# navallo/collision_avoidance

Hardware: AMD Instinct MI355X
Metric: agent-steps/sec (whole node), 4096 arenas x 64 agents per GPU (higher is better)
Workload: dtype f32

## Files before the change

### collision_avoidance_amd/_lib.py

```python
import ctypes as C
import os

from . import build as _build

OBS_DIM = 64
MAX_NEIGHBORS, MAX_OBST_NEIGHBORS, MAX_AGENTS = 16, 64, 1024
MAX_AGENTS_LARGE = 16384
CREATE_TILED = 1
DONE_XLESS, DONE_GOAL, DONE_REGOAL = 0, 1, 2
F_OBS, F_STATS, F_AUTORESET, F_NODONE, F_FREEZE = 1, 2, 4, 8, 16
SCN_CROWD, SCN_CIRCLE, SCN_DOORWAY, SCN_CONGESTED, SCN_INCOMING, SCN_BLOCKS, SCN_DEADLOCK, SCN_CROWD_SEPARATED = range(8)

(FLD_POS_X, FLD_POS_Y, FLD_VEL_X, FLD_VEL_Y, FLD_PREF_X, FLD_PREF_Y, FLD_GOAL_X, FLD_GOAL_Y,
 FLD_GOAL2_X, FLD_GOAL2_Y, FLD_REWARD, FLD_AGENT_DONE, FLD_ARRIVE_STEP, FLD_NB_COUNT, FLD_NB_IDX,
 FLD_OBST_COUNT, FLD_OBST_IDX, FLD_OBS, FLD_STEP_COUNT, FLD_ARENA_DONE, FLD_EPISODE,
 FLD_REGOAL_COUNT, FLD_ALAN_WEIGHTS, FLD_ALAN_TIMES, FLD_ALAN_ACTION, FLD_ARENA_STATS) = range(26)

EXPORTS = ("ca_create", "ca_destroy", "ca_last_error", "ca_set_stream", "ca_set_obstacles", "ca_init_scenario", "ca_set",
           "ca_get", "ca_field_ptr", "ca_bind_obs", "ca_reset", "ca_step", "ca_step_host", "ca_orca_step", "ca_observe", "ca_rollout",
           "ca_get_stats", "ca_reset_stats", "ca_sync", "ca_debug_math", "ca_profile", "ca_profile_read", "ca_launch_info",
           "ca_alan_configure", "ca_alan_step", "ca_alan_rollout", "ca_reset_masked", "ca_get_obstacles",
           "ca_set_obstacles_per_arena", "ca_get_obstacles_arena", "ca_solver_info", "ca_source_sha", "ca_host_alloc", "ca_host_free",
           "ca_step_packed", "ca_allow_obstacle_overflow", "ca_alan_configure_per_arena", "ca_alan_actions_arena",
           "ca_set_agent_params", "ca_get_agent_params", "ca_agent_params_info",
           "ca_set_agent_counts", "ca_get_agent_counts", "ca_agent_counts_info", "ca_create_ex", "ca_tiled_info")


class Config(C.Structure):
    _fields_ = [
        ("n_arenas", C.c_int32), ("n_agents", C.c_int32), ("arena_offset", C.c_int64),
        ("seed", C.c_uint64), ("reward_scale", C.c_double), ("time_step", C.c_float),
        ("neighbor_dist", C.c_float), ("max_neighbors", C.c_int32), ("time_horizon", C.c_float),
        ("time_horizon_obst", C.c_float), ("radius", C.c_float), ("max_speed", C.c_float),
        ("max_obst_neighbors", C.c_int32), ("max_step", C.c_int32), ("done_mode", C.c_int32),
        ("done_x_thresh", C.c_float), ("spawn_x0", C.c_float), ("spawn_x1", C.c_float),
        ("spawn_y0", C.c_float), ("spawn_y1", C.c_float), ("goal_x0", C.c_float),
        ("goal_x1", C.c_float), ("goal_y0", C.c_float), ("goal_y1", C.c_float),
    ]


class Stats(C.Structure):
    _fields_ = [("agent_steps", C.c_uint64), ("episodes", C.c_uint64), ("collisions", C.c_uint64),
                ("obst_collisions", C.c_uint64), ("goals_reached", C.c_uint64),
                ("obst_overflow", C.c_uint64), ("sum_reward", C.c_double)]

    def as_dict(self):
        return {k: getattr(self, k) for k, _ in self._fields_}


_lib = None


def lib_path():
    return _build.LIB_PATH


def load():
    global _lib
    if _lib is not None:
        return _lib
    path = lib_path()
    if not os.path.exists(path):
        raise RuntimeError("libcaenv.so is not built (%s); run `python -m collision_avoidance_amd.build` "
                           "-- the HIP extension is the only implementation of this path" % path)
    L = C.CDLL(path)
    vp, i32, u32, sz = C.c_void_p, C.c_int32, C.c_uint32, C.c_size_t
    L.ca_create.argtypes = [C.POINTER(Config), C.c_int, vp, C.POINTER(vp)]
    L.ca_create_ex.argtypes = [C.POINTER(Config), u32, C.c_int, vp, C.POINTER(vp)]
    L.ca_tiled_info.argtypes = [vp] + [C.POINTER(i32)] * 4
    L.ca_destroy.argtypes = [vp]
    L.ca_last_error.argtypes = [vp]
    L.ca_last_error.restype = C.c_char_p
    L.ca_set_stream.argtypes = [vp, vp]
    L.ca_set_obstacles.argtypes = [vp, vp, vp, i32]
    L.ca_init_scenario.argtypes = [vp, i32]
    L.ca_get_obstacles.argtypes = [vp, vp, vp, vp, i32, C.POINTER(i32)]
    L.ca_set_obstacles_per_arena.argtypes = [vp, vp, vp, vp]
    L.ca_get_obstacles_arena.argtypes = [vp, i32, vp, vp, vp, i32, C.POINTER(i32)]
    L.ca_set.argtypes = [vp, i32, vp, sz, i32]
    L.ca_get.argtypes = [vp, i32, vp, sz, i32]
    L.ca_field_ptr.argtypes = [vp, i32, C.POINTER(vp), C.POINTER(sz)]
    L.ca_bind_obs.argtypes = [vp, vp, sz]
    L.ca_reset.argtypes = [vp, vp, vp, i32, u32]
    L.ca_reset_masked.argtypes = [vp, vp, i32, u32]
    L.ca_step.argtypes = [vp, vp, u32]
    L.ca_step_host.argtypes = [vp, vp, u32]
    L.ca_step_packed.argtypes = [vp, vp, u32, vp, sz]
    L.ca_host_alloc.argtypes = [vp, sz, C.POINTER(vp)]
    L.ca_host_free.argtypes = [vp, vp]
    L.ca_orca_step.argtypes = [vp, u32]
    L.ca_observe.argtypes = [vp]
    L.ca_rollout.argtypes = [vp, i32, u32]
    L.ca_alan_configure.argtypes = [vp, vp, i32, C.c_double, C.c_double, C.c_double]
    L.ca_alan_configure_per_arena.argtypes = [vp, vp, vp, C.c_double, C.c_double, C.c_double]
    L.ca_alan_actions_arena.argtypes = [vp, i32, vp, i32, C.POINTER(i32)]
    L.ca_alan_step.argtypes = [vp, vp, i32, u32]
    L.ca_alan_rollout.argtypes = [vp, i32, u32]
    L.ca_get_stats.argtypes = [vp, C.POINTER(Stats)]
    L.ca_reset_stats.argtypes = [vp]
    L.ca_sync.argtypes = [vp]
    L.ca_allow_obstacle_overflow.argtypes = [vp, i32]
    L.ca_debug_math.argtypes = [vp, i32, vp, vp, i32]
    L.ca_profile.argtypes = [vp, i32]
    L.ca_profile_read.argtypes = [vp, C.POINTER(i32), C.POINTER(C.c_float)]
    L.ca_launch_info.argtypes = [vp] + [C.POINTER(i32)] * 4
    L.ca_solver_info.argtypes = [vp, C.POINTER(i32), C.POINTER(i32)]
    L.ca_set_agent_params.argtypes = [vp, vp, vp, vp, vp, sz, i32]
    L.ca_get_agent_params.argtypes = [vp, vp, vp, vp, vp, sz, i32]
    L.ca_agent_params_info.argtypes = [vp, C.POINTER(i32)]
    L.ca_set_agent_counts.argtypes = [vp, vp, sz, i32]
    L.ca_get_agent_counts.argtypes = [vp, vp, sz, i32]
    L.ca_agent_counts_info.argtypes = [vp, C.POINTER(i32)]
    L.ca_source_sha.argtypes = []
    L.ca_source_sha.restype = C.c_char_p
    for name in EXPORTS:
        if name not in ("ca_last_error", "ca_source_sha"):
            getattr(L, name).restype = C.c_int
    _lib = L
    return L


def check(L, handle, rc, what):
    if rc != 0:
        msg = L.ca_last_error(handle)
        raise RuntimeError("%s failed (%d): %s" % (what, rc, msg.decode() if msg else "?"))
```

### collision_avoidance_amd/csrc/ca_common.h

```cpp
#pragma once
#include "ca_math.h"
#include <type_traits>
#include <utility>

struct AlanArenaSets;
struct WideObstLists;
struct AgentParams;
struct ArenaCounts;

namespace ca {

template <class T, class... P> constexpr bool has_tag = (std::is_same_v<T, P> || ...);

constexpr int SMAX = 16;
constexpr int SWIDE = 64;
constexpr float EPS = 0.00001f;

struct ObstDev {
    float px, py, ux, uy;
    float qx, qy, qux, quy;
    float pux, puy;
    int next, prev;
    int convex, qconvex, pad0, pad1;
};
static_assert(sizeof(ObstDev) == 64, "edge record is one 64-byte line");

struct Line {
    V2 point, dir;
};

struct StepCold {
    float *pos_x, *pos_y, *vel_x, *vel_y, *pref_x, *pref_y;
    double *goal_x, *goal_y;
    const double *goal2_x, *goal2_y;
    float* reward;
    float *orient_x, *orient_y;
    int *agent_done, *arrive_step, *regoal_count;
    int *step_count, *arena_done, *episode;
    unsigned long long* arena_stats;
    unsigned long long* arena_steps;
    unsigned long long* ovf_word;
    double reward_scale;
    uint64_t seed;
    int64_t arena_offset;
    int max_step, done_mode;
    float done_x_thresh;
    float spawn_x0, spawn_x1, spawn_y0, spawn_y1, goal_x0, goal_x1, goal_y0, goal_y1;
    const float *ap_radius, *ap_max_speed, *ap_time_horizon, *ap_time_horizon_obst;
    const int* agent_counts;
};

struct AlanCold {
    double *w, *t;
    int* action;
    float* reward;
    double act_c[32], act_s[32];
    double temp, window, dt, reward_scale;
    const double2* tab;
    const int* tab_n;
    int nA;
};

template <int ALAN, class AL>
__device__ __forceinline__ int alan_count(const AL& al, int a) {
    if constexpr (ALAN == 2) return al.tab_n[a];
    else return al.nA;
}
template <int ALAN, class AL>
__device__ __forceinline__ void alan_cs(const AL& al, int a, int id, double* cs, double* sn) {
    if constexpr (ALAN == 2) {
        const double2 v = al.tab[(size_t)a * 32 + id];
        *cs = v.x; *sn = v.y;
    } else {
        *cs = al.act_c[id]; *sn = al.act_s[id];
    }
}

struct StepArgs {
    const float *pos_x, *pos_y, *vel_x, *vel_y, *pref_x, *pref_y;
    const double *goal_x, *goal_y;
    unsigned short* counts;
    void* nb_idx;
    unsigned short* obst_idx;
    const int* arena_done;
    unsigned long long* arena_stats;
    const StepCold* cold;
    const ObstDev* obst;
    const int* tab_off;
#ifdef CA_STAMPS
    const int* order;
#endif
    const AlanCold* alan;
    const double* alan_u;
    const float* actions;
    const float* reset_px;
    const float* reset_py;
    const int* reset_mask;
    unsigned long long* dbg;
    int n_obst, A, N, P, logP, K, S;
    int a0, a1;
    int LS, apb, linv, dense;
    int nb_hint;
    int T;
    uint32_t flags;
    float time_step, neighbor_dist, time_horizon, time_horizon_obst, radius, max_speed;
};

__device__ __forceinline__ void note_overflow(const StepCold* cold, int a, int i, int oin) {
    const unsigned long long g = (unsigned long long)(cold->arena_offset + (int64_t)a) & 0xFFFFFFFFFFull;
    const unsigned long long v = (1ull << 63) | (g << 20) | ((unsigned long long)(i & 0x7FF) << 8) | (unsigned long long)(oin > 255 ? 255 : oin);
    __hip_atomic_store(cold->ovf_word, v, __ATOMIC_RELAXED, __HIP_MEMORY_SCOPE_SYSTEM);
}

enum { ST_EPISODES = 0, ST_COLL = 1, ST_OBST_COLL = 2, ST_GOALS = 3, ST_OVERFLOW = 4, ST_SUMREW = 5, ST_FROZEN = 6, ST_LASTEP = 7, ST_STRIDE = 8 };

#ifdef CA_STAMPS
__device__ __forceinline__ int work_block(const StepArgs& p) { return p.order ? p.order[blockIdx.x] : (int)blockIdx.x; }
#else
__device__ __forceinline__ int work_block(const StepArgs&) { return (int)blockIdx.x; }
#endif

__device__ __forceinline__ void lane_slot(const StepArgs& p, int tid, int& la, int& i) {
    la = (int)(__umul24((unsigned)tid, (unsigned)p.linv) >> 16);
    i = tid - (int)__umul24((unsigned)la, (unsigned)p.LS);
}

__device__ __forceinline__ bool arena_frozen(const StepArgs& p, int a) {
    return (p.flags & 16u) != 0 && a < p.a1 && p.arena_done[a] != 0;
}

__device__ __forceinline__ void wave_lds_sync() {
    __builtin_amdgcn_fence(__ATOMIC_RELEASE, "wavefront");
    __builtin_amdgcn_s_waitcnt(0xC07F);
    __builtin_amdgcn_wave_barrier();
    __builtin_amdgcn_fence(__ATOMIC_ACQUIRE, "wavefront");
}

#define CA_ROW_DPP(old, v, ctrl, rows) __builtin_amdgcn_update_dpp((int)(old), (int)(v), ctrl, rows, 0xF, false)
__device__ __forceinline__ unsigned wave_min_u32(unsigned v) {
    v = min(v, (unsigned)CA_ROW_DPP(~0u, v, 0x111, 0xF));
    v = min(v, (unsigned)CA_ROW_DPP(~0u, v, 0x112, 0xF));
    v = min(v, (unsigned)CA_ROW_DPP(~0u, v, 0x114, 0xF));
    v = min(v, (unsigned)CA_ROW_DPP(~0u, v, 0x118, 0xF));
    v = min(v, (unsigned)CA_ROW_DPP(~0u, v, 0x142, 0xA));
    v = min(v, (unsigned)CA_ROW_DPP(~0u, v, 0x143, 0xC));
    return v;
}
__device__ __forceinline__ unsigned wave_max_u32(unsigned v) {
    v = max(v, (unsigned)CA_ROW_DPP(0u, v, 0x111, 0xF));
    v = max(v, (unsigned)CA_ROW_DPP(0u, v, 0x112, 0xF));
    v = max(v, (unsigned)CA_ROW_DPP(0u, v, 0x114, 0xF));
    v = max(v, (unsigned)CA_ROW_DPP(0u, v, 0x118, 0xF));
    v = max(v, (unsigned)CA_ROW_DPP(0u, v, 0x142, 0xA));
    v = max(v, (unsigned)CA_ROW_DPP(0u, v, 0x143, 0xC));
    return v;
}
__device__ __forceinline__ int wave_prefix_sum(int v) {
    v += CA_ROW_DPP(0, v, 0x111, 0xF);
    v += CA_ROW_DPP(0, v, 0x112, 0xF);
    v += CA_ROW_DPP(0, v, 0x114, 0xF);
    v += CA_ROW_DPP(0, v, 0x118, 0xF);
    v += CA_ROW_DPP(0, v, 0x142, 0xA);
    v += CA_ROW_DPP(0, v, 0x143, 0xC);
    return v;
}

#ifdef CA_VAR_NB16
#define CA_NBW16(BS) true
#else
#define CA_NBW16(BS) ((BS) > 256)
#endif
#define CA_GLOBAL __attribute__((address_space(1)))
template <bool W16>
__device__ __forceinline__ int ld_idx_t(const void* b, size_t k) {
    if constexpr (W16) return (int)((const CA_GLOBAL unsigned short*)b)[k];
    else return (int)((const CA_GLOBAL unsigned char*)b)[k];
}
template <bool W16>
__device__ __forceinline__ void st_idx_t(void* b, size_t k, int v) {
    if constexpr (W16) ((CA_GLOBAL unsigned short*)b)[k] = (unsigned short)v;
    else ((CA_GLOBAL unsigned char*)b)[k] = (unsigned char)v;
}

__device__ __forceinline__ ObstDev load_obst(const ObstDev* __restrict__ t, int i) {
    const int4* q = reinterpret_cast<const int4*>(t + i);
    const int4 a = q[0], b = q[1], c = q[2], d = q[3];
    ObstDev o;
    o.px = __int_as_float(a.x); o.py = __int_as_float(a.y); o.ux = __int_as_float(a.z); o.uy = __int_as_float(a.w);
    o.qx = __int_as_float(b.x); o.qy = __int_as_float(b.y); o.qux = __int_as_float(b.z); o.quy = __int_as_float(b.w);
    o.pux = __int_as_float(c.x); o.puy = __int_as_float(c.y); o.next = c.z; o.prev = c.w;
    o.convex = d.x; o.qconvex = d.y; o.pad0 = 0; o.pad1 = 0;
    return o;
}

#ifndef CA_PRIO_B1
#define CA_PRIO_B1 2
#define CA_PRIO_B2 4
#define CA_PRIO_B3 6
#endif
#if CA_PRIO_B1 > 0
#define CA_PRIO_START() __builtin_amdgcn_s_setprio(3)
#define CA_PRIO_POINT(x)                                                    \
// ... 48 lines not shown
```

### collision_avoidance_amd/csrc/ca_env.hip

```cpp
#include "../../include/ca_env.h"

#include <hip/hip_runtime.h>
#include <hip/hip_ext.h>

#include <algorithm>
#include <cmath>
#include <cstdarg>
#include <cstdlib>
#include <cstdio>
#include <cstring>
#include <string>
#include <vector>

#include "ca_kernels.h"

using namespace ca;

struct ca_env {
    ca_config cfg;
    int device = 0;
    hipStream_t stream = nullptr;
    bool own_stream = false;
    float *pos_x = nullptr, *pos_y = nullptr, *vel_x = nullptr, *vel_y = nullptr, *pref_x = nullptr,
          *pref_y = nullptr, *reward = nullptr, *orient_x = nullptr, *orient_y = nullptr;
    bool orient_valid = false;
    double *goal_x = nullptr, *goal_y = nullptr, *goal2_x = nullptr, *goal2_y = nullptr;
    int *agent_done = nullptr, *arrive_step = nullptr, *regoal_count = nullptr;
    unsigned short* counts = nullptr;
    void* nb_idx = nullptr;
    unsigned short* obst_idx = nullptr;
    int nidx16 = 0;
    int* cvt_buf = nullptr;
    size_t cvt_cap = 0;
    int *step_count = nullptr, *arena_done = nullptr, *episode = nullptr;
    unsigned long long* arena_stats = nullptr;
    unsigned long long* arena_steps = nullptr;
    float* obs = nullptr;
    bool obs_external = false;
    float* slab = nullptr;
    unsigned long long* dbg = nullptr;
    unsigned long long* dbg_obs = nullptr;
    float *tmp_x = nullptr, *tmp_y = nullptr;
    double *alan_w = nullptr, *alan_t = nullptr, *alan_dirs = nullptr, *alan_u = nullptr;
    int* alan_action = nullptr;
    AlanCold* d_alan = nullptr;
    bool alan_fused = false;
    bool alan_lane = false;
    int* mask_buf = nullptr;
    std::vector<std::pair<void*, size_t>> host_allocs;
    int n_actions = 0;
    double act_c[CA_ALAN_MAX_ACTIONS], act_s[CA_ALAN_MAX_ACTIONS];
    bool alan_per = false;
    double2* d_act_tab = nullptr;
    int* d_act_n = nullptr;
    std::vector<double> h_act_tab;
    std::vector<int> h_act_n;
    double alan_temp = 0.2, alan_window = 2.0, alan_dt = 1.0 / 60.0;
    ObstDev* d_obst = nullptr;
    std::vector<ObstDev> h_obst;
    std::vector<int> h_tab_off;
    int* d_tab_off = nullptr;
    StepCold* d_cold = nullptr;
    unsigned long long* ovf_host = nullptr;
    bool allow_overflow = false;
    int* d_order = nullptr;
    int P = 1, logP = 0, BS = 64, grid = 1, K = 0, S = 1;
    bool obs_dense_on = false;
    bool lists_trusted = true;
    int LS = 1, apb = 1, linv = 65536, dense = 0;
    struct { int reg_lines = -1, pair = -1, alan_fused = -1; } sw;
    int ST = 0, KT = 16;
    int SMX = 4;
    int max_edges = 0;
    int n_cus = 256;
    bool pair = false;
    size_t lds_p = 0;
    bool quad = false;
    bool quad_roll = false;
    int BSq = 64, grid_q = 1, SQ = 4;
    size_t lds_q = 0;
    size_t lds = 0;
    bool ap = false, quad_cfg = false, quad_roll_cfg = false;
    float* d_ap[4] = {nullptr, nullptr, nullptr, nullptr};
    float* d_ap_oct = nullptr;
    std::vector<float> h_ap[4];
    bool ac = false, ap_user = false;
    int* d_counts = nullptr;
    std::vector<int> h_counts;
    bool tiled = false;
    int TILE = 128, tiles = 1;
    float *nv_x = nullptr, *nv_y = nullptr;
    unsigned* tscr = nullptr;
    uint64_t agent_steps_base = 0;
    uint64_t steps_done = 0;
    float rays[32], oct[32];
    bool profiling = false;
    int prof_period = 0;
    struct Span { hipEvent_t t0, t1; int kind; int steps; };
    std::vector<Span> spans;
    std::vector<hipEvent_t> free_events;
    std::string err;
};

static thread_local std::string g_create_err;

static int fail(ca_env* e, int code, const char* fmt, ...) {
    char buf[512];
    va_list ap;
    va_start(ap, fmt);
    vsnprintf(buf, sizeof buf, fmt, ap);
    va_end(ap);
    if (e) e->err = buf;
    else g_create_err = buf;
    return code;
}
#define HIPCHK(e, call)                                                                         \
    do {                                                                                        \
        hipError_t _r = (call);                                                                 \
        if (_r != hipSuccess) return fail(e, CA_EHIP, "%s failed: %s", #call, hipGetErrorString(_r)); \
    } while (0)

static int overflow_status(ca_env* e, const char* where) {
    if (e->allow_overflow || !e->ovf_host) return CA_OK;
    const unsigned long long v = *(volatile unsigned long long*)e->ovf_host;
    if (!(v >> 63)) return CA_OK;
    return fail(e, CA_ERANGE, "%s: an obstacle-neighbour list overflowed: arena %lld, agent %d had %d%s obstacle edges in range but "
                "max_obst_neighbors=%d, so the farthest were dropped (RVO2 keeps every edge in range: collision_avoidence_env.py:249, "
                "301-318).  Raise max_obst_neighbors (at most %d), coarsen the world's polylines, or accept the truncation with "
                "ca_allow_obstacle_overflow(env, 1); ca_reset_stats clears this status", where,
                (long long)(e->tiled ? (v >> 24) & 0xFFFFFFFFFull : (v >> 20) & 0xFFFFFFFFFFull),
                (int)(e->tiled ? (v >> 8) & 0xFFFF : (v >> 8) & 0x7FF), (int)(v & 0xFF), (v & 0xFF) == 255 ? "+" : "",
                e->S, CA_MAX_OBST_NEIGHBORS);
}

enum { KIND_NBR = 0, KIND_STEP = 1, KIND_OBS = 2, KIND_RESET = 3 };
enum { CA_ROLLOUT_MAX_T = 256 };
static hipEvent_t prof_event(ca_env* e) {
    if (!e->free_events.empty()) { hipEvent_t ev = e->free_events.back(); e->free_events.pop_back(); return ev; }
    hipEvent_t ev = nullptr;
    if (hipEventCreate(&ev) != hipSuccess) return nullptr;
    return ev;
}
struct ProfScope {
    ca_env* e; hipEvent_t t0 = nullptr, t1 = nullptr; int kind; int steps;
    ProfScope(ca_env* env, int k, int n_steps = 1) : e(env), kind(k), steps(n_steps) {
        if (!e->profiling) return;
        t0 = prof_event(e);
        t1 = t0 ? prof_event(e) : nullptr;
        if (t0 && !t1) { e->free_events.push_back(t0); t0 = nullptr; }
    }
    ~ProfScope() {
        if (t0) e->spans.push_back({t0, t1, kind, steps});
    }
};
template <class... Args>
static void launch_k(const ProfScope& ps, void (*kernel)(Args...), dim3 grid, dim3 block, size_t lds, hipStream_t stream,
                     Args... args) {
    if (ps.t0) hipExtLaunchKernelGGL(kernel, grid, block, (uint32_t)lds, stream, ps.t0, ps.t1, 0, args...);
    else hipLaunchKernelGGL(kernel, grid, block, lds, stream, args...);
}

static size_t AN(const ca_env* e) { return (size_t)e->cfg.n_arenas * e->cfg.n_agents; }

struct FieldInfo {
    void* ptr;
    size_t bytes;
    bool writable;
};
static FieldInfo field_info(ca_env* e, int f) {
    const size_t an = AN(e), A = e->cfg.n_arenas;
    switch (f) {
        case CA_FLD_POS_X: return {e->pos_x, an * 4, true};
        case CA_FLD_POS_Y: return {e->pos_y, an * 4, true};
        case CA_FLD_VEL_X: return {e->vel_x, an * 4, true};
        case CA_FLD_VEL_Y: return {e->vel_y, an * 4, true};
        case CA_FLD_PREF_X: return {e->pref_x, an * 4, true};
        case CA_FLD_PREF_Y: return {e->pref_y, an * 4, true};
        case CA_FLD_GOAL_X: return {e->goal_x, an * 8, true};
        case CA_FLD_GOAL_Y: return {e->goal_y, an * 8, true};
        case CA_FLD_GOAL2_X: return {e->goal2_x, an * 8, true};
        case CA_FLD_GOAL2_Y: return {e->goal2_y, an * 8, true};
        case CA_FLD_REWARD: return {e->reward, an * 4, true};
        case CA_FLD_AGENT_DONE: return {e->agent_done, an * 4, true};
        case CA_FLD_ARRIVE_STEP: return {e->arrive_step, an * 4, true};
        case CA_FLD_NB_COUNT: return {e->counts, an * 4, true};
        case CA_FLD_NB_IDX: return {e->nb_idx, an * 4 * (size_t)(e->K > 0 ? e->K : 1), true};
        case CA_FLD_OBST_COUNT: return {e->counts, an * 4, true};
        case CA_FLD_OBST_IDX: return {e->obst_idx, an * 4 * (size_t)e->S, true};
        case CA_FLD_OBS: return {e->obs, an * CA_OBS_DIM * 4, false};
        case CA_FLD_STEP_COUNT: return {e->step_count, A * 4, true};
        case CA_FLD_ARENA_DONE: return {e->arena_done, A * 4, true};
        case CA_FLD_EPISODE: return {e->episode, A * 4, true};
        case CA_FLD_REGOAL_COUNT: return {e->regoal_count, an * 4, true};
        case CA_FLD_ALAN_WEIGHTS: return {e->alan_w, an * 8 * (size_t)e->n_actions, true};
        case CA_FLD_ALAN_TIMES: return {e->alan_t, an * 8 * (size_t)e->n_actions, true};
        case CA_FLD_ALAN_ACTION: return {e->alan_action, an * 4, true};
        case CA_FLD_ARENA_STATS: return {e->arena_stats, A * ST_STRIDE * 8, false};
        default: return {nullptr, 0, false};
    }
}

static void host_tables(ca_env* e) {
    const double nd = (double)e->cfg.neighbor_dist, r = (double)e->cfg.radius;
    for (int i = 0; i < 16; ++i) {
        const double th = i * (2.0 * M_PI / 16);
        e->rays[2 * i] = (float)(nd * std::cos(th));
        e->rays[2 * i + 1] = (float)(-nd * std::sin(th));
    }
    double first[2] = {r * std::cos(0.0), -r * std::sin(0.0)}, cur[2] = {first[0], first[1]};
    int k = 0;
    for (int i = 1; i < 8; ++i, ++k) {
        const double th = i * (2.0 * M_PI / 8);
        const double nx = r * std::cos(th), ny = -r * std::sin(th);
        e->oct[4 * k] = (float)cur[0]; e->oct[4 * k + 1] = (float)cur[1];
        e->oct[4 * k + 2] = (float)nx; e->oct[4 * k + 3] = (float)ny;
        cur[0] = nx; cur[1] = ny;
    }
    e->oct[4 * k] = (float)cur[0]; e->oct[4 * k + 1] = (float)cur[1];
    e->oct[4 * k + 2] = (float)first[0]; e->oct[4 * k + 3] = (float)first[1];
}

static void fill_cold(const ca_env* e, StepCold& c) {
    const ca_config& g = e->cfg;
    c.pos_x = e->pos_x; c.pos_y = e->pos_y; c.vel_x = e->vel_x; c.vel_y = e->vel_y;
    c.pref_x = e->pref_x; c.pref_y = e->pref_y; c.goal_x = e->goal_x; c.goal_y = e->goal_y;
    c.goal2_x = e->goal2_x; c.goal2_y = e->goal2_y; c.reward = e->reward;
    c.orient_x = e->orient_x; c.orient_y = e->orient_y;
    c.agent_done = e->agent_done; c.arrive_step = e->arrive_step; c.regoal_count = e->regoal_count;
    c.step_count = e->step_count; c.arena_done = e->arena_done; c.episode = e->episode;
    c.arena_stats = e->arena_stats; c.arena_steps = e->arena_steps; c.ovf_word = e->ovf_host;
    c.reward_scale = g.reward_scale; c.seed = g.seed; c.arena_offset = g.arena_offset;
    c.max_step = g.max_step; c.done_mode = g.done_mode; c.done_x_thresh = g.done_x_thresh;
    c.spawn_x0 = g.spawn_x0; c.spawn_x1 = g.spawn_x1; c.spawn_y0 = g.spawn_y0; c.spawn_y1 = g.spawn_y1;
    c.goal_x0 = g.goal_x0; c.goal_x1 = g.goal_x1; c.goal_y0 = g.goal_y0; c.goal_y1 = g.goal_y1;
    c.ap_radius = e->ap ? e->d_ap[0] : nullptr; c.ap_max_speed = e->ap ? e->d_ap[1] : nullptr;
    c.ap_time_horizon = e->ap ? e->d_ap[2] : nullptr; c.ap_time_horizon_obst = e->ap ? e->d_ap[3] : nullptr;
    c.agent_counts = e->ac ? e->d_counts : nullptr;
}

static void fill_args(ca_env* e, StepArgs& a, const float* actions, uint32_t flags) {
    const ca_config& c = e->cfg;
    a.pos_x = e->pos_x; a.pos_y = e->pos_y; a.vel_x = e->vel_x; a.vel_y = e->vel_y;
    a.pref_x = e->pref_x; a.pref_y = e->pref_y; a.goal_x = e->goal_x; a.goal_y = e->goal_y;
    a.counts = e->counts; a.nb_idx = e->nb_idx; a.obst_idx = e->obst_idx;
    a.arena_done = e->arena_done; a.arena_stats = e->arena_stats; a.cold = e->d_cold;
    a.obst = e->d_obst; a.tab_off = e->d_tab_off; a.actions = actions; a.alan = nullptr; a.alan_u = nullptr;
#ifdef CA_STAMPS
    a.order = e->d_order;
#endif
    a.reset_px = nullptr; a.reset_py = nullptr; a.reset_mask = nullptr; a.dbg = e->dbg;
    a.n_obst = e->h_tab_off.empty() ? (int)e->h_obst.size() : 0; a.A = c.n_arenas; a.N = c.n_agents; a.P = e->P; a.logP = e->logP;
    a.K = e->K; a.S = e->S; a.flags = flags; a.a0 = 0; a.a1 = c.n_arenas; a.T = 1;
    a.LS = e->LS; a.apb = e->apb; a.linv = e->linv; a.dense = e->dense; a.nb_hint = e->lists_trusted ? 1 : 0;
    a.time_step = c.time_step; a.neighbor_dist = c.neighbor_dist; a.time_horizon = c.time_horizon;
    a.time_horizon_obst = c.time_horizon_obst; a.radius = c.radius; a.max_speed = c.max_speed;
}

struct SolveLaunch { const void* fn; dim3 grid, block; size_t lds; };
template <class F> static const void* fn_ptr(F* f) { return reinterpret_cast<const void*>(f); }
template <int KMAX, int ST, int SMX, bool ALAN, class... PER>
static const void* step_fn_for(int BS) {
    if constexpr (ALAN) {
        return BS == 64 ? fn_ptr(&step_kernel<KMAX, 64, ST, SMX, true, PER...>) : fn_ptr(&step_kernel<KMAX, 128, ST, SMX, true, PER...>);
    } else {
        switch (BS) {
            case 64: return fn_ptr(&step_kernel<KMAX, 64, ST, SMX>);
            case 128: return fn_ptr(&step_kernel<KMAX, 128, ST, SMX>);
            case 256: return fn_ptr(&step_kernel<KMAX, 256, ST, SMX>);
            case 512: return fn_ptr(&step_kernel<KMAX, 512, ST, SMX>);
            default: return fn_ptr(&step_kernel<KMAX, 1024, ST, SMX>);
        }
    }
}
template <int KMAX>
static const void* pair_fn_for(int BS) {
    return BS == 256 ? fn_ptr(&pair_kernel<KMAX, 256>) : fn_ptr(&pair_kernel<KMAX, 512>);
}
template <int KMAX, int SQ, bool ALAN, class... PER>
static const void* quad_fn_for(int BS) {
    switch (BS) {
        case 64: return fn_ptr(&quad_kernel<KMAX, 64, SQ, ALAN, PER...>);
        case 128: return fn_ptr(&quad_kernel<KMAX, 128, SQ, ALAN, PER...>);
        case 256: return fn_ptr(&quad_kernel<KMAX, 256, SQ, ALAN, PER...>);
        default: return fn_ptr(&quad_kernel<KMAX, 512, SQ, ALAN, PER...>);
    }
}
template <int KMAX>
static const void* wide_fn_for(int BS) {
    return BS == 64 ? fn_ptr(&step_kernel<KMAX, 64, 0, SWIDE>) : fn_ptr(&step_kernel<KMAX, 128, 0, SWIDE>);
}
template <int KMAX>
static const void* ap_fn_for(int BS) {
    switch (BS) {
        case 64: return fn_ptr(&step_kernel<KMAX, 64, 0, SMAX, false, AgentParams>);
        case 128: return fn_ptr(&step_kernel<KMAX, 128, 0, SMAX, false, AgentParams>);
        case 256: return fn_ptr(&step_kernel<KMAX, 256, 0, SMAX, false, AgentParams>);
        case 512: return fn_ptr(&step_kernel<KMAX, 512, 0, SMAX, false, AgentParams>);
        default: return fn_ptr(&step_kernel<KMAX, 1024, 0, SMAX, false, AgentParams>);
    }
}
template <int KMAX>
static const void* ac_fn_for(int BS) {
    switch (BS) {
        case 64: return fn_ptr(&step_kernel<KMAX, 64, 0, SMAX, false, ArenaCounts>);
        case 128: return fn_ptr(&step_kernel<KMAX, 128, 0, SMAX, false, ArenaCounts>);
        case 256: return fn_ptr(&step_kernel<KMAX, 256, 0, SMAX, false, ArenaCounts>);
        case 512: return fn_ptr(&step_kernel<KMAX, 512, 0, SMAX, false, ArenaCounts>);
        default: return fn_ptr(&step_kernel<KMAX, 1024, 0, SMAX, false, ArenaCounts>);
    }
}
template <bool ALAN, class... PER>
static const void* lane_fn_for(const ca_env* e) {
    if (e->ac) return e->KT == 5 ? ac_fn_for<5>(e->BS) : (e->KT == 16 ? ac_fn_for<16>(e->BS) : ac_fn_for<10>(e->BS));
    if (e->ap) return e->KT == 5 ? ap_fn_for<5>(e->BS) : (e->KT == 16 ? ap_fn_for<16>(e->BS) : ap_fn_for<10>(e->BS));
    if (e->SMX > SMAX) return e->KT == 5 ? wide_fn_for<5>(e->BS) : (e->KT == 16 ? wide_fn_for<16>(e->BS) : wide_fn_for<10>(e->BS));
    if (e->ST > 0 && e->SMX > 4) return e->KT == 5 ? step_fn_for<5, 4, 16, ALAN, PER...>(e->BS) : step_fn_for<10, 4, 16, ALAN, PER...>(e->BS);
    if (e->ST > 0) return e->KT == 5 ? step_fn_for<5, 4, 4, ALAN, PER...>(e->BS) : step_fn_for<10, 4, 4, ALAN, PER...>(e->BS);
    if (e->KT == 5) return step_fn_for<5, 0, SMAX, ALAN, PER...>(e->BS);
    if constexpr (!ALAN) { if (e->KT == 16) return step_fn_for<16, 0, SMAX, false>(e->BS); }
    return step_fn_for<10, 0, SMAX, ALAN, PER...>(e->BS);
}
template <bool ALAN, class... PER>
static const void* quad_fn_for(const ca_env* e) {
    if (e->SQ > 4) return e->KT == 5 ? quad_fn_for<5, 16, ALAN, PER...>(e->BSq) : quad_fn_for<10, 16, ALAN, PER...>(e->BSq);
    return e->KT == 5 ? quad_fn_for<5, 4, ALAN, PER...>(e->BSq) : quad_fn_for<10, 4, ALAN, PER...>(e->BSq);
}
template <int KMAX>
static const void* tiled_fn_for(int TILE) {
    switch (TILE) {
        case 64: return fn_ptr(&tiled_solve_kernel<KMAX, 64>);
        case 256: return fn_ptr(&tiled_solve_kernel<KMAX, 256>);
        default: return fn_ptr(&tiled_solve_kernel<KMAX, 128>);
    }
}
static SolveLaunch solve_launch(const ca_env* e, bool alan, bool rollout) {
    if (e->tiled)
        return {e->KT == 5 ? tiled_fn_for<5>(e->TILE) : (e->KT == 16 ? tiled_fn_for<16>(e->TILE) : tiled_fn_for<10>(e->TILE)),
                dim3(e->grid), dim3(e->TILE), e->lds};
    const bool per = alan && e->alan_per;
    if (e->quad || (rollout && e->quad_roll) || (alan && !e->alan_lane)) {
        const void* f = per ? quad_fn_for<true, AlanArenaSets>(e) : (alan ? quad_fn_for<true>(e) : quad_fn_for<false>(e));
        return {f, dim3(e->grid_q), dim3(e->BSq), alan ? quad_lds_bytes(e->BSq, e->KT, e->SQ, e->n_actions) : e->lds_q};
    }
    if (e->pair)
        return {e->KT == 5 ? pair_fn_for<5>(e->BS) : pair_fn_for<10>(e->BS), dim3(e->grid), dim3(2 * e->BS), e->lds_p};
    const void* f = per ? lane_fn_for<true, AlanArenaSets>(e) : (alan ? lane_fn_for<true>(e) : lane_fn_for<false>(e));
    return {f, dim3(e->grid), dim3(e->BS), e->lds};
}
static hipError_t allow_lds(const SolveLaunch& s) {
    return s.lds > 48 * 1024 ? hipFuncSetAttribute(s.fn, hipFuncAttributeMaxDynamicSharedMemorySize, (int)s.lds) : hipSuccess;
}
static hipError_t launch_step(ca_env* e, const StepArgs& a) {
    const SolveLaunch s = solve_launch(e, a.alan != nullptr, a.T > 1);
    if (!(a.flags & CA_F_FREEZE)) e->lists_trusted = true;
    if (e->tiled) {
        TiledArgs ta;
        ta.s = a; ta.nv_x = e->nv_x; ta.nv_y = e->nv_y; ta.scr = e->tscr; ta.tiles = e->tiles;
        void* params[] = {&ta};
        const void* fns[3] = {s.fn, fn_ptr(&tiled_advance_kernel), fn_ptr(&tiled_close_kernel)};
        const size_t lds[3] = {s.lds, 0, (size_t)e->TILE * 8};
        for (int k = 0; k < 3; ++k) {
            ProfScope ps(e, KIND_STEP);
            const hipError_t r = ps.t0 ? hipExtLaunchKernel(fns[k], s.grid, s.block, params, lds[k], e->stream, ps.t0, ps.t1, 0)
                                       : hipLaunchKernel(fns[k], s.grid, s.block, params, lds[k], e->stream);
            if (r != hipSuccess) return r;
        }
        return hipSuccess;
    }
    ProfScope ps(e, KIND_STEP, a.T > 1 ? a.T : 1);
    StepArgs arg = a;
    void* params[] = {&arg};
    if (ps.t0) return hipExtLaunchKernel(s.fn, s.grid, s.block, params, s.lds, e->stream, ps.t0, ps.t1, 0);
    return hipLaunchKernel(s.fn, s.grid, s.block, params, s.lds, e->stream);
}

typedef void (*obs_fn_t)(const ObsArgs);
static obs_fn_t obs_fn(int obs_bs, bool w16, bool dense = false, bool wide = false, bool ap = false, bool ac = false) {
    if (ac) return dense ? obs_kernel<256, false, true, ArenaCounts> : (w16 ? obs_kernel<256, true, false, ArenaCounts> : obs_kernel<256, false, false, ArenaCounts>);
    if (ap) return dense ? obs_kernel<256, false, true, AgentParams> : (w16 ? obs_kernel<256, true, false, AgentParams> : obs_kernel<256, false, false, AgentParams>);
    if (wide) return dense ? obs_kernel<256, false, true, WideObstLists> : obs_kernel<256, false, false, WideObstLists>;
    if (dense) return obs_kernel<256, false, true>;
    switch (obs_bs) {
        case 1024: return w16 ? obs_kernel<1024, true> : obs_kernel<1024, false>;
        case 512: return w16 ? obs_kernel<512, true> : obs_kernel<512, false>;
        case 128: return w16 ? obs_kernel<128, true> : obs_kernel<128, false>;
        case 64: return w16 ? obs_kernel<64, true> : obs_kernel<64, false>;
        default: return w16 ? obs_kernel<256, true> : obs_kernel<256, false>;
    }
}

static bool obs_dense(const ca_env* e) { return e->obs_dense_on; }
static int obs_nstage(const ca_env* e) { return e->tiled ? 0 : (obs_dense(e) ? 16 + 2 * e->cfg.n_agents : e->cfg.n_agents); }
static bool obs_wide(const ca_env* e) { return e->S > SMAX; }
static size_t obs_lds(const ca_env* e, int obs_bs) {
    if (e->ap) return obs_lds_bytes_ap(obs_nstage(e), obs_bs, 16 * (e->K + e->S));
    return obs_lds_bytes(obs_nstage(e), obs_bs, 16 * (e->K + e->S), obs_wide(e) ? e->S : 16);
}
static obs_fn_t obs_fn_of(const ca_env* e) { return obs_fn(obs_block_threads(e->cfg.n_agents), e->nidx16 != 0, obs_dense(e), obs_wide(e), e->ap, e->ac); }
static hipError_t allow_obs_lds(const ca_env* e) {
    const size_t ol = obs_lds(e, obs_block_threads(e->cfg.n_agents));
    return ol > 48 * 1024 ? hipFuncSetAttribute(reinterpret_cast<const void*>(obs_fn_of(e)), hipFuncAttributeMaxDynamicSharedMemorySize, (int)ol) : hipSuccess;
}

static hipError_t launch_obs(ca_env* e) {
    if (!e->orient_valid) {
        StepArgs a;
        fill_args(e, a, nullptr, 0);
        const unsigned an = (unsigned)AN(e);
        hipLaunchKernelGGL(orient_kernel, dim3((an + 255) / 256), dim3(256), 0, e->stream, a);
        hipError_t r = hipGetLastError();
        if (r != hipSuccess) return r;
        e->orient_valid = true;
    }
    ObsArgs o;
    o.pos_x = e->pos_x; o.pos_y = e->pos_y; o.vel_x = e->vel_x; o.vel_y = e->vel_y;
    o.orient_x = e->orient_x; o.orient_y = e->orient_y; o.counts = e->counts; o.nb_idx = e->nb_idx;
    o.obst_idx = e->obst_idx; o.obst = e->d_obst; o.tab_off = e->d_tab_off;
    o.obs = e->obs;
    o.A = e->cfg.n_arenas; o.N = e->cfg.n_agents; o.S = e->S;
    o.K = e->K > 0 ? e->K : 1;
    const int obs_bs = obs_block_threads(o.N), apb = obs_bs / 16;
    o.bpa = (o.N + apb - 1) / apb;
    o.paircap = 16 * (e->K + e->S);
    o.a0 = 0; o.dbg = e->dbg_obs;
    o.dense = obs_dense(e) ? 1 : 0;
    o.nstage_max = obs_nstage(e);
    o.xcd = (o.A % 8 == 0 && !o.dense) ? 1 : 0;
    o.radius = e->cfg.radius;
    memcpy(o.rays, e->rays, sizeof o.rays);
    memcpy(o.oct, e->oct, sizeof o.oct);
    o.ap_oct = e->ap ? e->d_ap_oct : nullptr;
    o.agent_counts = e->ac ? e->d_counts : nullptr;
    const dim3 grid(o.dense ? (unsigned)(((size_t)o.A * o.N + apb - 1) / apb) : (unsigned)((size_t)o.A * o.bpa)), block(obs_bs);
    const size_t lds = obs_lds(e, obs_bs);
    ProfScope ps(e, KIND_OBS);
    launch_k(ps, obs_fn_of(e), grid, block, lds, e->stream, o);
    return hipGetLastError();
}

static hipError_t launch_reset(ca_env* e, const StepArgs& a) {
    const unsigned an = (unsigned)AN(e);
    {
        ProfScope ps(e, KIND_RESET);
        launch_k(ps, e->ac ? reset_counts_kernel : reset_kernel, dim3((an + 255) / 256), dim3(256), 0, e->stream, a);
    }
    hipError_t r = hipGetLastError();
    if (r != hipSuccess) return r;
    {
        ProfScope ps(e, KIND_RESET);
        launch_k(ps, reset_arena_kernel, dim3((e->cfg.n_arenas + 255) / 256), dim3(256), 0, e->stream, a);
    }
    return hipGetLastError();
}

static void split_crossing_edges(std::vector<ObstDev>& tab) {
    struct Side { int left, right; };
    auto sides = [&](int split, int edge, float* a, float* b) {
        const V2 s1 = mk(tab[split].px, tab[split].py), s2 = mk(tab[tab[split].next].px, tab[tab[split].next].py);
        *a = leftOf(s1, s2, mk(tab[edge].px, tab[edge].py));
        *b = leftOf(s1, s2, mk(tab[tab[edge].next].px, tab[tab[edge].next].py));
    };
    auto worse_or_equal = [](Side x, Side y) {
        const int xm = x.left > x.right ? x.left : x.right, xn = x.left < x.right ? x.left : x.right;
        const int ym = y.left > y.right ? y.left : y.right, yn = y.left < y.right ? y.left : y.right;
        return xm > ym || (xm == ym && xn >= yn);
    };
    std::vector<std::vector<int>> work(1);
    for (int i = 0; i < (int)tab.size(); ++i) work[0].push_back(i);
    while (!work.empty()) {
        const std::vector<int> edges = std::move(work.back());
        work.pop_back();
        const int n = (int)edges.size();
        if (n == 0) continue;
        int pick = 0;
        Side best = {n, n};
        for (int i = 0; i < n; ++i) {
            Side c = {0, 0};
            for (int j = 0; j < n; ++j) {
                if (j == i) continue;
                float a, b;
                sides(edges[i], edges[j], &a, &b);
                if (a >= -EPS && b >= -EPS) ++c.left;
                else if (a <= EPS && b <= EPS) ++c.right;
                else { ++c.left; ++c.right; }
                if (worse_or_equal(c, best)) break;
            }
            if (!worse_or_equal(c, best)) { best = c; pick = i; }
        }
        std::vector<int> lhs, rhs;
        const int sp = edges[pick];
        const V2 s1 = mk(tab[sp].px, tab[sp].py), s2 = mk(tab[tab[sp].next].px, tab[tab[sp].next].py);
        for (int j = 0; j < n; ++j) {
            if (j == pick) continue;
            const int e1 = edges[j], e2 = tab[e1].next;
            float a, b;
            sides(sp, e1, &a, &b);
            if (a >= -EPS && b >= -EPS) { lhs.push_back(e1); continue; }
            if (a <= EPS && b <= EPS) { rhs.push_back(e1); continue; }
            const V2 p1 = mk(tab[e1].px, tab[e1].py), p2 = mk(tab[e2].px, tab[e2].py);
            const float t = det(s2 - s1, p1 - s1) / det(s2 - s1, p1 - p2);
            const V2 cut = p1 + t * (p2 - p1);
            ObstDev o;
            memset(&o, 0, sizeof o);
            o.px = cut.x; o.py = cut.y; o.ux = tab[e1].ux; o.uy = tab[e1].uy;
            o.prev = e1; o.next = e2; o.convex = 1;
            const int id = (int)tab.size();
            tab.push_back(o);
            tab[e1].next = id; tab[e2].prev = id;
            if (a > 0.0f) { lhs.push_back(e1); rhs.push_back(id); }
            else { rhs.push_back(e1); lhs.push_back(id); }
        }
        work.push_back(std::move(rhs));
        work.push_back(std::move(lhs));
    }
}

template <class T>
static hipError_t dalloc(ca_env* e, T** p, size_t n, bool zero = true) {
    hipError_t r = hipMalloc((void**)p, n * sizeof(T));
    if (r != hipSuccess || !zero) return r;
    return hipMemsetAsync(*p, 0, n * sizeof(T), e->stream);
}
static hipError_t upload(ca_env* e, void* dst, const void* src, size_t bytes) {
    hipError_t r = hipMemcpyAsync(dst, src, bytes, hipMemcpyHostToDevice, e->stream);
    return r != hipSuccess ? r : hipStreamSynchronize(e->stream);
}
static hipError_t download(ca_env* e, void* dst, const void* src, size_t bytes) {
    hipError_t r = hipMemcpyAsync(dst, src, bytes, hipMemcpyDeviceToHost, e->stream);
    return r != hipSuccess ? r : hipStreamSynchronize(e->stream);
}

static size_t lds_static_bytes(const ca_env* e) {
    return (size_t)e->BS * 8 +
           (e->BS >= 1024 ? (size_t)e->BS * 2 + 16 + 1024 + 1028 : (e->BS >= 256 ? (size_t)e->BS * 2 + (size_t)e->BS * 8 + 16 + 4096 + 4100 : 0)) + 64;
}

static void pick_variant(ca_env* e) {
    const bool allow = e->sw.reg_lines != 0, force = e->sw.reg_lines == 1;
    e->KT = e->K <= 5 ? 5 : (e->K <= 10 ? 10 : 16);
    if (e->tiled) {
        e->ST = 0; e->SMX = SMAX; e->pair = false;
        e->lds = tiled_lds_bytes(e->TILE, e->K, e->S);
        return;
    }
    const size_t table_per_wg = step_lds_bytes(e->BS, e->K, e->S, 0, e->KT) + lds_static_bytes(e);
    const bool table_fits = table_per_wg <= 160 * 1024;
    const bool small_world = e->max_edges <= 16;
    const bool table_resident = table_fits && (long)e->grid <= (long)e->n_cus * (long)((160 * 1024) / table_per_wg);
    if (e->S > SMAX) { e->ST = 0; e->SMX = SWIDE; }
    else if (e->ap) { e->ST = 0; e->SMX = SMAX; }
    else if (allow && e->K <= 10 && e->S <= 4) { e->ST = 4; e->SMX = 4; }
    else if (allow && e->K <= 10 && (small_world || force || !table_resident)) { e->ST = 4; e->SMX = 16; }
    else { e->ST = 0; e->SMX = 16; }
    e->lds = e->ap ? step_lds_bytes_ap(e->BS, e->K, e->S) : step_lds_bytes(e->BS, e->K, e->S, e->ST, e->KT);
    e->pair = e->sw.pair != 0 && e->ST > 0 && e->SMX == 4 && (e->BS == 256 || e->BS == 512) && e->K > 0;
    e->lds_p = pair_lds_bytes(e->BS, e->KT);
}

static const size_t LDS_PER_CU = 160 * 1024;
static hipError_t apply_variant_attributes(ca_env* e, bool* misfit) {
    const SolveLaunch plain = solve_launch(e, false, false);
    if (e->tiled) { *misfit = false; return allow_lds(plain); }
    *misfit = !e->pair && e->lds + lds_static_bytes(e) > LDS_PER_CU;
    hipError_t r = hipSuccess;
    if (e->pair) {
        hipFuncAttributes fa;
        r = hipFuncGetAttributes(&fa, plain.fn);
        *misfit = r == hipSuccess && fa.sharedSizeBytes + plain.lds > LDS_PER_CU;
    }
    if (r != hipSuccess || *misfit) return r;
    r = allow_lds(plain);
    if (r == hipSuccess) r = allow_lds(solve_launch(e, false, true));
    return r;
}

static int alan_pick(ca_env* e) {
    e->alan_fused = e->alan_lane = false;
    if (e->n_actions <= 0 || e->tiled) return CA_OK;
    const size_t lq = quad_lds_bytes(e->BSq, e->KT, e->SQ, e->n_actions);
    const bool on = e->sw.alan_fused != 0;
    e->alan_fused = on && (e->quad || e->quad_roll) && lq <= 64 * 1024;
    e->alan_lane = on && !e->ap && !e->quad && !e->pair && e->BS <= 128 && e->K <= 10 && e->S <= SMAX &&
                   e->n_actions <= (e->ST > 0 ? 4 + e->KT : 2 * (e->K + e->S));
    if (e->alan_fused) HIPCHK(e, allow_lds(solve_launch(e, true, true)));
    if (e->alan_lane) HIPCHK(e, allow_lds(solve_launch(e, true, false)));
    return CA_OK;
}

extern "C" {

const char* ca_last_error(const ca_env* env) { return env ? env->err.c_str() : g_create_err.c_str(); }

int ca_create(const ca_config* cfg, int device, void* stream, ca_env** out) { return ca_create_ex(cfg, 0u, device, stream, out); }

int ca_create_ex(const ca_config* cfg, uint32_t create_flags, int device, void* stream, ca_env** out) {
    if (!cfg || !out) return fail(nullptr, CA_EINVAL, "ca_create: null argument");
    *out = nullptr;
    if (create_flags & ~CA_CREATE_TILED) return fail(nullptr, CA_EINVAL, "ca_create_ex: unknown create_flags 0x%x", create_flags);
    const bool tiled = (create_flags & CA_CREATE_TILED) != 0;
    const int max_agents = tiled ? CA_MAX_AGENTS_LARGE : CA_MAX_AGENTS;
    if (cfg->n_arenas <= 0 || cfg->n_agents <= 0 || cfg->n_agents > max_agents)
        return fail(nullptr, CA_ERANGE, "ca_create: n_arenas=%d n_agents=%d out of range (agents 1..%d)",
                    cfg->n_arenas, cfg->n_agents, max_agents);
    if (tiled && cfg->max_obst_neighbors > SMAX)
        return fail(nullptr, CA_ERANGE, "ca_create_ex: max_obst_neighbors=%d: wide obstacle lists (above %d) have no tiled form",
                    cfg->max_obst_neighbors, SMAX);
    if (cfg->max_neighbors < 0 || cfg->max_neighbors > CA_MAX_NEIGHBORS)
        return fail(nullptr, CA_ERANGE, "ca_create: max_neighbors=%d out of range 0..%d", cfg->max_neighbors,
                    CA_MAX_NEIGHBORS);
    if (cfg->max_obst_neighbors < 1 || cfg->max_obst_neighbors > CA_MAX_OBST_NEIGHBORS)
        return fail(nullptr, CA_ERANGE, "ca_create: max_obst_neighbors=%d out of range 1..%d",
                    cfg->max_obst_neighbors, CA_MAX_OBST_NEIGHBORS);
    if (cfg->done_mode < 0 || cfg->done_mode > 2) return fail(nullptr, CA_EINVAL, "ca_create: bad done_mode");
    {
        const struct { const char* name; float v, lo, hi; } rng[] = {
            {"time_step", cfg->time_step, CA_MIN_TIME_STEP, CA_MAX_TIME_STEP}, {"neighbor_dist", cfg->neighbor_dist, CA_MIN_LENGTH, CA_MAX_LENGTH},
            {"time_horizon", cfg->time_horizon, CA_MIN_LENGTH, CA_MAX_LENGTH}, {"time_horizon_obst", cfg->time_horizon_obst, CA_MIN_LENGTH, CA_MAX_LENGTH},
            {"radius", cfg->radius, CA_MIN_LENGTH, CA_MAX_LENGTH}, {"max_speed", cfg->max_speed, CA_MIN_LENGTH, CA_MAX_LENGTH}};
        for (const auto& q : rng)
            if (!(q.v >= q.lo && q.v <= q.hi))
                return fail(nullptr, CA_ERANGE, "ca_create: %s=%g outside the supported range [%g, %g]", q.name, (double)q.v, (double)q.lo, (double)q.hi);
        const float box[] = {cfg->spawn_x0, cfg->spawn_x1, cfg->spawn_y0, cfg->spawn_y1, cfg->goal_x0, cfg->goal_x1, cfg->goal_y0, cfg->goal_y1,
                             cfg->done_x_thresh};
        for (float v : box)
            if (!(fabsf(v) <= CA_MAX_COORD)) return fail(nullptr, CA_ERANGE, "ca_create: a spawn / goal box coordinate (%g) is beyond %g or not a number", (double)v, (double)CA_MAX_COORD);
    }
    if ((size_t)cfg->n_arenas * cfg->n_agents > (size_t)1 << 30)
        return fail(nullptr, CA_ERANGE, "ca_create: more than 2^30 agents on one handle");
    int ndev = 0;
    if (hipGetDeviceCount(&ndev) != hipSuccess || ndev <= 0)
        return fail(nullptr, CA_ENODEV, "ca_create: no HIP device (this library has no CPU path)");
    if (device < 0 || device >= ndev) return fail(nullptr, CA_ENODEV, "ca_create: device %d of %d", device, ndev);
    ca_env* e = new ca_env();
    e->cfg = *cfg;
    e->device = device;
    hipError_t r = hipSetDevice(device);
    if (r == hipSuccess) {
        if (stream) e->stream = (hipStream_t)stream;
        else { r = hipStreamCreateWithFlags(&e->stream, hipStreamNonBlocking); e->own_stream = true; }
    }
    {
        auto digit = [](const char* name) { const char* v = getenv(name); return (v && v[0] >= '0' && v[0] <= '9') ? v[0] - '0' : -1; };
        e->sw.reg_lines = digit("CA_REG_LINES"); e->sw.pair = digit("CA_PAIR"); e->sw.alan_fused = digit("CA_ALAN_FUSED");
    }
    e->tiled = tiled;
    if (tiled) {
        const char* v = getenv("CA_TILE");
        const int want = v ? atoi(v) : 0;
        e->TILE = (want == 64 || want == 256) ? want : 128;
        e->tiles = (cfg->n_agents + e->TILE - 1) / e->TILE;
    }
    int P = 1, logP = 0;
    while (P < cfg->n_agents) { P <<= 1; ++logP; }
    e->P = P; e->logP = logP;
    e->BS = P > 64 ? P : 64;
    e->LS = P; e->apb = e->BS / P; e->linv = 65536 / P; e->dense = 0;
    e->grid = (cfg->n_arenas + e->apb - 1) / e->apb;
    if (tiled) {
        if ((size_t)cfg->n_arenas * e->tiles > (size_t)0x7FFFFFFF) {
            fail(nullptr, CA_ERANGE, "ca_create_ex: n_arenas=%d x %d tiles per arena is more workgroups than a launch holds", cfg->n_arenas, e->tiles);
            if (e->own_stream && e->stream) hipStreamDestroy(e->stream);
            delete e;
            return CA_ERANGE;
        }
        e->BS = e->TILE; e->LS = e->TILE; e->apb = 1; e->linv = 65536 / e->TILE;
        e->grid = cfg->n_arenas * e->tiles;
    }
    {
        const char* v = getenv("CA_OBS_DENSE");
        e->obs_dense_on = !tiled && cfg->n_agents < 16 && !(v && v[0] == '0');
    }
    {
        const char* v = getenv("CA_DENSE");
        const int N = cfg->n_agents;
        if (!tiled && !(v && v[0] == '0') && e->BS == 64 && P < 64 && 64 / N > 64 / P) {
            const int linv = (65536 + N - 1) / N;
            bool exact = true;
            for (int t = 0; t < 64; ++t) exact = exact && ((t * linv) >> 16) == t / N;
            if (exact) {
                e->LS = N; e->apb = 64 / N; e->linv = linv; e->dense = 1;
                e->grid = (cfg->n_arenas + e->apb - 1) / e->apb;
            }
        }
    }
    e->K = cfg->max_neighbors;
    e->S = cfg->max_obst_neighbors;
    {
        int cus = 0;
        if (hipDeviceGetAttribute(&cus, hipDeviceAttributeMultiprocessorCount, device) == hipSuccess && cus > 0) e->n_cus = cus;
    }
    pick_variant(e);
    {
        const char* v = getenv("CA_QUAD");
        e->SQ = e->S <= 4 ? 4 : 16;
        const bool fits = !tiled && e->S <= SMAX && e->K <= 10 && 4 * P <= ((e->SQ == 16 && e->KT == 10) ? 256 : 512);
        const long lane_waves = tiled ? 0 : (long)((cfg->n_arenas + e->BS / P - 1) / (e->BS / P)) * (e->BS / 64);
        e->quad = fits && (v ? v[0] == '1' : lane_waves < 1024);
        e->quad_roll = fits && (v ? v[0] == '1' : lane_waves <= 1024);
        e->BSq = 4 * P > 64 ? 4 * P : 64;
        const int apbq = (e->BSq / 4) / P;
        e->grid_q = (cfg->n_arenas + apbq - 1) / apbq;
        e->lds_q = quad_lds_bytes(e->BSq, e->KT, e->SQ);
        e->quad_cfg = e->quad; e->quad_roll_cfg = e->quad_roll;
    }
    if (e->S > SMAX && (e->lds + lds_static_bytes(e) > LDS_PER_CU || e->BS > 128 || obs_block_threads(cfg->n_agents) != 256)) {
        if (e->lds + lds_static_bytes(e) > LDS_PER_CU)
            fail(nullptr, CA_ERANGE, "ca_create: the solve kernel for n_agents=%d, max_neighbors=%d, max_obst_neighbors=%d does not fit the "
                 "160 KiB of LDS of a CU (%zu B: obstacle lists above %d take the LDS line table, max_neighbors + max_obst_neighbors lines "
                 "per lane)", cfg->n_agents, e->K, e->S, e->lds + lds_static_bytes(e), SMAX);
        else
            fail(nullptr, CA_ERANGE, "ca_create: max_obst_neighbors=%d: obstacle lists above %d are built for arenas of at most 128 agents "
                 "(n_agents=%d)", e->S, SMAX, cfg->n_agents);
        if (e->own_stream && e->stream) hipStreamDestroy(e->stream);
        delete e;
        return CA_ERANGE;
    }
    if (!tiled && !e->pair && e->lds + lds_static_bytes(e) > LDS_PER_CU) {
        fail(nullptr, CA_ERANGE, "ca_create: the solve kernel would need %zu B of LDS (> 160 KiB) for n_agents=%d, "
             "max_neighbors=%d, max_obst_neighbors=%d: arenas above 256 agents need max_neighbors <= 10 "
             "(register-line variant)", e->lds + lds_static_bytes(e), cfg->n_agents, e->K, e->S);
        if (e->own_stream && e->stream) hipStreamDestroy(e->stream);
        delete e;
        return CA_ERANGE;
    }
    host_tables(e);
    const size_t an = AN(e), A = cfg->n_arenas;
    float** f32s[] = {&e->pos_x, &e->pos_y, &e->vel_x, &e->vel_y, &e->pref_x, &e->pref_y,
                      &e->tmp_x, &e->tmp_y, &e->orient_x, &e->orient_y};
    for (auto p : f32s) if (r == hipSuccess) r = dalloc(e, p, an);
    double** f64s[] = {&e->goal_x, &e->goal_y, &e->goal2_x, &e->goal2_y};
    for (auto p : f64s) if (r == hipSuccess) r = dalloc(e, p, an);
    int** i32s[] = {&e->agent_done, &e->arrive_step, &e->regoal_count};
    for (auto p : i32s) if (r == hipSuccess) r = dalloc(e, p, an);
    if (tiled) {
        if (r == hipSuccess) r = dalloc(e, &e->nv_x, an);
        if (r == hipSuccess) r = dalloc(e, &e->nv_y, an);
        if (r == hipSuccess) r = dalloc(e, &e->tscr, A * (size_t)TS_STRIDE);
    }
    e->nidx16 = (tiled || CA_NBW16(e->BS)) ? 1 : 0;
    if (r == hipSuccess) r = dalloc(e, &e->counts, an);
    if (r == hipSuccess) r = dalloc(e, reinterpret_cast<unsigned char**>(&e->nb_idx),
                                    an * (size_t)(e->K > 0 ? e->K : 1) * (e->nidx16 ? 2 : 1));
    if (r == hipSuccess) r = dalloc(e, &e->obst_idx, an * (size_t)e->S);
    if (r == hipSuccess) r = dalloc(e, &e->slab, an * CA_OBS_DIM + an + 2 * A);
    if (r == hipSuccess) {
        e->obs = e->slab; e->reward = e->slab + an * CA_OBS_DIM;
        e->arena_done = reinterpret_cast<int*>(e->reward + an); e->step_count = e->arena_done + A;
    }
    if (r == hipSuccess) r = dalloc(e, &e->episode, A);
    if (r == hipSuccess) r = dalloc(e, &e->arena_stats, A * ST_STRIDE);
    if (r == hipSuccess) r = dalloc(e, &e->arena_steps, A);
    if (r == hipSuccess) r = dalloc(e, &e->d_obst, (size_t)1);
#ifdef CA_STAMPS
    if (r == hipSuccess) r = dalloc(e, &e->dbg, (size_t)std::max(e->grid * (2 * e->BS / 64), e->grid_q * (e->BSq / 64)) * 16);
    if (r == hipSuccess) r = dalloc(e, &e->dbg_obs, (size_t)cfg->n_arenas * ((cfg->n_agents + 15) / 16 + 16) * 4 * 16);
#endif
    bool lds_misfit = false;
    if (r == hipSuccess) r = apply_variant_attributes(e, &lds_misfit);
    if (r == hipSuccess) r = allow_obs_lds(e);
    if (r == hipSuccess) {
        r = hipHostMalloc((void**)&e->ovf_host, sizeof(unsigned long long), hipHostMallocDefault);
        if (r == hipSuccess) *e->ovf_host = 0ull;
    }
    if (r == hipSuccess) r = hipMalloc((void**)&e->d_cold, sizeof(StepCold));
    if (r == hipSuccess) {
        StepCold hc;
        fill_cold(e, hc);
        r = upload(e, e->d_cold, &hc, sizeof hc);
    }
    if (r == hipSuccess) r = hipStreamSynchronize(e->stream);
    if (r == hipSuccess && lds_misfit) {
        fail(nullptr, CA_ERANGE, "ca_create: the solve kernel for n_agents=%d, max_neighbors=%d, max_obst_neighbors=%d does not fit the "
             "160 KiB of LDS of a CU", cfg->n_agents, e->K, e->S);
        ca_destroy(e);
        return CA_ERANGE;
    }
    if (r != hipSuccess) {
        fail(nullptr, CA_EHIP, "ca_create: %s", hipGetErrorString(r));
        ca_destroy(e);
        return CA_EHIP;
    }
    *out = e;
    return CA_OK;
}

int ca_destroy(ca_env* e) {
    if (!e) return CA_OK;
    hipSetDevice(e->device);
    if (e->stream) hipStreamSynchronize(e->stream);
    void* bufs[] = {e->pos_x, e->pos_y, e->vel_x, e->vel_y, e->pref_x, e->pref_y, e->goal_x, e->goal_y,
                    e->goal2_x, e->goal2_y, e->slab, e->tmp_x, e->tmp_y, e->orient_x, e->orient_y,
                    e->agent_done, e->arrive_step,
                    e->regoal_count, e->counts, e->nb_idx, e->obst_idx, e->cvt_buf, e->d_tab_off, e->d_cold, e->d_order,
                    e->episode, e->arena_stats, e->arena_steps, e->d_obst, e->dbg, e->dbg_obs,
                    e->alan_w, e->alan_t, e->alan_dirs, e->alan_u, e->alan_action, e->d_alan, e->mask_buf,
                    e->d_act_tab, e->d_act_n, e->d_ap[0], e->d_ap[1], e->d_ap[2], e->d_ap[3], e->d_ap_oct, e->d_counts,
                    e->nv_x, e->nv_y, e->tscr};
    for (void* b : bufs) if (b) hipFree(b);
    for (const auto& h : e->host_allocs) hipHostFree(h.first);
    if (e->ovf_host) hipHostFree(e->ovf_host);
    for (const ca_env::Span& sp : e->spans) { hipEventDestroy(sp.t0); hipEventDestroy(sp.t1); }
    for (hipEvent_t ev : e->free_events) hipEventDestroy(ev);
    if (e->own_stream && e->stream) hipStreamDestroy(e->stream);
    delete e;
    return CA_OK;
}

int ca_set_stream(ca_env* e, void* stream) {
    if (!e) return CA_EINVAL;
    HIPCHK(e, hipSetDevice(e->device));
    HIPCHK(e, hipStreamSynchronize(e->stream));
    if (e->own_stream && e->stream) HIPCHK(e, hipStreamDestroy(e->stream));
    e->stream = (hipStream_t)stream;
    e->own_stream = false;
    return CA_OK;
}

static int build_table(ca_env* e, const float* verts_xy, const int32_t* poly_sizes, int n_poly, std::vector<ObstDev>& tab) {
    size_t off = 0;
    for (int pi = 0; pi < n_poly; ++pi) {
        const int n = poly_sizes[pi];
        if (n < 2) return fail(e, CA_EINVAL, "ca_set_obstacles: polygon %d has %d vertices (need >= 2)", pi, n);
        const int base = (int)tab.size();
        for (int i = 0; i < n; ++i) {
            const int in = (i == n - 1) ? 0 : i + 1, ip = (i == 0) ? n - 1 : i - 1;
            const V2 pt = mk(verts_xy[2 * (off + i)], verts_xy[2 * (off + i) + 1]);
            const V2 pn = mk(verts_xy[2 * (off + in)], verts_xy[2 * (off + in) + 1]);
            const V2 pp = mk(verts_xy[2 * (off + ip)], verts_xy[2 * (off + ip) + 1]);
            if (!(fabsf(pt.x) <= CA_MAX_COORD && fabsf(pt.y) <= CA_MAX_COORD))
                return fail(e, CA_ERANGE, "ca_set_obstacles: polygon %d vertex %d = (%g, %g) is beyond %g or not a number", pi, i,
                            (double)pt.x, (double)pt.y, (double)CA_MAX_COORD);
            if (pn.x == pt.x && pn.y == pt.y)
                return fail(e, CA_EINVAL, "ca_set_obstacles: polygon %d has an edge of length zero (vertex %d twice)", pi, i);
            if (absSq(pn - pt) < CA_MIN_EDGE * CA_MIN_EDGE)
                return fail(e, CA_ERANGE, "ca_set_obstacles: polygon %d edge %d is shorter than %g", pi, i, (double)CA_MIN_EDGE);
            const V2 u = normalize(pn - pt);
            ObstDev o;
            memset(&o, 0, sizeof o);
            o.px = pt.x; o.py = pt.y; o.ux = u.x; o.uy = u.y;
            o.next = base + in; o.prev = base + ip;
            o.convex = (n == 2) ? 1 : (leftOf(pp, pt, pn) >= 0.0f ? 1 : 0);
            tab.push_back(o);
        }
        off += n;
    }
    split_crossing_edges(tab);
    for (ObstDev& o : tab) {
        const ObstDev& nx = tab[o.next];
        const ObstDev& pv = tab[o.prev];
        o.qx = nx.px; o.qy = nx.py; o.qux = nx.ux; o.quy = nx.uy; o.qconvex = nx.convex;
        o.pux = pv.ux; o.puy = pv.uy;
    }
    return CA_OK;
}

__global__ void clear_obst_counts_kernel(unsigned short* counts, size_t n) {
    const size_t q = (size_t)blockIdx.x * blockDim.x + threadIdx.x;
    if (q < n) counts[q] &= 0x00FFu;
}

static int install_tables(ca_env* e, std::vector<ObstDev>& all, std::vector<int>& offs) {
    HIPCHK(e, hipSetDevice(e->device));
    HIPCHK(e, hipStreamSynchronize(e->stream));
    ObstDev* n_obst = nullptr;
    int* n_off = nullptr;
    hipError_t r = hipMalloc((void**)&n_obst, (all.size() + 1) * sizeof(ObstDev));
    if (r == hipSuccess && !all.empty()) r = upload(e, n_obst, all.data(), all.size() * sizeof(ObstDev));
    if (r == hipSuccess && !offs.empty()) {
        r = hipMalloc((void**)&n_off, offs.size() * sizeof(int));
        if (r == hipSuccess) r = upload(e, n_off, offs.data(), offs.size() * sizeof(int));
    }
    if (r == hipSuccess) {
        const size_t an = AN(e);
        hipLaunchKernelGGL(clear_obst_counts_kernel, dim3((unsigned)((an + 255) / 256)), dim3(256), 0, e->stream, e->counts, an);
        r = hipGetLastError();
        if (r == hipSuccess) r = hipStreamSynchronize(e->stream);
    }
    if (r != hipSuccess) {
        if (n_obst) hipFree(n_obst);
        if (n_off) hipFree(n_off);
        return fail(e, CA_EHIP, "ca_set_obstacles: %s (the previous tables stay installed)", hipGetErrorString(r));
    }
    int me = 0;
    if (offs.empty()) me = (int)all.size();
    else for (size_t a = 0; a + 1 < offs.size(); ++a) me = std::max(me, offs[a + 1] - offs[a]);
    struct { int ST, SMX, KT, max_edges; bool pair; size_t lds, lds_p; } old_v = {e->ST, e->SMX, e->KT, e->max_edges, e->pair, e->lds, e->lds_p};
    e->max_edges = me;
    pick_variant(e);
    bool misfit = false;
    const hipError_t ra = apply_variant_attributes(e, &misfit);
    if (misfit || ra != hipSuccess) {
        e->ST = old_v.ST; e->SMX = old_v.SMX; e->KT = old_v.KT; e->max_edges = old_v.max_edges; e->pair = old_v.pair;
        e->lds = old_v.lds; e->lds_p = old_v.lds_p;
        bool dummy = false;
        (void)apply_variant_attributes(e, &dummy);
        hipFree(n_obst);
        if (n_off) hipFree(n_off);
        if (misfit)
            return fail(e, CA_ERANGE, "ca_set_obstacles: the solve kernel this world selects does not fit the 160 KiB of LDS of a CU "
                        "(n_agents=%d, max_neighbors=%d, max_obst_neighbors=%d); the previous tables stay installed", e->cfg.n_agents, e->K, e->S);
        return fail(e, CA_EHIP, "ca_set_obstacles: %s (the previous tables stay installed)", hipGetErrorString(ra));
    }
    if (e->d_obst) hipFree(e->d_obst);
    if (e->d_tab_off) hipFree(e->d_tab_off);
    e->d_obst = n_obst;
    e->d_tab_off = n_off;
    e->h_obst.swap(all);
    e->h_tab_off.swap(offs);
    return alan_pick(e);
}

int ca_set_obstacles(ca_env* e, const float* verts_xy, const int32_t* poly_sizes, int32_t n_poly) {
    if (!e || n_poly < 0 || (n_poly > 0 && (!verts_xy || !poly_sizes))) return fail(e, CA_EINVAL, "ca_set_obstacles: bad argument");
    std::vector<ObstDev> tab;
    const int rc = build_table(e, verts_xy, poly_sizes, n_poly, tab);
    if (rc) return rc;
    if (tab.size() > 65536) return fail(e, CA_ERANGE, "ca_set_obstacles: %zu edges (at most 65536)", tab.size());
    std::vector<int> none;
    return install_tables(e, tab, none);
}

int ca_set_obstacles_per_arena(ca_env* e, const float* verts_xy, const int32_t* poly_sizes, const int32_t* n_poly) {
    if (!e || !n_poly) return fail(e, CA_EINVAL, "ca_set_obstacles_per_arena: null argument");
    const int A = e->cfg.n_arenas;
    std::vector<ObstDev> all;
    std::vector<int> offs(1, 0);
    size_t voff = 0, poff = 0;
    for (int a = 0; a < A; ++a) {
        if (n_poly[a] < 0 || (n_poly[a] > 0 && (!verts_xy || !poly_sizes)))
            return fail(e, CA_EINVAL, "ca_set_obstacles_per_arena: bad argument for arena %d", a);
        std::vector<ObstDev> tab;
        const int rc = build_table(e, verts_xy ? verts_xy + 2 * voff : nullptr, poly_sizes ? poly_sizes + poff : nullptr,
                                   n_poly[a], tab);
        if (rc) return rc;
        for (int k = 0; k < n_poly[a]; ++k) voff += (size_t)poly_sizes[poff + k];
        poff += (size_t)n_poly[a];
        if (tab.size() > 65536) return fail(e, CA_ERANGE, "ca_set_obstacles_per_arena: arena %d has %zu edges (at most 65536)", a, tab.size());
        all.insert(all.end(), tab.begin(), tab.end());
        if (all.size() > (size_t)0x7FFFFFFF) return fail(e, CA_ERANGE, "ca_set_obstacles_per_arena: too many edges");
        offs.push_back((int)all.size());
    }
    return install_tables(e, all, offs);
}

static int get_table(ca_env* e, int arena, float* verts_xy, int32_t* next, int32_t* convex, int32_t cap, int32_t* n_out) {
    const bool per = !e->h_tab_off.empty();
    const int t0 = per ? e->h_tab_off[arena] : 0;
    const int n = per ? e->h_tab_off[arena + 1] - t0 : (int)e->h_obst.size();
    *n_out = n;
    for (int i = 0; i < n && i < cap; ++i) {
// ... 458 lines not shown
    HIPCHK(e, hipMemsetAsync(e->arrive_step, 0xff, an * 4, st));
    HIPCHK(e, hipMemsetAsync(e->regoal_count, 0, an * 4, st));
    HIPCHK(e, hipMemsetAsync(e->counts, 0, an * 2, st));
    HIPCHK(e, hipMemsetAsync(e->step_count, 0, (size_t)A * 4, st));
    HIPCHK(e, hipMemsetAsync(e->arena_done, 0, (size_t)A * 4, st));
    HIPCHK(e, hipMemsetAsync(e->episode, 0, (size_t)A * 4, st));
    HIPCHK(e, hipMemsetAsync(e->obs, 0, an * CA_OBS_DIM * 4, st));
    HIPCHK(e, hipStreamSynchronize(st));
    e->orient_valid = false;
    return CA_OK;
}

__global__ void unpack_list_kernel(const void* src, int kind, int w16, int* dst, size_t n) {
    const size_t q = (size_t)blockIdx.x * blockDim.x + threadIdx.x;
    if (q >= n) return;
    if (kind == 0) dst[q] = (int)(reinterpret_cast<const unsigned short*>(src)[q] & 0xFFu);
    else if (kind == 1) dst[q] = (int)(reinterpret_cast<const unsigned short*>(src)[q] >> 8);
    else dst[q] = w16 ? ld_idx_t<true>(src, q) : ld_idx_t<false>(src, q);
}
__global__ void pack_list_kernel(const int* src, int kind, int w16, void* dst, size_t n) {
    const size_t q = (size_t)blockIdx.x * blockDim.x + threadIdx.x;
    if (q >= n) return;
    unsigned short* c = reinterpret_cast<unsigned short*>(dst);
    if (kind == 0) c[q] = (unsigned short)((c[q] & 0xFF00u) | ((unsigned)src[q] & 0xFFu));
    else if (kind == 1) c[q] = (unsigned short)((c[q] & 0x00FFu) | (((unsigned)src[q] & 0xFFu) << 8));
    else if (w16) st_idx_t<true>(dst, q, src[q]);
    else st_idx_t<false>(dst, q, src[q]);
}
static bool packed_field(int f) {
    return f == CA_FLD_NB_COUNT || f == CA_FLD_OBST_COUNT || f == CA_FLD_NB_IDX || f == CA_FLD_OBST_IDX;
}
static int packed_kind(int f) { return f == CA_FLD_NB_COUNT ? 0 : (f == CA_FLD_OBST_COUNT ? 1 : 2); }
static int cvt_reserve(ca_env* e, size_t elems) {
    if (e->cvt_cap >= elems) return CA_OK;
    HIPCHK(e, hipStreamSynchronize(e->stream));
    if (e->cvt_buf) HIPCHK(e, hipFree(e->cvt_buf));
    e->cvt_buf = nullptr; e->cvt_cap = 0;
    HIPCHK(e, hipMalloc((void**)&e->cvt_buf, elems * sizeof(int)));
    e->cvt_cap = elems;
    return CA_OK;
}

int ca_set(ca_env* e, int32_t field, const void* src, size_t bytes, int32_t src_is_device) {
    if (!e || !src) return fail(e, CA_EINVAL, "ca_set: null argument");
    const FieldInfo fi = field_info(e, field);
    if (!fi.ptr) return fail(e, CA_EINVAL, "ca_set: unknown field %d", field);
    if (!fi.writable) return fail(e, CA_EINVAL, "ca_set: field %d is read-only", field);
    if (bytes != fi.bytes) return fail(e, CA_ESIZE, "ca_set: field %d holds %zu bytes, got %zu", field, fi.bytes, bytes);
    HIPCHK(e, hipSetDevice(e->device));
    if (packed_field(field)) {
        e->lists_trusted = false;
        const size_t n = bytes / 4;
        const int rc = cvt_reserve(e, n);
        if (rc) return rc;
        HIPCHK(e, hipMemcpyAsync(e->cvt_buf, src, bytes, src_is_device ? hipMemcpyDeviceToDevice : hipMemcpyHostToDevice, e->stream));
        hipLaunchKernelGGL(pack_list_kernel, dim3((unsigned)((n + 255) / 256)), dim3(256), 0, e->stream, e->cvt_buf,
                           packed_kind(field), field == CA_FLD_NB_IDX ? e->nidx16 : 1, fi.ptr, n);
        HIPCHK(e, hipGetLastError());
        HIPCHK(e, hipStreamSynchronize(e->stream));
        return CA_OK;
    }
    HIPCHK(e, hipMemcpyAsync(fi.ptr, src, bytes, src_is_device ? hipMemcpyDeviceToDevice : hipMemcpyHostToDevice, e->stream));
    if (!src_is_device) HIPCHK(e, hipStreamSynchronize(e->stream));
    if (field == CA_FLD_POS_X || field == CA_FLD_POS_Y || field == CA_FLD_GOAL_X || field == CA_FLD_GOAL_Y)
        e->orient_valid = false;
    return CA_OK;
}

int ca_get(ca_env* e, int32_t field, void* dst, size_t bytes, int32_t dst_is_device) {
    if (!e || !dst) return fail(e, CA_EINVAL, "ca_get: null argument");
    const FieldInfo fi = field_info(e, field);
    if (!fi.ptr) return fail(e, CA_EINVAL, "ca_get: unknown field %d", field);
    if (bytes != fi.bytes) return fail(e, CA_ESIZE, "ca_get: field %d holds %zu bytes, got %zu", field, fi.bytes, bytes);
    HIPCHK(e, hipSetDevice(e->device));
    if (packed_field(field)) {
        const size_t n = bytes / 4;
        const int rc = cvt_reserve(e, n);
        if (rc) return rc;
        hipLaunchKernelGGL(unpack_list_kernel, dim3((unsigned)((n + 255) / 256)), dim3(256), 0, e->stream, fi.ptr,
                           packed_kind(field), field == CA_FLD_NB_IDX ? e->nidx16 : 1, e->cvt_buf, n);
        HIPCHK(e, hipGetLastError());
        HIPCHK(e, hipMemcpyAsync(dst, e->cvt_buf, bytes, dst_is_device ? hipMemcpyDeviceToDevice : hipMemcpyDeviceToHost, e->stream));
        HIPCHK(e, hipStreamSynchronize(e->stream));
        return CA_OK;
    }
    HIPCHK(e, hipMemcpyAsync(dst, fi.ptr, bytes, dst_is_device ? hipMemcpyDeviceToDevice : hipMemcpyDeviceToHost, e->stream));
    if (!dst_is_device) HIPCHK(e, hipStreamSynchronize(e->stream));
    return CA_OK;
}

int ca_field_ptr(ca_env* e, int32_t field, void** dev_ptr, size_t* bytes) {
    if (!e || !dev_ptr) return fail(e, CA_EINVAL, "ca_field_ptr: null argument");
    const FieldInfo fi = field_info(e, field);
    if (!fi.ptr) return fail(e, CA_EINVAL, "ca_field_ptr: unknown field %d", field);
    if (packed_field(field))
        return fail(e, CA_EINVAL, "ca_field_ptr: field %d is stored packed (u8/u16); read it through ca_get", field);
    *dev_ptr = fi.ptr;
    if (bytes) *bytes = fi.bytes;
    return CA_OK;
}

int ca_bind_obs(ca_env* e, void* dev_ptr, size_t bytes) {
    if (!e || !dev_ptr) return fail(e, CA_EINVAL, "ca_bind_obs: null argument");
    if (bytes != AN(e) * CA_OBS_DIM * 4)
        return fail(e, CA_ESIZE, "ca_bind_obs: need %zu bytes, got %zu", AN(e) * CA_OBS_DIM * 4, bytes);
    if (((uintptr_t)dev_ptr & 15) != 0) return fail(e, CA_EINVAL, "ca_bind_obs: buffer must be 16-byte aligned");
    HIPCHK(e, hipSetDevice(e->device));
    HIPCHK(e, hipStreamSynchronize(e->stream));
    e->obs = (float*)dev_ptr;
    e->obs_external = true;
    return CA_OK;
}

int ca_reset(ca_env* e, const float* pos_x, const float* pos_y, int32_t pos_is_device, uint32_t flags) {
    if (!e) return CA_EINVAL;
    if ((pos_x == nullptr) != (pos_y == nullptr)) return fail(e, CA_EINVAL, "ca_reset: pos_x and pos_y go together");
    HIPCHK(e, hipSetDevice(e->device));
    StepArgs a;
    fill_args(e, a, nullptr, flags);
    if (pos_x) {
        if (pos_is_device) { a.reset_px = pos_x; a.reset_py = pos_y; }
        else {
            HIPCHK(e, hipMemcpyAsync(e->tmp_x, pos_x, AN(e) * 4, hipMemcpyHostToDevice, e->stream));
            HIPCHK(e, hipMemcpyAsync(e->tmp_y, pos_y, AN(e) * 4, hipMemcpyHostToDevice, e->stream));
            HIPCHK(e, hipStreamSynchronize(e->stream));
            a.reset_px = e->tmp_x; a.reset_py = e->tmp_y;
        }
    }
    HIPCHK(e, launch_reset(e, a));
    HIPCHK(e, hipGetLastError());
    e->orient_valid = true;
    if (flags & CA_F_OBS) HIPCHK(e, launch_obs(e));
    return CA_OK;
}

int ca_reset_masked(ca_env* e, const int32_t* mask, int32_t mask_is_device, uint32_t flags) {
    if (!e || !mask) return fail(e, CA_EINVAL, "ca_reset_masked: null argument");
    HIPCHK(e, hipSetDevice(e->device));
    const int A = e->cfg.n_arenas;
    if (!mask_is_device) {
        if (!e->mask_buf) HIPCHK(e, dalloc(e, &e->mask_buf, (size_t)A, false));
        HIPCHK(e, upload(e, e->mask_buf, mask, (size_t)A * 4));
        mask = e->mask_buf;
    }
    StepArgs a;
    fill_args(e, a, nullptr, flags);
    a.reset_mask = mask;
    HIPCHK(e, launch_reset(e, a));
    HIPCHK(e, hipGetLastError());
    if (flags & CA_F_OBS) HIPCHK(e, launch_obs(e));
    return CA_OK;
}

static int do_step(ca_env* e, const float* actions, uint32_t flags) {
    { const int rs = overflow_status(e, "step"); if (rs) return rs; }
    if (e->prof_period > 1) e->profiling = (e->steps_done % (uint64_t)e->prof_period) == 0;
    StepArgs a;
    fill_args(e, a, actions, flags);
    HIPCHK(e, launch_step(e, a));
    e->orient_valid = true;
    if (flags & CA_F_OBS) HIPCHK(e, launch_obs(e));
    e->steps_done += 1;
    return CA_OK;
}

int ca_step(ca_env* e, const float* actions, uint32_t flags) {
    if (!e) return CA_EINVAL;
    if (!actions) return fail(e, CA_EINVAL, "ca_step: actions is null (use ca_orca_step for the ORCA-only step)");
    if (flags & CA_F_NODONE) return fail(e, CA_EINVAL, "ca_step: CA_F_NODONE applies to ca_orca_step only");
    HIPCHK(e, hipSetDevice(e->device));
    return do_step(e, actions, flags);
}

int ca_step_host(ca_env* e, const float* actions_host, uint32_t flags) {
    if (!e) return CA_EINVAL;
    if (!actions_host) return fail(e, CA_EINVAL, "ca_step_host: actions is null");
    if (flags & CA_F_NODONE) return fail(e, CA_EINVAL, "ca_step_host: CA_F_NODONE applies to ca_orca_step only");
    HIPCHK(e, hipSetDevice(e->device));
    HIPCHK(e, hipMemcpyAsync(e->tmp_x, actions_host, AN(e) * 4, hipMemcpyHostToDevice, e->stream));
    HIPCHK(e, hipStreamSynchronize(e->stream));
    return do_step(e, e->tmp_x, flags);
}

int ca_step_packed(ca_env* e, const float* actions_host, uint32_t flags, void* out_host, size_t out_bytes) {
    if (!e || !out_host) return fail(e, CA_EINVAL, "ca_step_packed: null argument");
    const size_t an = AN(e), A = (size_t)e->cfg.n_arenas;
    const size_t obs_b = an * CA_OBS_DIM * 4, rest_b = an * 4 + 2 * A * 4;
    if (out_bytes != obs_b + rest_b) return fail(e, CA_ESIZE, "ca_step_packed: need %zu bytes, got %zu", obs_b + rest_b, out_bytes);
    if (actions_host && (flags & CA_F_NODONE)) return fail(e, CA_EINVAL, "ca_step_packed: CA_F_NODONE applies to the ORCA-only step");
    HIPCHK(e, hipSetDevice(e->device));
    const float* act = nullptr;
    if (actions_host) {
        bool mapped = false;
        for (const auto& h : e->host_allocs)
            if ((const char*)actions_host >= (const char*)h.first && (const char*)actions_host + an * 4 <= (const char*)h.first + h.second) { mapped = true; break; }
        if (mapped) act = actions_host;
        else {
            HIPCHK(e, hipMemcpyAsync(e->tmp_x, actions_host, an * 4, hipMemcpyHostToDevice, e->stream));
            act = e->tmp_x;
        }
    }
    const int rc = do_step(e, act, flags);
    if (rc) return rc;
    char* out = (char*)out_host;
    if (!e->obs_external) {
        HIPCHK(e, hipMemcpyAsync(out, e->slab, obs_b + rest_b, hipMemcpyDeviceToHost, e->stream));
    } else {
        HIPCHK(e, hipMemcpyAsync(out, e->obs, obs_b, hipMemcpyDeviceToHost, e->stream));
        HIPCHK(e, hipMemcpyAsync(out + obs_b, e->reward, rest_b, hipMemcpyDeviceToHost, e->stream));
    }
    HIPCHK(e, hipStreamSynchronize(e->stream));
    return overflow_status(e, "ca_step_packed");
}

int ca_orca_step(ca_env* e, uint32_t flags) {
    if (!e) return CA_EINVAL;
    HIPCHK(e, hipSetDevice(e->device));
    return do_step(e, nullptr, flags);
}

static void alan_unit(double x, double y, double* c, double* s) {
    const double len = std::sqrt(x * x + y * y);
    *c = len == 0.0 ? 1.0 : x / len;
    *s = len == 0.0 ? 0.0 : y / len;
}

static int alan_install(ca_env* e, int nA, double temp, double timewindow, double time_step) {
    for (double** b : {&e->alan_w, &e->alan_t, &e->alan_dirs, &e->alan_u}) { if (*b) hipFree(*b); *b = nullptr; }
    if (e->alan_action) { hipFree(e->alan_action); e->alan_action = nullptr; }
    const size_t an = AN(e);
    HIPCHK(e, dalloc(e, &e->alan_w, an * (size_t)nA));
    HIPCHK(e, dalloc(e, &e->alan_t, an * (size_t)nA));
    HIPCHK(e, dalloc(e, &e->alan_dirs, an * 4));
    HIPCHK(e, dalloc(e, &e->alan_u, an));
    HIPCHK(e, dalloc(e, &e->alan_action, an));
    if (e->alan_per) {
        const size_t A = (size_t)e->cfg.n_arenas;
        if (!e->d_act_tab) HIPCHK(e, hipMalloc((void**)&e->d_act_tab, A * CA_ALAN_MAX_ACTIONS * sizeof(double2)));
        if (!e->d_act_n) HIPCHK(e, hipMalloc((void**)&e->d_act_n, A * sizeof(int)));
        HIPCHK(e, hipMemcpyAsync(e->d_act_tab, e->h_act_tab.data(), A * CA_ALAN_MAX_ACTIONS * sizeof(double2),
                                 hipMemcpyHostToDevice, e->stream));
        HIPCHK(e, hipMemcpyAsync(e->d_act_n, e->h_act_n.data(), A * sizeof(int), hipMemcpyHostToDevice, e->stream));
    }
    HIPCHK(e, hipStreamSynchronize(e->stream));
    e->n_actions = nA;
    e->alan_temp = temp; e->alan_window = timewindow; e->alan_dt = time_step;
    {
        if (!e->d_alan) HIPCHK(e, hipMalloc((void**)&e->d_alan, sizeof(AlanCold)));
        AlanCold h;
        memset(&h, 0, sizeof h);
        h.w = e->alan_w; h.t = e->alan_t; h.action = e->alan_action; h.reward = e->reward;
        memcpy(h.act_c, e->act_c, sizeof h.act_c); memcpy(h.act_s, e->act_s, sizeof h.act_s);
        h.temp = temp; h.window = timewindow; h.dt = time_step; h.reward_scale = e->cfg.reward_scale; h.nA = nA;
        h.tab = e->alan_per ? e->d_act_tab : nullptr;
        h.tab_n = e->alan_per ? e->d_act_n : nullptr;
        HIPCHK(e, upload(e, e->d_alan, &h, sizeof h));
    }
    return alan_pick(e);
}

int ca_alan_configure(ca_env* e, const double* actions_xy, int32_t n_actions, double temp, double timewindow,
                      double time_step) {
    if (!e || !actions_xy) return fail(e, CA_EINVAL, "ca_alan_configure: null argument");
    if (e->ac) return fail(e, CA_EINVAL, "ca_alan_configure: ALAN is not supported while per-arena agent counts are set");
    if (n_actions < 1 || n_actions > CA_ALAN_MAX_ACTIONS)
        return fail(e, CA_ERANGE, "ca_alan_configure: n_actions=%d out of range 1..%d", n_actions, CA_ALAN_MAX_ACTIONS);
    if (!(temp > 0.0) || !(timewindow > 0.0) || !(time_step > 0.0))
        return fail(e, CA_EINVAL, "ca_alan_configure: temp, timewindow and time_step must be positive");
    HIPCHK(e, hipSetDevice(e->device));
    HIPCHK(e, hipStreamSynchronize(e->stream));
    e->n_actions = 0;
    for (int k = 0; k < n_actions; ++k) alan_unit(actions_xy[2 * k], actions_xy[2 * k + 1], &e->act_c[k], &e->act_s[k]);
    e->alan_per = false;
    return alan_install(e, n_actions, temp, timewindow, time_step);
}

int ca_alan_configure_per_arena(ca_env* e, const double* actions_xy, const int32_t* n_actions, double temp, double timewindow,
                                double time_step) {
    if (!e || !actions_xy || !n_actions) return fail(e, CA_EINVAL, "ca_alan_configure_per_arena: null argument");
    if (e->ac) return fail(e, CA_EINVAL, "ca_alan_configure_per_arena: ALAN is not supported while per-arena agent counts are set");
    const int A = e->cfg.n_arenas;
    int nmax = 0;
    for (int a = 0; a < A; ++a) {
        if (n_actions[a] < 1 || n_actions[a] > CA_ALAN_MAX_ACTIONS)
            return fail(e, CA_ERANGE, "ca_alan_configure_per_arena: n_actions[%d]=%d out of range 1..%d", a, n_actions[a],
                        CA_ALAN_MAX_ACTIONS);
        nmax = n_actions[a] > nmax ? n_actions[a] : nmax;
    }
    if (!(temp > 0.0) || !(timewindow > 0.0) || !(time_step > 0.0))
        return fail(e, CA_EINVAL, "ca_alan_configure_per_arena: temp, timewindow and time_step must be positive");
    HIPCHK(e, hipSetDevice(e->device));
    HIPCHK(e, hipStreamSynchronize(e->stream));
    e->n_actions = 0;
    e->h_act_tab.assign((size_t)A * CA_ALAN_MAX_ACTIONS * 2, 0.0);
    e->h_act_n.assign(n_actions, n_actions + A);
    size_t off = 0;
    for (int a = 0; a < A; ++a)
        for (int k = 0; k < n_actions[a]; ++k, ++off) {
            double* cs = &e->h_act_tab[((size_t)a * CA_ALAN_MAX_ACTIONS + k) * 2];
            alan_unit(actions_xy[2 * off], actions_xy[2 * off + 1], cs, cs + 1);
        }
    e->alan_per = true;
    return alan_install(e, nmax, temp, timewindow, time_step);
}

int ca_alan_actions_arena(ca_env* e, int32_t arena, double* cs_xy, int32_t cap, int32_t* n_out) {
    if (!e || !n_out) return fail(e, CA_EINVAL, "ca_alan_actions_arena: null argument");
    if (arena < 0 || arena >= e->cfg.n_arenas)
        return fail(e, CA_ERANGE, "ca_alan_actions_arena: arena %d of %d", arena, e->cfg.n_arenas);
    if (e->n_actions <= 0) return fail(e, CA_EINVAL, "ca_alan_actions_arena: call ca_alan_configure first");
    const int n = e->alan_per ? e->h_act_n[arena] : e->n_actions;
    *n_out = n;
    if (!cs_xy) return CA_OK;
    for (int k = 0; k < n && k < cap; ++k) {
        if (e->alan_per) {
            cs_xy[2 * k] = e->h_act_tab[((size_t)arena * CA_ALAN_MAX_ACTIONS + k) * 2];
            cs_xy[2 * k + 1] = e->h_act_tab[((size_t)arena * CA_ALAN_MAX_ACTIONS + k) * 2 + 1];
        } else {
            cs_xy[2 * k] = e->act_c[k]; cs_xy[2 * k + 1] = e->act_s[k];
        }
    }
    return CA_OK;
}

int ca_alan_step(ca_env* e, const double* u, int32_t u_is_device, uint32_t flags) {
    if (!e) return CA_EINVAL;
    if (e->ac) return fail(e, CA_EINVAL, "ca_alan_step: ALAN is not supported while per-arena agent counts are set");
    if (e->n_actions <= 0) return fail(e, CA_EINVAL, "ca_alan_step: call ca_alan_configure first");
    if (flags & (CA_F_AUTORESET | CA_F_NODONE))
        return fail(e, CA_EINVAL, "ca_alan_step: CA_F_AUTORESET / CA_F_NODONE do not apply (ALAN:106-123)");
    HIPCHK(e, hipSetDevice(e->device));
    { const int rs = overflow_status(e, "ca_alan_step"); if (rs) return rs; }
    if (u && !u_is_device) {
        HIPCHK(e, hipMemcpyAsync(e->alan_u, u, AN(e) * 8, hipMemcpyHostToDevice, e->stream));
        HIPCHK(e, hipStreamSynchronize(e->stream));
        u = e->alan_u;
    }
    if (e->prof_period > 1) e->profiling = (e->steps_done % (uint64_t)e->prof_period) == 0;
    if ((e->alan_fused && e->quad) || e->alan_lane) {
        StepArgs a;
        fill_args(e, a, nullptr, flags);
        a.alan = e->d_alan; a.alan_u = u;
        HIPCHK(e, launch_step(e, a));
        e->orient_valid = true;
        if (flags & CA_F_OBS) HIPCHK(e, launch_obs(e));
        e->steps_done += 1;
        return CA_OK;
    }
    const ca_config& c = e->cfg;
    AlanArgs p;
    p.pos_x = e->pos_x; p.pos_y = e->pos_y; p.vel_x = e->vel_x; p.vel_y = e->vel_y;
    p.goal_x = e->goal_x; p.goal_y = e->goal_y; p.pref_x = e->pref_x; p.pref_y = e->pref_y; p.reward = e->reward;
    p.w = e->alan_w; p.t = e->alan_t; p.action = e->alan_action; p.dirs = e->alan_dirs; p.u = u;
    p.step_count = e->step_count; p.arena_done = e->arena_done; p.episode = e->episode; p.arena_stats = e->arena_stats;
    memcpy(p.act_c, e->act_c, sizeof p.act_c);
    memcpy(p.act_s, e->act_s, sizeof p.act_s);
    p.tab = e->alan_per ? e->d_act_tab : nullptr; p.tab_n = e->alan_per ? e->d_act_n : nullptr;
    p.temp = e->alan_temp; p.window = e->alan_window; p.dt = e->alan_dt; p.reward_scale = c.reward_scale;
    p.seed = c.seed; p.arena_offset = c.arena_offset; p.A = c.n_arenas; p.N = c.n_agents; p.nA = e->n_actions;
    p.flags = flags;
    const dim3 grid((unsigned)((AN(e) + ALAN_BS - 1) / ALAN_BS)), block(ALAN_BS);
    {
        ProfScope ps(e, KIND_RESET);
        if (e->alan_per) launch_k(ps, alan_select_kernel<2>, grid, block, (size_t)e->n_actions * ALAN_BS * 8, e->stream, p);
        else launch_k(ps, alan_select_kernel<1>, grid, block, (size_t)e->n_actions * ALAN_BS * 8, e->stream, p);
    }
    HIPCHK(e, hipGetLastError());
    StepArgs a;
    fill_args(e, a, nullptr, flags);
    HIPCHK(e, launch_step(e, a));
    {
        ProfScope ps(e, KIND_RESET);
        if (e->alan_per) launch_k(ps, alan_update_kernel<2>, grid, block, 0, e->stream, p);
        else launch_k(ps, alan_update_kernel<1>, grid, block, 0, e->stream, p);
    }
    HIPCHK(e, hipGetLastError());
    e->orient_valid = true;
    if (flags & CA_F_OBS) HIPCHK(e, launch_obs(e));
    e->steps_done += 1;
    return CA_OK;
}

int ca_alan_rollout(ca_env* e, int32_t steps, uint32_t flags) {
    if (!e || steps < 0) return fail(e, CA_EINVAL, "ca_alan_rollout: bad argument");
    if (e->ac) return fail(e, CA_EINVAL, "ca_alan_rollout: ALAN is not supported while per-arena agent counts are set");
    { const int rs = overflow_status(e, "ca_alan_rollout"); if (rs) return rs; }
    if (e->n_actions > 0 && e->alan_fused && e->quad_roll && !(flags & (CA_F_OBS | CA_F_AUTORESET | CA_F_NODONE)) && steps > 1) {
        HIPCHK(e, hipSetDevice(e->device));
        StepArgs a;
        fill_args(e, a, nullptr, flags);
        a.alan = e->d_alan;
        for (int done = 0; done < steps; done += CA_ROLLOUT_MAX_T) {
            if (e->prof_period > 1) e->profiling = (e->steps_done / (uint64_t)CA_ROLLOUT_MAX_T) % (uint64_t)e->prof_period == 0;
            a.T = steps - done < CA_ROLLOUT_MAX_T ? steps - done : CA_ROLLOUT_MAX_T;
            if (a.T == 1 && !e->quad) {
                const int rc = ca_alan_step(e, nullptr, 0, flags);
                if (rc) return rc;
                continue;
            }
            HIPCHK(e, launch_step(e, a));
            e->steps_done += (uint64_t)a.T;
        }
        e->orient_valid = true;
        return CA_OK;
    }
    for (int s = 0; s < steps; ++s) {
        const int rc = ca_alan_step(e, nullptr, 0, flags);
        if (rc) return rc;
    }
    return CA_OK;
}

int ca_observe(ca_env* e) {
    if (!e) return CA_EINVAL;
    HIPCHK(e, hipSetDevice(e->device));
    HIPCHK(e, launch_obs(e));
    return CA_OK;
}

int ca_rollout(ca_env* e, int32_t steps, uint32_t flags) {
    if (!e || steps < 0) return fail(e, CA_EINVAL, "ca_rollout: bad argument");
    HIPCHK(e, hipSetDevice(e->device));
    { const int rs = overflow_status(e, "ca_rollout"); if (rs) return rs; }
    if (e->quad_roll && !(flags & CA_F_OBS) && steps > 1) {
        StepArgs a;
        fill_args(e, a, nullptr, flags);
        for (int done = 0; done < steps; done += CA_ROLLOUT_MAX_T) {
            if (e->prof_period > 1) e->profiling = (e->steps_done / (uint64_t)CA_ROLLOUT_MAX_T) % (uint64_t)e->prof_period == 0;
            a.T = steps - done < CA_ROLLOUT_MAX_T ? steps - done : CA_ROLLOUT_MAX_T;
            HIPCHK(e, launch_step(e, a));
            e->steps_done += (uint64_t)a.T;
        }
        e->orient_valid = true;
        return CA_OK;
    }
    for (int s = 0; s < steps; ++s) {
        const int rc = do_step(e, nullptr, flags);
        if (rc) return rc;
    }
    return CA_OK;
}

int ca_sync(ca_env* e) {
    if (!e) return CA_EINVAL;
    HIPCHK(e, hipSetDevice(e->device));
    HIPCHK(e, hipStreamSynchronize(e->stream));
    return overflow_status(e, "ca_sync");
}

int ca_allow_obstacle_overflow(ca_env* e, int32_t allow) {
    if (!e) return CA_EINVAL;
    e->allow_overflow = allow != 0;
    return CA_OK;
}

int ca_get_stats(ca_env* e, ca_stats* out) {
    if (!e || !out) return fail(e, CA_EINVAL, "ca_get_stats: null argument");
    HIPCHK(e, hipSetDevice(e->device));
    const size_t A = e->cfg.n_arenas;
    std::vector<unsigned long long> h(A * ST_STRIDE);
    HIPCHK(e, hipMemcpyAsync(h.data(), e->arena_stats, h.size() * 8, hipMemcpyDeviceToHost, e->stream));
    HIPCHK(e, hipStreamSynchronize(e->stream));
    ca_stats s;
    memset(&s, 0, sizeof s);
    for (size_t a = 0; a < A; ++a) {
        const unsigned long long* r = &h[a * ST_STRIDE];
        s.episodes += r[ST_EPISODES]; s.collisions += r[ST_COLL]; s.obst_collisions += r[ST_OBST_COLL];
        s.goals_reached += r[ST_GOALS]; s.obst_overflow += r[ST_OVERFLOW];
        double d;
        memcpy(&d, &r[ST_SUMREW], 8);
        s.sum_reward += d;
    }
    std::vector<unsigned long long> hs(A);
    HIPCHK(e, hipMemcpyAsync(hs.data(), e->arena_steps, A * 8, hipMemcpyDeviceToHost, e->stream));
    HIPCHK(e, hipStreamSynchronize(e->stream));
    unsigned long long arena_steps = 0;
    for (size_t a = 0; a < A; ++a) arena_steps += hs[a] * (uint64_t)(e->ac ? e->h_counts[a] : e->cfg.n_agents);
    s.agent_steps = e->agent_steps_base + arena_steps;
    *out = s;
    return CA_OK;
}

int ca_reset_stats(ca_env* e) {
    if (!e) return CA_EINVAL;
    HIPCHK(e, hipSetDevice(e->device));
    HIPCHK(e, hipMemsetAsync(e->arena_stats, 0, (size_t)e->cfg.n_arenas * ST_STRIDE * 8, e->stream));
    HIPCHK(e, hipMemsetAsync(e->arena_steps, 0, (size_t)e->cfg.n_arenas * 8, e->stream));
    e->steps_done = 0;
    e->agent_steps_base = 0;
    if (e->ovf_host && (*(volatile unsigned long long*)e->ovf_host >> 63)) {
        HIPCHK(e, hipStreamSynchronize(e->stream));
        *(volatile unsigned long long*)e->ovf_host = 0ull;
    }
    return CA_OK;
}

int ca_debug_math(ca_env* e, int32_t op, const void* in, void* out, int32_t n) {
    if (!e || !in || !out || n <= 0 || op < 0 || op > 7) return fail(e, CA_EINVAL, "ca_debug_math: bad argument");
    static const size_t in_b[] = {4, 8, 8, 16, 16, 8, 8, 4}, out_b[] = {4, 4, 16, 16, 16, 8, 4, 4};
    HIPCHK(e, hipSetDevice(e->device));
    void *di = nullptr, *dout = nullptr;
    HIPCHK(e, hipMalloc(&di, in_b[op] * n));
    HIPCHK(e, hipMalloc(&dout, out_b[op] * n));
    HIPCHK(e, upload(e, di, in, in_b[op] * n));
    hipLaunchKernelGGL(debug_math_kernel, dim3((n + 255) / 256), dim3(256), 0, e->stream, op, di, dout, n, e->cfg.seed);
    HIPCHK(e, hipGetLastError());
    HIPCHK(e, download(e, out, dout, out_b[op] * n));
    hipFree(di);
    hipFree(dout);
    return CA_OK;
}

#ifdef CA_STAMPS
int ca_debug_set_order(ca_env* e, const int32_t* order) {
    if (!e) return CA_EINVAL;
    HIPCHK(e, hipSetDevice(e->device));
    HIPCHK(e, hipStreamSynchronize(e->stream));
    if (e->d_order) { HIPCHK(e, hipFree(e->d_order)); e->d_order = nullptr; }
    if (!order) return CA_OK;
    std::vector<char> seen((size_t)e->grid, 0);
    for (int b = 0; b < e->grid; ++b) {
        if (order[b] < 0 || order[b] >= e->grid || seen[order[b]]) return fail(e, CA_EINVAL, "ca_debug_set_order: not a permutation");
        seen[order[b]] = 1;
    }
    HIPCHK(e, hipMalloc((void**)&e->d_order, (size_t)e->grid * sizeof(int)));
    HIPCHK(e, upload(e, e->d_order, order, (size_t)e->grid * sizeof(int)));
    return CA_OK;
}

__global__ void debug_clock_kernel(unsigned long long* out) {
    const unsigned long long t0 = __builtin_amdgcn_s_memrealtime();
    __builtin_amdgcn_s_waitcnt(0xC07F);
    if (threadIdx.x == 0) out[0] = t0;
    __builtin_amdgcn_sched_barrier(0);
    const unsigned long long t1 = __builtin_amdgcn_s_memrealtime();
    __builtin_amdgcn_s_waitcnt(0xC07F);
    if (threadIdx.x == 0) out[1] = t1;
}
__global__ void debug_empty_kernel(unsigned long long* dbg, int waves_per_block) {
    extern __shared__ float4 smem4[];
    const unsigned long long t0 = __builtin_amdgcn_s_memrealtime();
    __builtin_amdgcn_s_waitcnt(0xC07F);
    if (threadIdx.x == 4096) smem4[0] = make_float4(0.f, 0.f, 0.f, 0.f);
    __builtin_amdgcn_sched_barrier(0);
    const unsigned long long t1 = __builtin_amdgcn_s_memrealtime();
    __builtin_amdgcn_s_waitcnt(0xC07F);
    if ((threadIdx.x & 63) == 0) {
        unsigned long long* r = dbg + ((size_t)blockIdx.x * waves_per_block + (threadIdx.x >> 6)) * 16;
        r[12] = t0; r[11] = t1;
    }
}
static unsigned long long* g_dbg_clock = nullptr;
int ca_debug_clock(ca_env* e, int32_t slot) {
    if (!e || slot < 0 || slot >= 64) return fail(e, CA_EINVAL, "ca_debug_clock: bad argument");
    HIPCHK(e, hipSetDevice(e->device));
    if (!g_dbg_clock) HIPCHK(e, hipMalloc((void**)&g_dbg_clock, 64 * 2 * 8));
    hipLaunchKernelGGL(debug_clock_kernel, dim3(1), dim3(64), 0, e->stream, g_dbg_clock + 2 * slot);
    return CA_OK;
}
int ca_debug_clock_read(ca_env* e, unsigned long long* out, int32_t n_slots) {
    if (!e || !g_dbg_clock || n_slots > 64) return fail(e, CA_EINVAL, "ca_debug_clock_read: bad argument");
    HIPCHK(e, download(e, out, g_dbg_clock, (size_t)n_slots * 2 * 8));
    return CA_OK;
}
int ca_debug_empty(ca_env* e) {
    if (!e || !e->dbg) return fail(e, CA_EINVAL, "ca_debug_empty: not a CA_STAMPS build");
    HIPCHK(e, hipSetDevice(e->device));
    ProfScope ps(e, KIND_RESET);
    launch_k(ps, debug_empty_kernel, dim3(e->grid), dim3(e->BS), (size_t)e->lds, e->stream, e->dbg, e->BS / 64);
    return CA_OK;
}

int ca_debug_stamps(ca_env* e, unsigned long long* out, int32_t max_waves, int32_t* n_waves) {
    if (!e || !e->dbg) return fail(e, CA_EINVAL, "ca_debug_stamps: not a CA_STAMPS build");
    const bool obs = max_waves < 0;
    if (obs) max_waves = -max_waves;
    const int nw = obs ? e->cfg.n_arenas * ((e->cfg.n_agents + 15) / 16) * 4 : (e->quad ? e->grid_q * (e->BSq / 64) : e->grid * ((e->pair ? 2 : 1) * e->BS / 64));
    if (n_waves) *n_waves = nw;
    const int n = nw < max_waves ? nw : max_waves;
    HIPCHK(e, hipSetDevice(e->device));
    HIPCHK(e, download(e, out, obs ? e->dbg_obs : e->dbg, (size_t)n * 16 * 8));
    return CA_OK;
}
#endif

int ca_host_alloc(ca_env* e, size_t bytes, void** out) {
    if (!e || !out || bytes == 0) return fail(e, CA_EINVAL, "ca_host_alloc: bad argument");
    *out = nullptr;
    HIPCHK(e, hipSetDevice(e->device));
    void* p = nullptr;
    HIPCHK(e, hipHostMalloc(&p, bytes, hipHostMallocDefault));
    e->host_allocs.push_back({p, bytes});
    *out = p;
    return CA_OK;
}
int ca_host_free(ca_env* e, void* p) {
    if (!e || !p) return fail(e, CA_EINVAL, "ca_host_free: bad argument");
    for (size_t k = 0; k < e->host_allocs.size(); ++k)
        if (e->host_allocs[k].first == p) {
            e->host_allocs.erase(e->host_allocs.begin() + k);
            HIPCHK(e, hipHostFree(p));
            return CA_OK;
        }
    return fail(e, CA_EINVAL, "ca_host_free: not a buffer of this handle");
}

int ca_profile(ca_env* e, int32_t period) {
    if (!e || period < 0) return fail(e, CA_EINVAL, "ca_profile: bad argument");
    e->prof_period = period;
    e->profiling = period == 1;
    if (period > 0) {
        HIPCHK(e, hipSetDevice(e->device));
        while (e->free_events.size() < 256) {
            hipEvent_t ev = nullptr;
            if (hipEventCreate(&ev) != hipSuccess) break;
            e->free_events.push_back(ev);
        }
    }
    return CA_OK;
}

int ca_profile_read(ca_env* e, int32_t counts[4], float mean_ms[4]) {
    if (!e || !counts || !mean_ms) return fail(e, CA_EINVAL, "ca_profile_read: null argument");
    HIPCHK(e, hipSetDevice(e->device));
    HIPCHK(e, hipStreamSynchronize(e->stream));
    double sum[4] = {0, 0, 0, 0};
    for (int k = 0; k < 4; ++k) counts[k] = 0;
    for (const ca_env::Span& sp : e->spans) {
        float ms = 0.0f;
        if (hipEventElapsedTime(&ms, sp.t0, sp.t1) == hipSuccess) { sum[sp.kind] += ms / (sp.steps > 0 ? sp.steps : 1); counts[sp.kind] += 1; }
        e->free_events.push_back(sp.t0);
        e->free_events.push_back(sp.t1);
    }
    e->spans.clear();
    for (int k = 0; k < 4; ++k) mean_ms[k] = counts[k] ? (float)(sum[k] / counts[k]) : 0.0f;
    return CA_OK;
}

int ca_launch_info(ca_env* e, int32_t* block, int32_t* grid, int32_t* lds_bytes, int32_t* obs_grid) {
    if (!e) return CA_EINVAL;
    const SolveLaunch s = solve_launch(e, false, false);
    if (block) *block = (int32_t)s.block.x;
    if (grid) *grid = (int32_t)s.grid.x;
    if (lds_bytes) *lds_bytes = (int32_t)s.lds;
    if (obs_grid) {
        const int apb = obs_block_threads(e->cfg.n_agents) / 16;
        *obs_grid = obs_dense(e) ? (int32_t)(((size_t)e->cfg.n_arenas * e->cfg.n_agents + apb - 1) / apb)
                                 : (int32_t)((size_t)e->cfg.n_arenas * ((e->cfg.n_agents + apb - 1) / apb));
    }
    return CA_OK;
}

#ifndef CA_SRC_SHA
#define CA_SRC_SHA "unknown"
#endif
const char* ca_source_sha(void) { return CA_SRC_SHA; }

int ca_solver_info(ca_env* e, int32_t* lanes_per_agent, int32_t* rollout_one_launch) {
    if (!e) return CA_EINVAL;
    if (lanes_per_agent) *lanes_per_agent = e->quad ? 4 : (e->pair ? 2 : 1);
    if (rollout_one_launch) *rollout_one_launch = e->quad_roll ? 1 : 0;
    return CA_OK;
}

int ca_tiled_info(ca_env* e, int32_t* tiled, int32_t* tile_agents, int32_t* tiles_per_arena, int32_t* launches_per_step) {
    if (!e) return CA_EINVAL;
    if (tiled) *tiled = e->tiled ? 1 : 0;
    if (tile_agents) *tile_agents = e->tiled ? e->TILE : 0;
    if (tiles_per_arena) *tiles_per_arena = e->tiled ? e->tiles : 0;
    if (launches_per_step) *launches_per_step = e->tiled ? 3 : 0;
    return CA_OK;
}

}
```

### collision_avoidance_amd/csrc/ca_obs.h

```cpp
#pragma once
#include "ca_common.h"

namespace ca {

struct ObsArgs {
    const float *pos_x, *pos_y, *vel_x, *vel_y, *orient_x, *orient_y;
    const unsigned short* counts;
    const void* nb_idx;
    const unsigned short* obst_idx;
    const ObstDev* obst;
    const int* tab_off;
    float* obs;
    int A, N, K, S, bpa;
    int nstage_max;
    int paircap;
    int a0;
    int xcd;
    int dense;
    unsigned long long* dbg;
    float radius;
    float rays[32];
    float oct[32];
    const float* ap_oct;
    const int* agent_counts;
};

#ifdef CA_STAMPS
#define CA_OSTAMP(k)                                                                       \
    do {                                                                                   \
        __builtin_amdgcn_sched_barrier(0);                                                 \
        const unsigned long long _t = CA_STAMP_CLOCK();                                    \
        __builtin_amdgcn_s_waitcnt(0xC07F);                                                \
        if ((threadIdx.x & 63) == 0 && p.dbg)                                              \
            p.dbg[((size_t)blockIdx.x * (blockDim.x >> 6) + (threadIdx.x >> 6)) * 16 + (k)] = _t; \
        __builtin_amdgcn_sched_barrier(0);                                                 \
    } while (0)
#else
#define CA_OSTAMP(k) do { } while (0)
#endif

__host__ __device__ inline size_t obs_lds_bytes(int nstage_max, int obs_bs, int paircap, int obw = 16) {
    const size_t apb = obs_bs / 16;
    return (size_t)nstage_max * 16 + 2 * apb * 16 * 8 + apb * 16 + apb * 16 * 4 + apb * (size_t)obw * 4 + 64 * 4 + 2 * apb * 4 + apb * (size_t)paircap * 2;
}
__host__ __device__ inline size_t obs_lds_bytes_ap(int nstage_max, int obs_bs, int paircap) {
    return ((obs_lds_bytes(nstage_max, obs_bs, paircap) + 15) & ~(size_t)15) + (size_t)(obs_bs / 16) * 16 * 64;
}
#ifndef CA_OBS_BS_MAX
#define CA_OBS_BS_MAX 256
#endif
__host__ __device__ inline int obs_block_threads(int N) {
    const int want = N > 32 ? 1024 : (N > 16 ? 512 : 256);
    return want < CA_OBS_BS_MAX ? want : CA_OBS_BS_MAX;
}

struct SegGeom {
    float s02x, s02y;
    float s32x, s32y;
    float t_numer;
    float r1x, r1y, r2x, r2y;
};

__device__ __forceinline__ float ray_dial(float x, float y) {
    const float yy = -y;
    const float ax = fabsf(x), ay = fabsf(yy);
    const float mx = fmaxf(ax, ay), mn = fminf(ax, ay);
    const float a = mn * __builtin_amdgcn_rcpf(mx);
    const float s = a * a;
    float r = a * (0.99997726f + s * (-0.33262347f + s * (0.19354346f + s * (-0.11643287f +
              s * (0.05265332f + s * -0.01172120f)))));
    r = (ay > ax) ? 1.57079632679f - r : r;
    r = (x < 0.0f) ? 3.14159265359f - r : r;
    r = (yy < 0.0f) ? -r : r;
    const float u = r * 2.54647908947f;
    return (u < 0.0f) ? u + 16.0f : u;
}

template <int OBS_BS, bool NW16, bool DENSE = false, class... WIDE_TAG>
__global__ __launch_bounds__(OBS_BS) void obs_kernel(const ObsArgs p) {
    constexpr bool WIDE = has_tag<WideObstLists, WIDE_TAG...>;
    constexpr bool AC = has_tag<ArenaCounts, WIDE_TAG...>;
    constexpr bool AP = has_tag<AgentParams, WIDE_TAG...> || AC;
    static_assert(!(WIDE && AP), "per-agent parameters go with obstacle lists of up to 16");
    constexpr int OBS_APB = OBS_BS / 16;
    extern __shared__ float4 smem4[];
    const int tid = threadIdx.x;
    const int g = tid >> 4, r = tid & 15;
    const int N = p.N, K = p.K, S = p.S;
    const int PAIRCAP = p.paircap;
    int bid = blockIdx.x;
    if (p.xcd) { const int x = bid & 7, idx = bid >> 3, q8 = idx / p.bpa; bid = (x + 8 * q8) * p.bpa + (idx - q8 * p.bpa); }
    int a, i, a_lo, nstage;
    bool active;
    if constexpr (DENSE) {
        const int first = bid * OBS_APB, gi = first + g;
        active = gi < p.A * N;
        const int ga = active ? gi : p.A * N - 1;
        a = p.a0 + ga / N; i = ga - (ga / N) * N;
        a_lo = p.a0 + first / N;
        const int last = min(first + OBS_APB - 1, p.A * N - 1);
        nstage = (last / N - first / N + 1) * N;
    } else {
        const int ab = bid / p.bpa;
        a = p.a0 + ab;
        i = (bid - ab * p.bpa) * OBS_APB + g;
        active = i < N;
        a_lo = a; nstage = N;
    }
    const int abase = DENSE ? (a - a_lo) * N : 0;
    const size_t q = (size_t)a * N + (active ? i : 0);
    const size_t aoff = (size_t)a * N;
    const unsigned ii = active ? (unsigned)i : 0u;
    const ObstDev* tab = p.obst + (p.tab_off ? p.tab_off[a] : 0);

    const int NST = p.nstage_max;
    float* s_px = reinterpret_cast<float*>(smem4);
    float* s_py = s_px + NST;
    float* s_vx = s_py + NST;
    float* s_vy = s_vx + NST;
    unsigned long long* s_key = reinterpret_cast<unsigned long long*>(s_vy + NST);
    float2* s_rel = reinterpret_cast<float2*>(s_key + OBS_APB * 16);
    float4* s_frame = reinterpret_cast<float4*>(s_rel + OBS_APB * 16);
    int* s_nb = reinterpret_cast<int*>(s_frame + OBS_APB);
    int* s_ob = s_nb + OBS_APB * 16;
    const int OBW = WIDE ? S : 16;
    float* s_rays = reinterpret_cast<float*>(s_ob + OBS_APB * OBW);
    float* s_oct = s_rays + 32;
    int* s_cnt = reinterpret_cast<int*>(s_oct + 32);
    int* s_cnt2 = s_cnt + OBS_APB;
    unsigned short* s_pair = reinterpret_cast<unsigned short*>(s_cnt2 + OBS_APB);
    const int SPAIRS = 16 * S;
    float2* s_noct = reinterpret_cast<float2*>(reinterpret_cast<char*>(smem4) + ((obs_lds_bytes(NST, OBS_BS, PAIRCAP) + 15) & ~(size_t)15));
    CA_OSTAMP(0);
    if (tid < 32) { s_rays[tid] = p.rays[tid]; s_oct[tid] = p.oct[tid]; }

    constexpr bool GATHER = NW16;
    const float* gpx = p.pos_x + (size_t)a * N;
    const float* gpy = p.pos_y + (size_t)a * N;
    const float* gvx = p.vel_x + (size_t)a * N;
    const float* gvy = p.vel_y + (size_t)a * N;
    if constexpr (!GATHER) {
        if constexpr (DENSE) {
            for (int t = tid; t < nstage; t += OBS_BS) {
                const size_t qa = (size_t)a_lo * N + t;
                s_px[t] = p.pos_x[qa]; s_py[t] = p.pos_y[qa]; s_vx[t] = p.vel_x[qa]; s_vy[t] = p.vel_y[qa];
            }
        } else {
            for (unsigned t = tid; t < (unsigned)nstage; t += OBS_BS) {
                s_px[t] = (p.pos_x + aoff)[t]; s_py[t] = (p.pos_y + aoff)[t]; s_vx[t] = (p.vel_x + aoff)[t]; s_vy[t] = (p.vel_y + aoff)[t];
            }
        }
    }
    int nn = 0, ns = 0;
    float c = 1.0f, s = 0.0f;
    if (active) {
        if constexpr (DENSE) {
            const int cnts = p.counts[q];
            nn = cnts & 0xFF; ns = cnts >> 8;
            if constexpr (AC) { if (i >= p.agent_counts[a]) { nn = 0; ns = 0; } }
            c = p.orient_x[q]; s = -p.orient_y[q];
            if (r < nn) s_nb[g * 16 + r] = abase + ld_idx_t<NW16>(p.nb_idx, ((size_t)a * K + r) * N + i);
            if constexpr (WIDE) { for (int t = r; t < ns; t += 16) s_ob[g * OBW + t] = (int)p.obst_idx[((size_t)a * S + t) * N + i]; }
            else if (r < ns) s_ob[g * 16 + r] = (int)p.obst_idx[((size_t)a * S + r) * N + i];
        } else {
            const int cnts = (p.counts + aoff)[ii];
            nn = cnts & 0xFF; ns = cnts >> 8;
            if constexpr (AC) { if (i >= p.agent_counts[a]) { nn = 0; ns = 0; } }
            c = (p.orient_x + aoff)[ii]; s = -(p.orient_y + aoff)[ii];
            const unsigned li = (unsigned)r * (unsigned)N + ii;
            const char* nbase = (const char*)p.nb_idx + aoff * (size_t)K * (NW16 ? 2 : 1);
            if (r < nn) s_nb[g * 16 + r] = ld_idx_t<NW16>(nbase, li);
            if constexpr (WIDE) { for (unsigned t = (unsigned)r; t < (unsigned)ns; t += 16u) s_ob[g * OBW + t] = (int)(p.obst_idx + aoff * (size_t)S)[t * (unsigned)N + ii]; }
            else if (r < ns) s_ob[g * 16 + r] = (int)(p.obst_idx + aoff * (size_t)S)[li];
        }
    }
    s_key[g * 16 + r] = ~0ull;
    if (r == 0) { s_cnt[g] = 0; s_cnt2[g] = 0; }
    CA_OSTAMP(1);
    __syncthreads();
    CA_OSTAMP(2);

    const int M = 8 * nn + ns;
    float mx = 0.0f, my = 0.0f;
    if (M > 0) { mx = GATHER ? gpx[i] : s_px[abase + i]; my = GATHER ? gpy[i] : s_py[abase + i]; }
    if (r == 0) s_frame[g] = make_float4(c, s, mx, my);
    {
        const int k = r;
        int i0 = 0, w = 0;
        if (k < nn) {
            const int nb = s_nb[g * 16 + k];
            const float rx = (GATHER ? gpx[nb] : s_px[nb]) - mx, ry = (GATHER ? gpy[nb] : s_py[nb]) - my;
            s_rel[g * 16 + k] = make_float2(rx, ry);
            float Rk = p.radius;
            if constexpr (AP) {
                const size_t nq = (DENSE ? (size_t)a_lo * N : aoff) + (size_t)nb;
                const float2* src = reinterpret_cast<const float2*>(p.ap_oct) + nq * 8;
                float2* dst = s_noct + (g * 16 + k) * 8;
#pragma unroll
                for (int e = 0; e < 8; ++e) dst[e] = src[e];
                Rk = src[0].x;
            }
            const float d2 = rx * rx + ry * ry, R = Rk;
            const float ax = c * rx - s * ry, ay = s * rx + c * ry;
            const bool all = !(d2 > 1.0404f * R * R);
            const float ua = ray_dial(ax, ay);
            const float t = R * __builtin_amdgcn_rsqf(d2);
            const float t2 = t * t;
            const float hw = t * (1.0f + t2 * (0.16666667f + t2 * (0.075f + t2 * 0.32914f))) * 2.54647908947f + 0.002f;
            int i1 = (int)floorf(ua + hw);
            i0 = (int)ceilf(ua - hw);
            if (all || i1 - i0 >= 15) { i0 = 0; i1 = 15; }
            w = max(i1 - i0 + 1, 0);
        }
        const int incl = wave_prefix_sum(w);
        int base = 0;
        if ((tid & 63) == 63) base = atomicAdd(&s_cnt[0], incl);
        base = __builtin_amdgcn_readlane(base, 63) + (incl - w);
        const unsigned short hd = (unsigned short)((g << 8) | (k << 4));
#pragma unroll
        for (int t2 = 0; t2 < 4; ++t2)
            if (t2 < w) s_pair[base + t2] = (unsigned short)(hd | ((i0 + t2) & 15));
        if (__builtin_expect(__ballot(w > 4) != 0ull, 0)) {
#pragma clang loop vectorize(disable) unroll(disable)
            for (int t2 = 4; t2 < w; ++t2) s_pair[base + t2] = (unsigned short)(hd | ((i0 + t2) & 15));
        }
    }
    {
        const float dx = s_rays[2 * r], dy = s_rays[2 * r + 1];
        int cnt2 = 0;
        for (int sidx = 0; sidx < ns; ++sidx) {
            const ObstDev o1 = load_obst(tab, s_ob[g * OBW + sidx]);
            const float x1 = o1.px - mx, y1 = o1.py - my, x2 = o1.qx - mx, y2 = o1.qy - my;
            const float ax = c * x1 - s * y1, ay = s * x1 + c * y1;
            const float bx = c * x2 - s * y2, by = s * x2 + c * y2;
            const float c2 = dx * ay - dy * ax, c3 = dx * by - dy * bx;
            const float f2 = dx * ax + dy * ay, f3 = dx * bx + dy * by;
            const float tolE = 1e-5f * p.rays[0] * (fabsf(ax) + fabsf(ay) + fabsf(bx) + fabsf(by) + 1.0f);
            const bool keep = !(c2 > tolE && c3 > tolE) && !(c2 < -tolE && c3 < -tolE) && (fmaxf(f2, f3) >= -tolE);
            const unsigned grp = (unsigned)(__ballot(keep) >> (threadIdx.x & 48)) & 0xFFFFu;
            if (keep)
                s_pair[OBS_APB * PAIRCAP - 1 - (g * SPAIRS + cnt2 + __popc(grp & ((1u << r) - 1u)))] =
                    (unsigned short)(((nn + sidx) << 4) | r);
            cnt2 += __popc(grp);
        }
        if (r == 0) s_cnt2[g] = cnt2;
    }
    CA_OSTAMP(3);
    __syncthreads();
    CA_OSTAMP(4);
    auto build = [&](int m, SegGeom& sg, float& velx, float& vely, bool want_vel) {
        float x1, y1, x2, y2, vx = 0.0f, vy = 0.0f;
        if (m < 8 * nn) {
            const int k = m >> 3, e = m & 7;
            const float2 rel = s_rel[g * 16 + k];
            const float rx = rel.x, ry = rel.y;
            if constexpr (AP) {
                const float2 va = s_noct[(g * 16 + k) * 8 + e], vb = s_noct[(g * 16 + k) * 8 + ((e + 1) & 7)];
                x1 = va.x + rx; y1 = va.y + ry;
                x2 = vb.x + rx; y2 = vb.y + ry;
            } else {
                const float4 oc = reinterpret_cast<const float4*>(s_oct)[e];
                x1 = oc.x + rx; y1 = oc.y + ry;
                x2 = oc.z + rx; y2 = oc.w + ry;
            }
            if (want_vel) { const int nb = s_nb[g * 16 + k]; vx = GATHER ? gvx[nb] : s_vx[nb]; vy = GATHER ? gvy[nb] : s_vy[nb]; }
        } else {
            const ObstDev o1 = load_obst(tab, s_ob[g * OBW + (m - 8 * nn)]);
            x1 = o1.px - mx; y1 = o1.py - my;
            x2 = o1.qx - mx; y2 = o1.qy - my;
        }
        sg.r1x = c * x1 - s * y1; sg.r1y = s * x1 + c * y1;
        sg.r2x = c * x2 - s * y2; sg.r2y = s * x2 + c * y2;
        sg.s32x = sg.r2x - sg.r1x; sg.s32y = sg.r2y - sg.r1y;
        sg.s02x = 0.0f - sg.r1x; sg.s02y = 0.0f - sg.r1y;
        sg.t_numer = sg.s32x * sg.s02y - sg.s32y * sg.s02x;
        if (want_vel) {
            const float lvx = x1 + vx, lvy = y1 + vy;
            const float rvx = c * lvx - s * lvy, rvy = s * lvx + c * lvy;
            velx = rvx - sg.r1x; vely = rvy - sg.r1y;
        }
    };
    auto build_nb = [&](const float2& fr, float rx, float ry, int e, SegGeom& sg, int slot) {
        float x1, y1, x2, y2;
        if constexpr (AP) {
            const float2 va = s_noct[slot * 8 + e], vb = s_noct[slot * 8 + ((e + 1) & 7)];
            x1 = va.x + rx; y1 = va.y + ry; x2 = vb.x + rx; y2 = vb.y + ry;
        } else {
            const float4 oc = reinterpret_cast<const float4*>(s_oct)[e];
            x1 = oc.x + rx; y1 = oc.y + ry; x2 = oc.z + rx; y2 = oc.w + ry;
        }
        sg.r1x = fr.x * x1 - fr.y * y1; sg.r1y = fr.y * x1 + fr.x * y1;
        sg.r2x = fr.x * x2 - fr.y * y2; sg.r2y = fr.y * x2 + fr.x * y2;
        sg.s32x = sg.r2x - sg.r1x; sg.s32y = sg.r2y - sg.r1y;
        sg.s02x = 0.0f - sg.r1x; sg.s02y = 0.0f - sg.r1y;
        sg.t_numer = sg.s32x * sg.s02y - sg.s32y * sg.s02x;
    };
    auto hit = [&](const SegGeom& sg, float s10x, float s10y, float& d, float& hx, float& hy) -> bool {
        const float denom = s10x * sg.s32y - sg.s32x * s10y;
        if (denom == 0.0f) return false;
        const bool dpos = denom > 0.0f;
        const float s_numer = s10x * sg.s02y - s10y * sg.s02x;
        if ((s_numer < 0.0f) == dpos) return false;
        if ((sg.t_numer < 0.0f) == dpos) return false;
        if (((s_numer > denom) == dpos) || ((sg.t_numer > denom) == dpos)) return false;
        const float t = div_ir(sg.t_numer, denom);
        hx = 0.0f + t * s10x; hy = 0.0f + t * s10y;
        d = sqrt_ir(hx * hx + hy * hy);
        return true;
    };

    auto accept_nb = [&](const SegGeom& sg, float s10x, float s10y, float& denom) -> bool {
        denom = s10x * sg.s32y - sg.s32x * s10y;
        const float s_numer = s10x * sg.s02y - s10y * sg.s02x;
        const bool dpos = denom > 0.0f;
        return (denom != 0.0f) && ((s_numer < 0.0f) != dpos) && ((sg.t_numer < 0.0f) != dpos) &&
               ((s_numer > denom) != dpos) && ((sg.t_numer > denom) != dpos);
    };
    auto hit_dist = [&](float t_numer, float denom, float s10x, float s10y) -> float {
        const float t = div_ir(t_numer, denom);
        const float hx = 0.0f + t * s10x, hy = 0.0f + t * s10y;
        return sqrt_ir(hx * hx + hy * hy);
    };

    const float tol_u = 2e-5f * p.rays[0] * (p.rays[0] + 2.0f * p.radius + 1.0f);
    auto merge = [&](int ga, int ray, float best, int best_m) {
        if (best_m >= 0)
            atomicMin(&s_key[ga * 16 + ray], ((unsigned long long)__float_as_uint(best) << 32) | (unsigned)best_m);
    };
    const int ntot = s_cnt[0];
    for (int pi = tid; pi < ntot; pi += OBS_BS) {
        const int pr = s_pair[pi];
        const int ga = pr >> 8, k = (pr >> 4) & 15, ray = pr & 15;
        const float2 fr = *reinterpret_cast<const float2*>(&s_frame[ga]);
        const float2 rel = s_rel[pr >> 4];
        const float s10x = s_rays[2 * ray] - 0.0f, s10y = s_rays[2 * ray + 1] - 0.0f;
        float best = __int_as_float(0x7f800000);
        int best_m = -1;
        const float rx = rel.x, ry = rel.y;
        const float wx = fr.x * s10x + fr.y * s10y, wy = fr.x * s10y - fr.y * s10x;
        const float wb = wx * ry - wy * rx;
        float Rp = p.radius, tol = tol_u;
        if constexpr (AP) {
            Rp = s_noct[(pr >> 4) * 8].x;
            tol = 2e-5f * p.rays[0] * (p.rays[0] + 2.0f * Rp + 1.0f);
        }
        const float R = Rp, Rh = 0.70710678f * R;
        const float c0 = R * wy, c2 = R * wx, c1 = Rh * (wx + wy), c3 = Rh * (wy - wx);
        const float cr[8] = {wb - c0, wb - c1, wb - c2, wb + c3, wb + c0, wb + c1, wb + c2, wb - c3};
        unsigned acc = 0;
#pragma unroll
        for (int e = 0; e < 8; ++e) {
            const float ca = cr[e], cb = cr[(e + 1) & 7];
            const bool same_side = (ca > tol && cb > tol) || (ca < -tol && cb < -tol);
            acc |= same_side ? 0u : (1u << e);
        }
        while (acc) {
            const int e1 = __ffs(acc) - 1;
            acc &= acc - 1;
            const bool two = acc != 0;
            const int e2 = two ? __ffs(acc) - 1 : e1;
            acc &= acc - 1;
            SegGeom g1, g2;
            build_nb(fr, rx, ry, e1, g1, pr >> 4);
            build_nb(fr, rx, ry, e2, g2, pr >> 4);
            float dn1, dn2;
            const bool ok1 = accept_nb(g1, s10x, s10y, dn1), ok2 = accept_nb(g2, s10x, s10y, dn2) && two;
            const float lhs = fabsf(g1.t_numer) * fabsf(dn2), rhs = fabsf(g2.t_numer) * fabsf(dn1);
            const bool first = ok1 && (!ok2 || lhs < rhs);
            const float tnw = first ? g1.t_numer : g2.t_numer, dnw = first ? dn1 : dn2;
            const int ew = first ? e1 : e2;
            const bool sure = fminf(lhs, rhs) < 0.99999f * fmaxf(lhs, rhs) && fmaxf(lhs, rhs) > 1e-30f &&
                              fabsf(tnw) > 1e-12f * fabsf(dnw);
            if (ok1 && ok2 && !sure) {
                const float d1 = hit_dist(g1.t_numer, dn1, s10x, s10y), d2 = hit_dist(g2.t_numer, dn2, s10x, s10y);
                if (d1 < best) { best = d1; best_m = 8 * k + e1; }
                if (d2 < best) { best = d2; best_m = 8 * k + e2; }
            } else {
                const float dw = hit_dist(tnw, dnw, s10x, s10y);
                if ((ok1 || ok2) && dw < best) { best = dw; best_m = 8 * k + ew; }
            }
        }
        merge(ga, ray, best, best_m);
    }
    const int no = s_cnt2[g];
    for (int pi = r; pi < no; pi += 16) {
        const int pr = s_pair[OBS_APB * PAIRCAP - 1 - (g * SPAIRS + pi)];
        const int k = pr >> 4, ray = pr & 15;
        const float s10x = s_rays[2 * ray] - 0.0f, s10y = s_rays[2 * ray + 1] - 0.0f;
        SegGeom sg;
        float dum0, dum1, d, hx, hy;
        const int m = 8 * nn + (k - nn);
        build(m, sg, dum0, dum1, false);
        if (hit(sg, s10x, s10y, d, hx, hy)) merge(g, ray, d, m);
    }
    CA_OSTAMP(5);
    __syncthreads();
    CA_OSTAMP(6);
    if (!active) return;
    const unsigned long long key = s_key[g * 16 + r];
    float bx = 0.0f, by = 0.0f, vx = 0.0f, vy = 0.0f;
    if (key != ~0ull) {
        SegGeom sg;
        float wx, wy;
        build((int)(unsigned)key, sg, wx, wy, true);
        const float s10x = s_rays[2 * r] - 0.0f, s10y = s_rays[2 * r + 1] - 0.0f;
        const float t = div_ir(sg.t_numer, s10x * sg.s32y - sg.s32x * s10y);
        bx = 0.0f + t * s10x; by = 0.0f + t * s10y;
        if (!(bx == 0.0f && by == 0.0f)) { vx = wx; vy = wy; }
    }
    CA_OSTAMP(7);
    {
        typedef float v4f __attribute__((ext_vector_type(4)));
        const v4f out = {bx, by, vx, vy};
        if constexpr (DENSE) __builtin_nontemporal_store(out, reinterpret_cast<v4f*>(p.obs) + (q * 16 + r));
        else __builtin_nontemporal_store(out, (reinterpret_cast<v4f*>(p.obs) + aoff * 16) + (ii * 16u + (unsigned)r));
    }
    CA_OSTAMP(8);
}

}
```

### collision_avoidance_amd/csrc/ca_step.h

```cpp
#pragma once
#include "ca_lp.h"
#include "ca_lines.h"
#include "ca_nbr.h"
#include "ca_rules.h"

namespace ca {

__host__ __device__ inline size_t step_lds_bytes(int BS, int K, int S, int ST = 0, int KMAX = 0) {
    if (ST > 0) return (size_t)(BS / 64) * (2 * (ST + KMAX)) * POOL_SLOTS * 16 + (size_t)BS * 32;
    return (size_t)BS * ((size_t)(K + S) * 16 + 16 + 16);
}
__host__ __device__ inline size_t step_lds_bytes_ap(int BS, int K, int S) { return step_lds_bytes(BS, K, S) + (size_t)BS * 4; }



#define CA_AS(n) __attribute__((address_space(n)))
template <bool NW16, int TS>
__device__ __noinline__ void solve_many_obstacles(CA_AS(3) char* tbl3, int MLX, const CA_AS(1) char* tab1, const CA_AS(1) char* oidx1,
                                                 const CA_AS(1) char* nidx1, int stride, int ocnt, int ncnt, const CA_AS(3) char* arena3, int bs,
                                                 V2 pos, V2 vel, V2 pref, float R, float invTO, float invT, float invDt, float max_speed) {
    float4* tbl = (float4*)tbl3;
    const ObstDev* tab = (const ObstDev*)tab1;
    const unsigned short* oidx = (const unsigned short*)oidx1;
    const void* nidx = (const void*)nidx1;
    const float* arena = (const float*)arena3;
    const float *ax = arena, *ay = arena + bs, *avx = arena + 2 * bs, *avy = arena + 3 * bs;
    LdsLines ls; ls.base = tbl; ls.stride = TS;
    int nl = 0;
    for (int s = 0; s < ocnt; ++s) {
        const int e = ld_idx_t<true>(oidx, (size_t)s * (size_t)stride);
        Line line;
        auto covered = [&](V2 c1, V2 c2) {
            for (int j = 0; j < nl; ++j) {
                const Line M = ls.get(j);
                if (det(c1 - M.point, M.dir) - invTO * R >= -EPS && det(c2 - M.point, M.dir) - invTO * R >= -EPS) return true;
            }
            return false;
        };
        if (obst_orca_line(tab, e, pos, vel, R, invTO, covered, line)) { ls.put(nl, line); ++nl; }
    }
    const int numObst = nl;
    for (int k = 0; k < ncnt; ++k) {
        const int j = ld_idx_t<NW16>(nidx, (size_t)k * (size_t)stride);
        ls.put(nl, agent_orca_line(pos, vel, mk(ax[j], ay[j]), mk(avx[j], avy[j]), R, invT, invDt));
        ++nl;
    }
    V2 nv = mk(0.0f, 0.0f);
    const int fail = lp2(ls, nl, max_speed, pref, false, nv);
    tbl[(2 * MLX - 1) * TS] = make_float4(nv.x, nv.y, __int_as_float(nl | (numObst << 8) | (fail << 16)), 0.0f);
}

#ifndef CA_LB512
#define CA_LB512 4
#endif
template <int KMAX, int BS, int ST, int SMX = (ST > 0 ? ST : SMAX), bool ALAN = false, class... PER>
__global__ __launch_bounds__(BS, ST > 0 ? (BS == 512 ? CA_LB512 : 4) : 1) void step_kernel(const StepArgs p) {
    constexpr int AM = !ALAN ? 0 : (has_tag<AlanArenaSets, PER...> ? 2 : 1);
    constexpr bool AC = has_tag<ArenaCounts, PER...>;
    constexpr bool AP = has_tag<AgentParams, PER...> || AC;
    static_assert(!AP || (ST == 0 && !ALAN && SMX <= SMAX), "per-agent parameters: the LDS line table with lists of up to 16, no ALAN form");
    extern __shared__ float4 smem4[];
    constexpr bool LISTP = BS > 64 && !AP;
    __shared__ unsigned s_vmax2;
    if constexpr (LISTP) { if (threadIdx.x == 0) s_vmax2 = 0u; }
    CA_PRIO_START();
    nbr_body<KMAX, BS, SMX, AP, AC>(p);
    constexpr int ML = ST + KMAX;
    const int tid = threadIdx.x;
    const int P = p.P;
    int la, i;
    lane_slot(p, tid, la, i);
    const int apb = p.apb;
    const int a = p.a0 + work_block(p) * apb + la;
    const bool frozen = arena_frozen(p, a);
    int n_a = p.N;
    if constexpr (AC) n_a = ((a < p.a1) && (la < apb)) ? p.cold->agent_counts[a] : 0;
    const bool active = (a < p.a1) && (i < n_a) && (la < apb) && !frozen;
    if (frozen && i == 0) p.arena_stats[(size_t)a * ST_STRIDE + ST_FROZEN] += 1;
    const int N = p.N, K = p.K, S = p.S;
    const int q = active ? a * N + i : 0;
    const int lbase = tid - i;

    float4* s_lines = smem4;
    float* s_px = reinterpret_cast<float*>(
        smem4 + (ST > 0 ? (size_t)(BS / 64) * (2 * ML) * POOL_SLOTS : (size_t)(K + S) * BS));
    float* s_py = s_px + BS;
    float* s_vx = s_py + BS;
    float* s_vy = s_vx + BS;
    int* s_misc = reinterpret_cast<int*>(s_vy + BS);
    float* s_rad = reinterpret_cast<float*>(s_misc + 4 * BS);
    LdsLines ls; ls.base = s_lines + tid; ls.stride = BS;

    CA_STAMP(0);
    V2 pos = mk(0.0f, 0.0f), vel = mk(0.0f, 0.0f), pref = mk(0.0f, 0.0f);
    V2 pf32 = mk(1.0f, 0.0f);
    if (active) {
        pos = mk(p.pos_x[q], p.pos_y[q]);
        vel = mk(p.vel_x[q], p.vel_y[q]);
        if (p.actions) {
            action_pref(pos, p.goal_x[q], p.goal_y[q], p.actions[q], pf32, pref);
        } else if constexpr (ALAN) {
            const AlanK& al = *(AlanK*)p.alan;
            const int nA = al.nA, nk = alan_count<AM>(al, a);
            constexpr int PSTR = ST > 0 ? 64 : BS;
            double* ps = ST > 0 ? reinterpret_cast<double*>(s_lines + (size_t)(tid >> 6) * (2 * ML) * POOL_SLOTS) + (tid & 63)
                                : reinterpret_cast<double*>(s_lines) + tid;
            const double* w = al.w + (size_t)a * nA * N + i;
            auto psk = [&](int k) -> double& { return ps[k * PSTR]; };
            alan_terms(nk, 0, 1, psk, [&](int k) { return w[(size_t)k * N]; }, al.temp);
            const StepCold* cp = p.cold;
            const int act_id = alan_draw(nk, psk, [&] { return alan_uniform(p.alan_u, q, cp->seed, cp->arena_offset, a, i, cp->episode[a], cp->step_count[a]); });
            double dgx, dgy, dlx, dly;
            alan_dirs<AM>(al, a, act_id, pos, p.goal_x[q], p.goal_y[q], &dgx, &dgy, &dlx, &dly);
            pref = mk((float)dlx, (float)dly);
            pf32 = mk(__int_as_float(act_id), 0.0f);
        } else {
            pref = mk(p.pref_x[q], p.pref_y[q]);
        }
    }
    float r_own = p.radius, ms = p.max_speed, th = p.time_horizon, tho = p.time_horizon_obst;
    if constexpr (AP) {
        if (active) {
            const StepCold* cp = p.cold;
            r_own = cp->ap_radius[q]; ms = cp->ap_max_speed[q]; th = cp->ap_time_horizon[q]; tho = cp->ap_time_horizon_obst[q];
        }
        s_rad[tid] = r_own;
    }
    s_px[tid] = pos.x; s_py[tid] = pos.y; s_vx[tid] = vel.x; s_vy[tid] = vel.y;
    reinterpret_cast<float*>(s_misc)[tid * 4 + 0] = pf32.x; reinterpret_cast<float*>(s_misc)[tid * 4 + 1] = pf32.y;
    constexpr bool PARK_PREF = ST > 0 && (BS > 64 || SMX > ST);
    if constexpr (PARK_PREF) { reinterpret_cast<float*>(s_misc)[tid * 4 + 2] = pref.x; reinterpret_cast<float*>(s_misc)[tid * 4 + 3] = pref.y; }
    __syncthreads();

    CA_STAMP(1);
    CA_PRIO_POINT(1);
    const void* nb_idx_s = p.nb_idx;
    const unsigned short* obst_idx_s = p.obst_idx;
    asm volatile("" : "+s"(nb_idx_s), "+s"(obst_idx_s));
    const int cnts = active ? (int)p.counts[q] : 0;
    const int ocnt = cnts >> 8, ncnt = cnts & 0xFF;
    const ObstDev* tab = p.obst + ((p.tab_off != nullptr && active) ? p.tab_off[a] : 0);
#if defined(CA_STAMPS) && CA_STAMPS == 3
    CA_STAMP_HWID();
#else
    CA_STAMP(2);
    CA_STAMP(3);
#endif
    const float R = AP ? r_own : p.radius;
    V2 nv = mk(0.0f, 0.0f);
    if constexpr (ST > 0) {
        float4 L[ML];
        static_for<ML>([&](auto kc) __attribute__((always_inline)) { L[decltype(kc)::value] = make_float4(0.0f, 0.0f, 1.0f, 0.0f); });
        int no = 0;
        const bool many = (SMX > ST) && active && ocnt > ST;
        const bool fast = active && !many;
        {
            const float invTO = 1.0f / p.time_horizon_obst;
            int e_next = (fast && ocnt > 0) ? ld_idx_t<true>(obst_idx_s, ((size_t)a * S + 0) * N + i) : 0;
            const int s_end = S < ST ? S : ST;
            for (int s = 0; s < s_end; ++s) {
                if (fast && s < ocnt) {
                    const int e = e_next;
                    if (s + 1 < ocnt) e_next = ld_idx_t<true>(obst_idx_s, ((size_t)a * S + (s + 1)) * N + i);
                    auto covered = [&](V2 c1, V2 c2) __attribute__((always_inline)) {
                        bool c = false;
                        static_for<ST>([&](auto jc) __attribute__((always_inline)) {
                            constexpr int j = decltype(jc)::value;
                            const Line M = unpack_line(L[j]);
                            if (j < no && det(c1 - M.point, M.dir) - invTO * R >= -EPS &&
                                det(c2 - M.point, M.dir) - invTO * R >= -EPS)
                                c = true;
                        });
                        return c;
                    };
                    Line line;
                    if (obst_orca_line(tab, e, pos, vel, R, invTO, covered, line)) {
                        const float4 pl = pack_line(line);
                        static_for<ST>([&](auto jc) __attribute__((always_inline)) {
                            constexpr int j = decltype(jc)::value;
                            if (j == no) L[j] = pl;
                        });
                        ++no;
                    }
                }
            }
        }
#if defined(CA_STAMPS) && CA_STAMPS == 3
        if ((tid & 63) == 0 && p.dbg) p.dbg[((size_t)blockIdx.x * (BS / 64) + (tid >> 6)) * 16 + 4] = 0;
#else
        CA_STAMP(4);
#endif
        CA_PRIO_POINT(2);
        {
            const float invT = 1.0f / p.time_horizon;
            const float invDt = 1.0f / p.time_step;
            int jn[KMAX];
            static_for<KMAX>([&](auto kc) __attribute__((always_inline)) {
                constexpr int k = decltype(kc)::value;
                jn[k] = (k < ncnt) ? ld_idx_t<CA_NBW16(BS)>(nb_idx_s, ((size_t)a * K + k) * N + i) : 0;
            });
            static_for<KMAX>([&](auto kc) __attribute__((always_inline)) {
                constexpr int k = decltype(kc)::value;
                if (k < ncnt) {
                    const int j = lbase + jn[k];
                    L[ST + k] = pack_line(agent_orca_line(pos, vel, mk(s_px[j], s_py[j]), mk(s_vx[j], s_vy[j]), R, invT, invDt));
                }
            });
        }
        CA_STAMP(5);
        CA_PRIO_POINT(3);
        const int nl = no + ncnt;
        int fail = nl;
        auto opt_fn = [&]() __attribute__((always_inline)) -> V2 {
// ... 143 lines not shown
    asm volatile("" : "+v"(tid_e));
    const StepCold* cold_e = p.cold;
    asm volatile("" : "+s"(cold_e));
    {
    const ColdK& c = *(ColdK*)cold_e;
    const int tid = tid_e;
    int la, i;
    lane_slot(p, tid, la, i);
    const int a = p.a0 + work_block(p) * apb + la;
    const int q = active ? a * N + i : 0;
    const int lbase = tid - i;
    int NA = N;
    if constexpr (AC) NA = active ? c.agent_counts[a] : 1;
    const ObstDev* tab = p.obst + ((p.tab_off != nullptr && active) ? p.tab_off[a] : 0);
    pf32 = mk(reinterpret_cast<float*>(s_misc)[tid * 4 + 0], reinterpret_cast<float*>(s_misc)[tid * 4 + 1]);
    if constexpr (PARK_PREF) pref = mk(reinterpret_cast<float*>(s_misc)[tid * 4 + 2], reinterpret_cast<float*>(s_misc)[tid * 4 + 3]);
    float rew_alan = 0.0f;
    if constexpr (ALAN) {
        const AlanK& al = *(AlanK*)p.alan;
        if (active) {
            const int act_id = __float_as_int(pf32.x), nA = al.nA, nk = alan_count<AM>(al, a);
            double dgx, dgy, dlx, dly;
            alan_dirs<AM>(al, a, act_id, mk(s_px[tid], s_py[tid]), c.goal_x[q], c.goal_y[q], &dgx, &dgy, &dlx, &dly);
            rew_alan = step_reward(al.reward_scale, vel, mk((float)dgx, (float)dgy), mk((float)dlx, (float)dly));
            al.reward[q] = rew_alan;
            double* w = al.w + (size_t)a * nA * N + i;
            double* t = al.t + (size_t)a * nA * N + i;
            alan_update(al, vel, dgx, dgy, dlx, dly, act_id, nk, 0, 1, [&](int k) -> double& { return w[(size_t)k * N]; },
                        [&](int k) -> double& { return t[(size_t)k * N]; });
            al.action[q] = act_id;
            c.pref_x[q] = (float)dlx; c.pref_y[q] = (float)dly;
        }
    }

    if constexpr (LISTP) {
        const unsigned sp = wave_max_u32(active ? __float_as_uint(absSq(vel)) : 0u);
        if ((tid & 63) == 63) atomicMax(&s_vmax2, sp);
    }
    __syncthreads();
    float2* s_xy2 = reinterpret_cast<float2*>(s_px);
    if constexpr (LISTP || AP) { s_px[tid] = pos.x; s_py[tid] = pos.y; }
    else if (i < p.N && la < apb) { s_xy2[2 * lbase + i] = make_float2(pos.x, pos.y); s_xy2[2 * lbase + i + p.N] = make_float2(pos.x, pos.y); }
    s_misc[tid * 4 + 0] = 0; s_misc[tid * 4 + 1] = 0; s_misc[tid * 4 + 2] = 0; s_misc[tid * 4 + 3] = 0;
    __syncthreads();
    int* red = s_misc + la * 4;

    if (p.flags & 2u) {
        int pairs = 0;
        const float crSq = sqr(R + R);
        float m2 = 0.0f;
        if constexpr (LISTP) m2 = 2.0002f * __builtin_sqrtf(__uint_as_float(s_vmax2)) * p.time_step;
        bool scan_all = active && !(LISTP && p.neighbor_dist >= R + R + m2);
        if constexpr (LISTP) if (active && !scan_all) {
            float far2 = 0.0f;
            const int ncnt = (int)(p.counts[q] & 0xFFu);
            int jn[KMAX];
            static_for<KMAX>([&](auto kc) __attribute__((always_inline)) {
                constexpr int k = decltype(kc)::value;
                jn[k] = (k < ncnt) ? ld_idx_t<CA_NBW16(BS)>(p.nb_idx, ((size_t)a * K + k) * N + i) : 0;
            });
            static_for<KMAX>([&](auto kc) __attribute__((always_inline)) {
                constexpr int k = decltype(kc)::value;
                if (k < ncnt) {
                    const int j = jn[k];
                    const float d2 = absSq(pos - mk(s_px[lbase + j], s_py[lbase + j]));
                    far2 = d2 > far2 ? d2 : far2;
                    if (j > i && d2 < crSq) ++pairs;
                }
            });
            scan_all = (ncnt == K) && !(far2 > sqr(R + R + 2.0f * m2));
        }
        if constexpr (AP) {
            if (active) {
                const int N = NA;
                const int H = (N - 1) >> 1;
                auto near = [&](int d) __attribute__((always_inline)) {
                    int j = i + d;
                    j = j >= N ? j - N : j;
                    return absSq(pos - mk(s_px[lbase + j], s_py[lbase + j])) < sqr(R + s_rad[lbase + j]) ? 1 : 0;
                };
                for (int d = 1; d <= H; ++d) pairs += near(d);
                if (!(N & 1) && N > 1) { const int h = N >> 1; if (i < h) pairs += near(h); }
            }
        } else if constexpr (LISTP) {
            if (__ballot(scan_all) != 0ull && scan_all) {
                pairs = 0;
                for (int j = i + 1; j < N; ++j)
                    if (absSq(pos - mk(s_px[lbase + j], s_py[lbase + j])) < crSq) ++pairs;
            }
        } else {
            const float2* xs = s_xy2 + (active ? 2 * lbase + i : 0);
            const int H = (N - 1) >> 1;
            auto near = [&](int d) __attribute__((always_inline)) { const float2 o = xs[d]; return absSq(pos - mk(o.x, o.y)) < crSq ? 1 : 0; };
            int d = 1;
            for (; d + 3 <= H; d += 4) pairs += near(d) + near(d + 1) + near(d + 2) + near(d + 3);
            for (; d <= H; ++d) pairs += near(d);
            if (!(N & 1) && N > 1) { const int h = N >> 1; if (i < h) pairs += near(h); }
        }
        if (active) {
            if (pairs) atomicAdd(&red[1], pairs);
            const bool wall = p.tab_off == nullptr ? touches_wall(p.obst, p.n_obst, pos, R) : touches_wall(tab, p.tab_off[a + 1] - p.tab_off[a], pos, R);
            if (wall) atomicAdd(&red[2], 1);
        }
    }

    CA_STAMP(8);
    CA_PRIO_POINT(7);
    float rew = 0.0f;
    double gx = 0.0, gy = 0.0;
    if (active) {
        gx = c.goal_x[q]; gy = c.goal_y[q];
        if (p.actions) {
            rew = step_reward(c.reward_scale, vel, pf32, pref);
            c.reward[q] = rew;
        } else {
            pref = goal_dir(pos, gx, gy);
        }
    }

    CA_STAMP(9);
    const bool nodone = (p.flags & 8u) != 0;
    bool goal_changed = false;
    int done = active ? c.agent_done[q] : 1;
    int steps = active ? c.step_count[a] : 0;
    if (!p.actions && !nodone) ++steps;
    if (active && !nodone && goal_hit(c, pos, gx, gy, AP ? R : p.radius, done)) {
        if (c.done_mode == 2) {
            const int rc = c.regoal_count[q];
            regoal_draw(c, a, i, rc, &gx, &gy);
            c.regoal_count[q] = rc + 1;
        } else {
            done = 1;
            c.arrive_step[q] = steps;
            arrival_goal(c, q, &gx, &gy);
            c.agent_done[q] = 1;
        }
        c.goal_x[q] = gx; c.goal_y[q] = gy;
        goal_changed = true;
        atomicAdd(&red[3], 1);
    }
    if (p.actions) ++steps;
    if (active && done == 0) atomicAdd(&red[0], 1);
    __syncthreads();

    const bool all_done = active && episode_over(c, nodone, red[0], steps);
    const bool do_reset = all_done && (p.flags & 4u);
    int epi = 0;
    if (do_reset) {
        epi = c.episode[a];
        pos = spawn_draw(c, a, i, epi);
        done = 0;
        c.agent_done[q] = 0;
        pref = goal_dir(pos, gx, gy);
    }
    if ((p.actions || ALAN) && (p.flags & 2u)) {
        double r = active ? (double)(ALAN ? rew_alan : rew) : 0.0;
        const int w = P < 64 ? P : 64;
        for (int off = w >> 1; off > 0; off >>= 1) { const double t = __shfl_down(r, off, 64); if (!p.dense || i + off < N) r += t; }
        if (active && (i & 63) == 0)
            atomicAdd(reinterpret_cast<double*>(&c.arena_stats[(size_t)a * ST_STRIDE + ST_SUMREW]), r);
    }
    const V2 o = obs_frame(pref, active && !do_reset && (p.actions != nullptr || goal_changed), pos, gx, gy);
    const float ox = o.x, oy = o.y;
    CA_STAMP(10);
    __syncthreads();
    if (active) {
#if defined(CA_NT_STATE)
        __builtin_nontemporal_store(ox, &c.orient_x[q]); __builtin_nontemporal_store(oy, &c.orient_y[q]);
        __builtin_nontemporal_store(pos.x, &c.pos_x[q]); __builtin_nontemporal_store(pos.y, &c.pos_y[q]);
        __builtin_nontemporal_store(vel.x, &c.vel_x[q]); __builtin_nontemporal_store(vel.y, &c.vel_y[q]);
        if constexpr (!ALAN) { __builtin_nontemporal_store(pref.x, &c.pref_x[q]); __builtin_nontemporal_store(pref.y, &c.pref_y[q]); }
#else
        c.orient_x[q] = ox; c.orient_y[q] = oy;
        c.pos_x[q] = pos.x; c.pos_y[q] = pos.y;
        c.vel_x[q] = vel.x; c.vel_y[q] = vel.y;
        if constexpr (!ALAN) { c.pref_x[q] = pref.x; c.pref_y[q] = pref.y; }
#endif
        if (i == 0) {
            flush_stats(c.arena_stats + (size_t)a * ST_STRIDE, red[1], red[2], red[3], all_done ? 1u : 0u, all_done, lastep_word(steps, NA, red[0]));
            c.arena_done[a] = all_done ? 1 : 0;
            c.step_count[a] = do_reset ? 0 : steps;
            atomicAdd(&c.arena_steps[a], 1ull);
            if (do_reset) c.episode[a] = epi + 1;
        }
    }
    }
    CA_STAMP(11);
}

template <bool AC>
__device__ __forceinline__ void reset_body(const StepArgs& p) {
    const ColdK& c = *(ColdK*)p.cold;
    const int q = blockIdx.x * blockDim.x + threadIdx.x;
    if (q >= p.A * p.N) return;
    const int a = q / p.N, i = q - a * p.N;
    if (p.reset_mask && p.reset_mask[a] == 0) return;
    if constexpr (AC) { if (i >= c.agent_counts[a]) return; }
    V2 pos;
    if (p.reset_px) {
        pos = mk(p.reset_px[q], p.reset_py[q]);
    } else {
        pos = spawn_draw(c, a, i, c.episode[a]);
    }
    const V2 d = goal_dir(pos, c.goal_x[q], c.goal_y[q]);
    c.pos_x[q] = pos.x; c.pos_y[q] = pos.y;
    c.pref_x[q] = d.x; c.pref_y[q] = d.y;
    c.orient_x[q] = d.x; c.orient_y[q] = d.y;
    c.agent_done[q] = 0;
}
__global__ void reset_kernel(const StepArgs p) { reset_body<false>(p); }
__global__ void reset_counts_kernel(const StepArgs p) { reset_body<true>(p); }
__global__ void orient_kernel(const StepArgs p) {
    const ColdK& c = *(ColdK*)p.cold;
    const int q = blockIdx.x * blockDim.x + threadIdx.x;
    if (q >= p.A * p.N) return;
    double dx, dy;
    pref_dir64(c.pos_x[q], c.pos_y[q], c.goal_x[q], c.goal_y[q], &dx, &dy);
    c.orient_x[q] = (float)dx; c.orient_y[q] = (float)dy;
}
__global__ void reset_arena_kernel(const StepArgs p) {
    const ColdK& c = *(ColdK*)p.cold;
    const int a = blockIdx.x * blockDim.x + threadIdx.x;
    if (a >= p.A) return;
    if (p.reset_mask && p.reset_mask[a] == 0) return;
    c.step_count[a] = 0;
    c.arena_done[a] = 0;
    c.episode[a] += 1;
}

}
```

### collision_avoidance_amd/vec_env.py

```python
import ctypes as C

import numpy as np

from . import _lib, scenarios

try:
    import torch
except Exception:
    torch = None

_I32_FIELDS = {_lib.FLD_AGENT_DONE, _lib.FLD_ARRIVE_STEP, _lib.FLD_NB_COUNT, _lib.FLD_NB_IDX,
               _lib.FLD_OBST_COUNT, _lib.FLD_OBST_IDX, _lib.FLD_STEP_COUNT, _lib.FLD_ARENA_DONE,
               _lib.FLD_EPISODE, _lib.FLD_REGOAL_COUNT, _lib.FLD_ALAN_ACTION}
_ARENA_FIELDS = {_lib.FLD_STEP_COUNT, _lib.FLD_ARENA_DONE, _lib.FLD_EPISODE}
DEFAULT_MAX_OBST_NEIGHBORS = 16
_F64_FIELDS = {_lib.FLD_GOAL_X, _lib.FLD_GOAL_Y, _lib.FLD_GOAL2_X, _lib.FLD_GOAL2_Y, _lib.FLD_ALAN_WEIGHTS,
               _lib.FLD_ALAN_TIMES}


def _ptr(a):
    return a.ctypes.data_as(C.c_void_p)


class VecCollisionAvoidanceEnv:
# ... 113 lines not shown
        return out

    def host_array(self, shape, dtype):
        n = int(np.prod(shape)) * np.dtype(dtype).itemsize
        ptr = C.c_void_p()
        self._call("ca_host_alloc", self.h, max(n, 1), C.byref(ptr))
        buf = (C.c_char * max(n, 1)).from_address(ptr.value)
        arr = np.frombuffer(buf, dtype=dtype, count=int(np.prod(shape))).reshape(shape)
        self.__dict__.setdefault("_host_arrays", []).append(arr)
        return arr

    def host_buffer(self, field):
        bufs = self.__dict__.setdefault("_host_bufs", {})
        if field not in bufs:
            shape, dt = self._shape_dtype(field)
            bufs[field] = self.host_array(shape, dt)
        return bufs[field]

    def step_packed(self, actions=None, with_obs=True, stats=False, autoreset=False, no_done=False):
        an, A = self.A * self.N, self.A
        if "_packed" not in self.__dict__:
            words = an * _lib.OBS_DIM + an + 2 * A
            raw = self.host_array((words,), np.float32)
            self._packed = (raw, raw[:an * _lib.OBS_DIM].reshape(A, self.N, _lib.OBS_DIM), raw[an * _lib.OBS_DIM:an * _lib.OBS_DIM + an].reshape(A, self.N),
                            raw[an * _lib.OBS_DIM + an:an * _lib.OBS_DIM + an + A].view(np.int32), raw[an * _lib.OBS_DIM + an + A:].view(np.int32))
            self._packed_act = self.host_array((A, self.N), np.float32)
        raw, obs, rew, done, steps = self._packed
        flags = (_lib.F_OBS if with_obs else 0) | (_lib.F_STATS if stats else 0) | (_lib.F_AUTORESET if autoreset else 0) | \
                (_lib.F_NODONE if no_done else 0)
        act_ptr = None
        if actions is not None:
            if torch is not None and isinstance(actions, torch.Tensor):
                actions = actions.detach().cpu().numpy()
            self._packed_act[...] = np.asarray(actions, np.float32).reshape(A, self.N)
            act_ptr = self._packed_act.ctypes.data
        self._call("ca_step_packed", self.h, act_ptr, flags, raw.ctypes.data, raw.nbytes)
        return obs, rew, done, steps

    def set(self, field, arr):
        shape, dt = self._shape_dtype(field)
        if field in (_lib.FLD_ALAN_WEIGHTS, _lib.FLD_ALAN_TIMES):
            arr = np.transpose(np.asarray(arr, dt).reshape(self.A, self.N, self.n_actions), (0, 2, 1))
        a = np.ascontiguousarray(np.asarray(arr, dt).reshape(shape))
        self._call("ca_set", self.h, field, _ptr(a), a.nbytes, 0)

    _STATE_FIELDS = ("POS_X", "POS_Y", "VEL_X", "VEL_Y", "PREF_X", "PREF_Y", "GOAL_X", "GOAL_Y", "GOAL2_X", "GOAL2_Y",
                     "AGENT_DONE", "ARRIVE_STEP", "NB_COUNT", "NB_IDX", "OBST_COUNT", "OBST_IDX", "STEP_COUNT", "ARENA_DONE",
                     "EPISODE", "REGOAL_COUNT", "REWARD")

    def get_state(self):
        st = {name: self.get(getattr(_lib, "FLD_" + name)) for name in self._STATE_FIELDS}
        if self.n_actions > 0:
            st["ALAN_WEIGHTS"] = self.get(_lib.FLD_ALAN_WEIGHTS)
            st["ALAN_TIMES"] = self.get(_lib.FLD_ALAN_TIMES)
            st["ALAN_ACTION"] = self.get(_lib.FLD_ALAN_ACTION)
        st["_shape"] = np.array([self.A, self.N, self.K, self.S, self.n_actions], np.int64)
        return st

    def set_state(self, st):
        shape = [int(v) for v in np.asarray(st["_shape"]).reshape(-1)]
        if shape != [self.A, self.N, self.K, self.S, self.n_actions]:
            raise ValueError("set_state: the state is of an environment of shape %s, this one is %s"
                             % (shape, [self.A, self.N, self.K, self.S, self.n_actions]))
        optional = ("REWARD", "ALAN_ACTION")
        need = [n for n in self._STATE_FIELDS if n not in optional] + (["ALAN_WEIGHTS", "ALAN_TIMES"] if self.n_actions > 0 else [])
        missing = [n for n in need if n not in st]
        if missing:
            raise KeyError("set_state: the snapshot lacks %s" % ", ".join(missing))
        for name in self._STATE_FIELDS:
            if name in st:
                self.set(getattr(_lib, "FLD_" + name), st[name])
        if self.n_actions > 0:
            self.set(_lib.FLD_ALAN_WEIGHTS, st["ALAN_WEIGHTS"])
            self.set(_lib.FLD_ALAN_TIMES, st["ALAN_TIMES"])
            if "ALAN_ACTION" in st:
                self.set(_lib.FLD_ALAN_ACTION, st["ALAN_ACTION"])

    def field_tensor(self, field):
        if torch is None:
            raise RuntimeError("field_tensor needs PyTorch")
        shape, dt = self._shape_dtype(field)
        ptr, nbytes = C.c_void_p(), C.c_size_t()
        self._call("ca_field_ptr", self.h, field, C.byref(ptr), C.byref(nbytes))

        class _View(object):
            pass
        v = _View()
        v.__cuda_array_interface__ = {"shape": tuple(shape), "typestr": np.dtype(dt).str, "data": (int(ptr.value), False),
                                      "version": 2, "strides": None}
        t = torch.as_tensor(v, device=torch.device("cuda", self.device))
        assert t.numel() * t.element_size() == nbytes.value
        return t

    def neighbor_lists(self):
        return self.get(_lib.FLD_NB_COUNT), np.transpose(self.get(_lib.FLD_NB_IDX), (0, 2, 1))[:, :, :self.K]

    def obstacle_neighbor_lists(self):
        return self.get(_lib.FLD_OBST_COUNT), np.transpose(self.get(_lib.FLD_OBST_IDX), (0, 2, 1))

    def set_obstacles(self, polys):
        polys = [np.asarray(q, np.float32).reshape(-1, 2) for q in polys]
        verts = np.ascontiguousarray(np.concatenate(polys) if polys else np.zeros((0, 2), np.float32))
        sizes = np.asarray([len(q) for q in polys], np.int32)
        self._call("ca_set_obstacles", self.h, _ptr(verts), _ptr(sizes), len(polys))

    def set_obstacles_per_arena(self, worlds):
        if len(worlds) != self.A:
            raise ValueError("set_obstacles_per_arena: %d worlds for %d arenas" % (len(worlds), self.A))
        polys = [np.asarray(q, np.float32).reshape(-1, 2) for w in worlds for q in w]
        verts = np.ascontiguousarray(np.concatenate(polys) if polys else np.zeros((0, 2), np.float32))
        sizes = np.asarray([len(q) for q in polys], np.int32)
        counts = np.asarray([len(w) for w in worlds], np.int32)
        self._call("ca_set_obstacles_per_arena", self.h, _ptr(verts), _ptr(sizes), _ptr(counts))

    def obstacle_table(self, arena=0):
        n = C.c_int32()
        self._call("ca_get_obstacles_arena", self.h, int(arena), None, None, None, 0, C.byref(n))
        verts, nxt, cvx = np.zeros((n.value, 2), np.float32), np.zeros(n.value, np.int32), np.zeros(n.value, np.int32)
        self._call("ca_get_obstacles_arena", self.h, int(arena), _ptr(verts), _ptr(nxt), _ptr(cvx), n.value, C.byref(n))
        return dict(verts=verts, next=nxt, convex=cvx)

    def init_scenario(self, scenario):
        sid = scenarios.SCENARIO_IDS[scenario] if isinstance(scenario, str) else int(scenario)
        self._call("ca_init_scenario", self.h, sid)

    def sync(self):
        self._call("ca_sync", self.h)

    def stats(self):
        s = _lib.Stats()
        self._call("ca_get_stats", self.h, C.byref(s))
        return s.as_dict()

    def reset_stats(self):
        self._call("ca_reset_stats", self.h)

    def profile(self, period=1):
        self._call("ca_profile", self.h, int(period))

    def profile_read(self):
        n = (C.c_int32 * 4)()
        ms = (C.c_float * 4)()
        self._call("ca_profile_read", self.h, n, ms)
        return {k: (n[i], ms[i]) for i, k in enumerate(("nbr_kernel", "step_kernel", "obs_kernel", "reset_kernels"))}

    def launch_info(self):
        v = [C.c_int32() for _ in range(4)]
        self._call("ca_launch_info", self.h, *[C.byref(x) for x in v])
        lanes, roll = C.c_int32(), C.c_int32()
        self._call("ca_solver_info", self.h, C.byref(lanes), C.byref(roll))
        per, cnt = C.c_int32(), C.c_int32()
        self._call("ca_agent_params_info", self.h, C.byref(per))
        self._call("ca_agent_counts_info", self.h, C.byref(cnt))
        return dict(block=v[0].value, grid=v[1].value, lds_bytes=v[2].value, obs_grid=v[3].value,
                    lanes_per_agent=lanes.value, rollout_one_launch=roll.value, agent_params=bool(per.value),
                    agent_counts=bool(cnt.value))

    def tiled_info(self):
        v = [C.c_int32() for _ in range(4)]
        self._call("ca_tiled_info", self.h, *[C.byref(x) for x in v])
        return dict(tiled=bool(v[0].value), tile_agents=v[1].value, tiles_per_arena=v[2].value, launches_per_step=v[3].value)

    _AGENT_PARAMS = ("radius", "max_speed", "time_horizon", "time_horizon_obst")

    def set_agent_params(self, radius=None, max_speed=None, time_horizon=None, time_horizon_obst=None):
        keep, ptrs = [], []
        for name, v in zip(self._AGENT_PARAMS, (radius, max_speed, time_horizon, time_horizon_obst)):
            if v is None:
                ptrs.append(None)
                continue
            if torch is not None and isinstance(v, torch.Tensor):
                v = v.detach().cpu().numpy()
            a = np.asarray(v, np.float32)
            if a.ndim == 1 and a.shape[0] == self.A:
                a = a[:, None]
            try:
                full = np.ascontiguousarray(np.broadcast_to(a, (self.A, self.N)), np.float32)
            except ValueError:
                raise ValueError("set_agent_params: %s must be a scalar, an [A] array or an [A,N] array (A=%d, N=%d), got shape %s"
                                 % (name, self.A, self.N, a.shape))
            keep.append(full)
            ptrs.append(_ptr(full))
        self._call("ca_set_agent_params", self.h, ptrs[0], ptrs[1], ptrs[2], ptrs[3], self.A * self.N * 4, 0)

    def clear_agent_params(self):
        self._call("ca_set_agent_params", self.h, None, None, None, None, 0, 0)

    def agent_params(self):
        out = {k: np.empty((self.A, self.N), np.float32) for k in self._AGENT_PARAMS}
        self._call("ca_get_agent_params", self.h, *[_ptr(out[k]) for k in self._AGENT_PARAMS], self.A * self.N * 4, 0)
        return out

    def set_agent_counts(self, counts):
        if torch is not None and isinstance(counts, torch.Tensor):
            counts = counts.detach().cpu().numpy()
        c = np.asarray(counts)
        if c.shape != (self.A,) or c.dtype.kind not in "iu":
            raise ValueError("set_agent_counts: counts must be an [A] integer array (A=%d), got shape %s, dtype %s" % (self.A, c.shape, c.dtype))
        c = np.ascontiguousarray(np.clip(c, -2 ** 31, 2 ** 31 - 1), np.int32)
        self._call("ca_set_agent_counts", self.h, _ptr(c), c.nbytes, 0)

    def clear_agent_counts(self):
        self._call("ca_set_agent_counts", self.h, None, 0, 0)

    def agent_counts(self):
        out = np.empty(self.A, np.int32)
        self._call("ca_get_agent_counts", self.h, _ptr(out), out.nbytes, 0)
        return out

    def agent_mask(self):
        return np.arange(self.N)[None, :] < self.agent_counts()[:, None]

    def _on_device(self, t, dtype):
        if not t.is_cuda:
            return t.detach().to(dtype=dtype).contiguous().numpy(), False
        dev = torch.device("cuda", self.device)
        t = t.detach().to(device=dev, dtype=dtype).contiguous()
        if not self.use_torch:
            torch.cuda.current_stream(self.device).synchronize()
        return t, True

    def _obs_out(self):
        return self._obs_t if self.use_torch else self.get(_lib.FLD_OBS)

    def reset(self, pos_x=None, pos_y=None, with_obs=True):
        flags = _lib.F_OBS if with_obs else 0
        if pos_x is None:
            self._call("ca_reset", self.h, None, None, 0, flags)
        elif torch is not None and isinstance(pos_x, torch.Tensor) and pos_x.is_cuda and \
                isinstance(pos_y, torch.Tensor) and pos_y.is_cuda:
            px, _ = self._on_device(pos_x, torch.float32)
            py, _ = self._on_device(pos_y, torch.float32)
            if px.numel() != self.A * self.N or py.numel() != self.A * self.N:
                raise ValueError("reset: pos_x / pos_y must hold %d x %d values" % (self.A, self.N))
            self._call("ca_reset", self.h, C.c_void_p(px.data_ptr()), C.c_void_p(py.data_ptr()), 1, flags)
            self.sync()
        else:
            if torch is not None and isinstance(pos_x, torch.Tensor):
                pos_x = pos_x.detach().cpu().numpy()
            if torch is not None and isinstance(pos_y, torch.Tensor):
                pos_y = pos_y.detach().cpu().numpy()
            px = np.ascontiguousarray(np.asarray(pos_x, np.float32).reshape(self.A, self.N))
            py = np.ascontiguousarray(np.asarray(pos_y, np.float32).reshape(self.A, self.N))
            self._call("ca_reset", self.h, _ptr(px), _ptr(py), 0, flags)
        return self._obs_out() if with_obs else None

    def reset_masked(self, mask, with_obs=True):
        flags = _lib.F_OBS if with_obs else 0
        on_dev = False
        if torch is not None and isinstance(mask, torch.Tensor):
            mask, on_dev = self._on_device(mask, torch.int32)
        if on_dev:
            if mask.numel() != self.A:
                raise ValueError("reset_masked: mask must hold %d values" % self.A)
            self._call("ca_reset_masked", self.h, C.c_void_p(mask.data_ptr()), 1, flags)
            self.sync()
        else:
            m = np.ascontiguousarray(np.asarray(mask, np.int32).reshape(self.A))
            self._call("ca_reset_masked", self.h, _ptr(m), 0, flags)
        return self._obs_out() if with_obs else None

    def arena_stats(self):
        r = self.get(_lib.FLD_ARENA_STATS)
        return dict(episodes=r[:, 0], collisions=r[:, 1], obst_collisions=r[:, 2], goals_reached=r[:, 3],
                    obst_overflow=r[:, 4], sum_reward=r[:, 5].copy().view(np.float64), frozen_steps=r[:, 6],
                    last_episode_steps=(r[:, 7] >> np.uint64(32)).astype(np.int64),
                    last_episode_arrived=(r[:, 7] & np.uint64(0xFFFFFFFF)).astype(np.int64))

    def step(self, actions, with_obs=True, stats=False, autoreset=False, copy=True):
        flags = (_lib.F_OBS if with_obs else 0) | (_lib.F_STATS if stats else 0) | \
                (_lib.F_AUTORESET if autoreset else 0)
        if self.use_torch:
            if not isinstance(actions, torch.Tensor):
                actions = torch.as_tensor(np.asarray(actions, np.float32).reshape(self.A, self.N))
            if actions.is_cuda and actions.dtype == torch.float32 and actions.is_contiguous() and \
                    actions.numel() == self.A * self.N and actions.device.index == self.device:
                src = actions
            else:
                self._act_t.copy_(actions.reshape(self.A, self.N), non_blocking=True)
                src = self._act_t
            self._call("ca_step", self.h, C.c_void_p(src.data_ptr()), flags)
            return (self._obs_t if with_obs else None), self._rew_t, self._done_t, {}
        a = np.ascontiguousarray(np.asarray(actions, np.float32).reshape(self.A, self.N))
        self._call("ca_step_host", self.h, _ptr(a), flags)
        if not copy:
            return (self.get(_lib.FLD_OBS, self.host_buffer(_lib.FLD_OBS)) if with_obs else None), \
                self.get(_lib.FLD_REWARD, self.host_buffer(_lib.FLD_REWARD)), \
                self.get(_lib.FLD_ARENA_DONE, self.host_buffer(_lib.FLD_ARENA_DONE)), {}
        return (self.get(_lib.FLD_OBS) if with_obs else None), self.get(_lib.FLD_REWARD), \
            self.get(_lib.FLD_ARENA_DONE), {}

    def orca_step(self, with_obs=False, stats=False, no_done=False, autoreset=False, freeze=False):
        flags = (_lib.F_OBS if with_obs else 0) | (_lib.F_STATS if stats else 0) | \
                (_lib.F_NODONE if no_done else 0) | (_lib.F_AUTORESET if autoreset else 0) | \
                (_lib.F_FREEZE if freeze else 0)
        self._call("ca_orca_step", self.h, flags)
        return self._obs_out() if with_obs else None

    def observe(self):
        self._call("ca_observe", self.h)
        return self._obs_out()

    def rollout(self, steps, with_obs=False, stats=False, autoreset=False, freeze=False):
        flags = (_lib.F_OBS if with_obs else 0) | (_lib.F_STATS if stats else 0) | \
                (_lib.F_AUTORESET if autoreset else 0) | (_lib.F_FREEZE if freeze else 0)
        self._call("ca_rollout", self.h, int(steps), flags)

    def alan_configure(self, actions, temp=0.2, timewindow=2.0, time_step=1 / 60.):
        a = np.ascontiguousarray(np.asarray(actions, np.float64).reshape(-1, 2))
# ... 47 lines not shown
```

### include/ca_env.h

```cpp
#ifndef CA_ENV_H
#define CA_ENV_H

#include <stddef.h>
#include <stdint.h>

#ifdef __cplusplus
extern "C" {
#endif

#define CA_OBS_DIM 64
#define CA_N_RAYS 16
#define CA_MAX_NEIGHBORS 16
#define CA_MAX_OBST_NEIGHBORS 64
#define CA_MAX_AGENTS 1024
#define CA_MAX_AGENTS_LARGE 16384

#define CA_CREATE_TILED 1u

#define CA_OK 0
#define CA_EINVAL (-1)
#define CA_ENODEV (-2)
#define CA_EHIP (-3)
#define CA_ESIZE (-4)
#define CA_ERANGE (-5)

#define CA_DONE_XLESS 0
#define CA_DONE_GOAL 1
#define CA_DONE_REGOAL 2

#define CA_F_OBS 1u
#define CA_F_STATS 2u
#define CA_F_AUTORESET 4u
#define CA_F_NODONE 8u
#define CA_F_FREEZE 16u
#define CA_ALAN_MAX_ACTIONS 32

#define CA_SCN_CROWD 0
#define CA_SCN_CIRCLE 1
#define CA_SCN_DOORWAY 2
#define CA_SCN_CONGESTED 3
#define CA_SCN_INCOMING 4
#define CA_SCN_BLOCKS 5
#define CA_SCN_DEADLOCK 6
#define CA_SCN_CROWD_SEPARATED 7

enum ca_field {
    CA_FLD_POS_X = 0, CA_FLD_POS_Y, CA_FLD_VEL_X, CA_FLD_VEL_Y, CA_FLD_PREF_X, CA_FLD_PREF_Y,
    CA_FLD_GOAL_X, CA_FLD_GOAL_Y, CA_FLD_GOAL2_X, CA_FLD_GOAL2_Y,
    CA_FLD_REWARD,
    CA_FLD_AGENT_DONE,
    CA_FLD_ARRIVE_STEP,
    CA_FLD_NB_COUNT,
    CA_FLD_NB_IDX,
    CA_FLD_OBST_COUNT,
    CA_FLD_OBST_IDX,
    CA_FLD_OBS,
    CA_FLD_STEP_COUNT,
    CA_FLD_ARENA_DONE,
    CA_FLD_EPISODE,
    CA_FLD_REGOAL_COUNT,
    CA_FLD_ALAN_WEIGHTS,
    CA_FLD_ALAN_TIMES,
    CA_FLD_ALAN_ACTION,
    CA_FLD_ARENA_STATS,
    CA_FLD__COUNT
};

#define CA_MIN_LENGTH 1e-3f
#define CA_MAX_LENGTH 1e3f
#define CA_MIN_TIME_STEP 1e-4f
#define CA_MAX_TIME_STEP 10.0f
#define CA_MAX_COORD 1e5f
#define CA_MIN_EDGE 1e-4f

typedef struct ca_config {
    int32_t n_arenas;
    int32_t n_agents;
    int64_t arena_offset;
    uint64_t seed;
    double reward_scale;
    float time_step;
    float neighbor_dist;
    int32_t max_neighbors;
    float time_horizon;
    float time_horizon_obst;
    float radius;
    float max_speed;
    int32_t max_obst_neighbors;
    int32_t max_step;
    int32_t done_mode;
    float done_x_thresh;
    float spawn_x0, spawn_x1, spawn_y0, spawn_y1;
    float goal_x0, goal_x1, goal_y0, goal_y1;
} ca_config;

typedef struct ca_stats {
    uint64_t agent_steps;
    uint64_t episodes;
    uint64_t collisions;
    uint64_t obst_collisions;
    uint64_t goals_reached;
    uint64_t obst_overflow;
    double sum_reward;
} ca_stats;

typedef struct ca_env ca_env;

int ca_create(const ca_config* cfg, int device, void* stream, ca_env** out);
int ca_create_ex(const ca_config* cfg, uint32_t create_flags, int device, void* stream, ca_env** out);
int ca_destroy(ca_env* env);
const char* ca_last_error(const ca_env* env);
int ca_set_stream(ca_env* env, void* stream);

int ca_set_obstacles(ca_env* env, const float* verts_xy, const int32_t* poly_sizes, int32_t n_poly);
int ca_get_obstacles(ca_env* env, float* verts_xy, int32_t* next, int32_t* convex, int32_t cap, int32_t* n_out);
int ca_set_obstacles_per_arena(ca_env* env, const float* verts_xy, const int32_t* poly_sizes, const int32_t* n_poly);
int ca_get_obstacles_arena(ca_env* env, int32_t arena, float* verts_xy, int32_t* next, int32_t* convex, int32_t cap,
                           int32_t* n_out);

int ca_set_agent_params(ca_env* env, const float* radius, const float* max_speed, const float* time_horizon,
                        const float* time_horizon_obst, size_t bytes_each, int32_t src_is_device);
int ca_get_agent_params(ca_env* env, float* radius, float* max_speed, float* time_horizon,
                        float* time_horizon_obst, size_t bytes_each, int32_t dst_is_device);
int ca_agent_params_info(ca_env* env, int32_t* per_agent);

int ca_set_agent_counts(ca_env* env, const int32_t* counts, size_t bytes, int32_t src_is_device);
int ca_get_agent_counts(ca_env* env, int32_t* counts, size_t bytes, int32_t dst_is_device);
int ca_agent_counts_info(ca_env* env, int32_t* per_arena);

int ca_init_scenario(ca_env* env, int32_t scenario);

int ca_set(ca_env* env, int32_t field, const void* src, size_t bytes, int32_t src_is_device);
int ca_get(ca_env* env, int32_t field, void* dst, size_t bytes, int32_t dst_is_device);
int ca_host_alloc(ca_env* env, size_t bytes, void** out);
int ca_host_free(ca_env* env, void* p);
int ca_field_ptr(ca_env* env, int32_t field, void** dev_ptr, size_t* bytes);
int ca_bind_obs(ca_env* env, void* dev_ptr, size_t bytes);

int ca_reset(ca_env* env, const float* pos_x, const float* pos_y, int32_t pos_is_device, uint32_t flags);

int ca_reset_masked(ca_env* env, const int32_t* mask, int32_t mask_is_device, uint32_t flags);

int ca_step(ca_env* env, const float* actions, uint32_t flags);
int ca_step_host(ca_env* env, const float* actions_host, uint32_t flags);
int ca_step_packed(ca_env* env, const float* actions_host, uint32_t flags, void* out_host, size_t out_bytes);
int ca_orca_step(ca_env* env, uint32_t flags);
int ca_observe(ca_env* env);
int ca_rollout(ca_env* env, int32_t steps, uint32_t flags);

int ca_alan_configure(ca_env* env, const double* actions_xy, int32_t n_actions, double temp, double timewindow,
                      double time_step);
int ca_alan_configure_per_arena(ca_env* env, const double* actions_xy, const int32_t* n_actions, double temp,
                                double timewindow, double time_step);
int ca_alan_actions_arena(ca_env* env, int32_t arena, double* cs_xy, int32_t cap, int32_t* n_out);
int ca_alan_step(ca_env* env, const double* u, int32_t u_is_device, uint32_t flags);
int ca_alan_rollout(ca_env* env, int32_t steps, uint32_t flags);

int ca_allow_obstacle_overflow(ca_env* env, int32_t allow);

int ca_get_stats(ca_env* env, ca_stats* out);
int ca_reset_stats(ca_env* env);
int ca_sync(ca_env* env);

int ca_debug_math(ca_env* env, int32_t op, const void* in, void* out, int32_t n);

int ca_profile(ca_env* env, int32_t period);
int ca_profile_read(ca_env* env, int32_t counts[4], float mean_ms[4]);

int ca_launch_info(ca_env* env, int32_t* block, int32_t* grid, int32_t* lds_bytes, int32_t* obs_grid);
int ca_solver_info(ca_env* env, int32_t* lanes_per_agent, int32_t* rollout_one_launch);
int ca_tiled_info(ca_env* env, int32_t* tiled, int32_t* tile_agents, int32_t* tiles_per_arena, int32_t* launches_per_step);
const char* ca_source_sha(void);

#ifdef __cplusplus
}
#endif
#endif
```

Baseline: 2.429 billion.

## Precompute observation ray windows in step kernel and hand them to obs kernel

The step kernel now computes, for each agent's neighbors, the ray-window start, width and prefix-summed pair base, and packs them with the neighbor id into a per-agent work word. It also writes per-16-agent pair totals. A dedicated obs_kernel variant reads these words instead of recomputing ray_window, the wave prefix sum and the LDS atomic, so the obs pass does less work and synchronisation. The cost is extra global writes and reads, more registers in the step kernel, and new template instantiations. The path is only used for non-tiled configurations that meet the handoff_ok conditions and is disabled for rollouts.

```diff
diff --git a/collision_avoidance_amd/_lib.py b/collision_avoidance_amd/_lib.py
--- a/collision_avoidance_amd/_lib.py
+++ b/collision_avoidance_amd/_lib.py
@@ -23,7 +23,7 @@
            "ca_set_obstacles_per_arena", "ca_get_obstacles_arena", "ca_solver_info", "ca_source_sha", "ca_host_alloc", "ca_host_free",
            "ca_step_packed", "ca_allow_obstacle_overflow", "ca_alan_configure_per_arena", "ca_alan_actions_arena",
            "ca_set_agent_params", "ca_get_agent_params", "ca_agent_params_info",
-           "ca_set_agent_counts", "ca_get_agent_counts", "ca_agent_counts_info", "ca_create_ex", "ca_tiled_info")
+           "ca_set_agent_counts", "ca_get_agent_counts", "ca_agent_counts_info", "ca_create_ex", "ca_tiled_info", "ca_obs_handoff_info")
 
 
 class Config(C.Structure):
@@ -111,6 +111,7 @@
     L.ca_set_agent_counts.argtypes = [vp, vp, sz, i32]
     L.ca_get_agent_counts.argtypes = [vp, vp, sz, i32]
     L.ca_agent_counts_info.argtypes = [vp, C.POINTER(i32)]
+    L.ca_obs_handoff_info.argtypes = [vp, C.POINTER(i32)]
     L.ca_source_sha.argtypes = []
     L.ca_source_sha.restype = C.c_char_p
     for name in EXPORTS:
diff --git a/collision_avoidance_amd/csrc/ca_common.h b/collision_avoidance_amd/csrc/ca_common.h
--- a/collision_avoidance_amd/csrc/ca_common.h
+++ b/collision_avoidance_amd/csrc/ca_common.h
@@ -7,6 +7,7 @@
 struct WideObstLists;
 struct AgentParams;
 struct ArenaCounts;
+struct ObsHandoff;
 
 namespace ca {
 
@@ -48,6 +49,8 @@
     float spawn_x0, spawn_x1, spawn_y0, spawn_y1, goal_x0, goal_x1, goal_y0, goal_y1;
     const float *ap_radius, *ap_max_speed, *ap_time_horizon, *ap_time_horizon_obst;
     const int* agent_counts;
+    unsigned* obs_work;
+    int* obs_work_tot;
 };
 
 struct AlanCold {
diff --git a/collision_avoidance_amd/csrc/ca_env.hip b/collision_avoidance_amd/csrc/ca_env.hip
--- a/collision_avoidance_amd/csrc/ca_env.hip
+++ b/collision_avoidance_amd/csrc/ca_env.hip
@@ -68,7 +68,9 @@
     bool obs_dense_on = false;
     bool lists_trusted = true;
     int LS = 1, apb = 1, linv = 65536, dense = 0;
-    struct { int reg_lines = -1, pair = -1, alan_fused = -1; } sw;
+    struct { int reg_lines = -1, pair = -1, alan_fused = -1, obs_handoff = -1; } sw;
+    unsigned* oh_work = nullptr;
+    int* oh_tot = nullptr;
     int ST = 0, KT = 16;
     int SMX = 4;
     int max_edges = 0;
@@ -236,6 +238,7 @@
     c.ap_radius = e->ap ? e->d_ap[0] : nullptr; c.ap_max_speed = e->ap ? e->d_ap[1] : nullptr;
     c.ap_time_horizon = e->ap ? e->d_ap[2] : nullptr; c.ap_time_horizon_obst = e->ap ? e->d_ap[3] : nullptr;
     c.agent_counts = e->ac ? e->d_counts : nullptr;
+    c.obs_work = e->oh_work; c.obs_work_tot = e->oh_tot;
 }
 
 static void fill_args(ca_env* e, StepArgs& a, const float* actions, uint32_t flags) {
@@ -333,7 +336,19 @@
         default: return fn_ptr(&tiled_solve_kernel<KMAX, 128>);
     }
 }
-static SolveLaunch solve_launch(const ca_env* e, bool alan, bool rollout) {
+static const void* handoff_fn_for(const ca_env* e) {
+    const bool two = e->BS == 128;
+    if (e->SMX > 4) return e->KT == 5 ? (two ? fn_ptr(&step_kernel<5, 128, 4, 16, false, ObsHandoff>) : fn_ptr(&step_kernel<5, 64, 4, 16, false, ObsHandoff>))
+                                      : (two ? fn_ptr(&step_kernel<10, 128, 4, 16, false, ObsHandoff>) : fn_ptr(&step_kernel<10, 64, 4, 16, false, ObsHandoff>));
+    return e->KT == 5 ? (two ? fn_ptr(&step_kernel<5, 128, 4, 4, false, ObsHandoff>) : fn_ptr(&step_kernel<5, 64, 4, 4, false, ObsHandoff>))
+                      : (two ? fn_ptr(&step_kernel<10, 128, 4, 4, false, ObsHandoff>) : fn_ptr(&step_kernel<10, 64, 4, 4, false, ObsHandoff>));
+}
+static bool handoff_ok(const ca_env* e) {
+    return e->oh_work != nullptr && !e->tiled && !e->quad && !e->pair && !e->ap && !e->ac && e->ST > 0 && e->S <= SMAX &&
+           e->BS <= 128 && e->cfg.n_agents > 16;
+}
+static SolveLaunch solve_launch(const ca_env* e, bool alan, bool rollout, bool handoff = false) {
+    if (handoff) return {handoff_fn_for(e), dim3(e->grid), dim3(e->BS), e->lds};
     if (e->tiled)
         return {e->KT == 5 ? tiled_fn_for<5>(e->TILE) : (e->KT == 16 ? tiled_fn_for<16>(e->TILE) : tiled_fn_for<10>(e->TILE)),
                 dim3(e->grid), dim3(e->TILE), e->lds};
@@ -350,8 +365,8 @@
 static hipError_t allow_lds(const SolveLaunch& s) {
     return s.lds > 48 * 1024 ? hipFuncSetAttribute(s.fn, hipFuncAttributeMaxDynamicSharedMemorySize, (int)s.lds) : hipSuccess;
 }
-static hipError_t launch_step(ca_env* e, const StepArgs& a) {
-    const SolveLaunch s = solve_launch(e, a.alan != nullptr, a.T > 1);
+static hipError_t launch_step(ca_env* e, const StepArgs& a, bool handoff = false) {
+    const SolveLaunch s = solve_launch(e, a.alan != nullptr, a.T > 1, handoff);
     if (!(a.flags & CA_F_FREEZE)) e->lists_trusted = true;
     if (e->tiled) {
         TiledArgs ta;
@@ -402,7 +417,7 @@
     return ol > 48 * 1024 ? hipFuncSetAttribute(reinterpret_cast<const void*>(obs_fn_of(e)), hipFuncAttributeMaxDynamicSharedMemorySize, (int)ol) : hipSuccess;
 }
 
-static hipError_t launch_obs(ca_env* e) {
+static hipError_t launch_obs(ca_env* e, bool handoff = false) {
     if (!e->orient_valid) {
         StepArgs a;
         fill_args(e, a, nullptr, 0);
@@ -431,10 +446,11 @@
     memcpy(o.oct, e->oct, sizeof o.oct);
     o.ap_oct = e->ap ? e->d_ap_oct : nullptr;
     o.agent_counts = e->ac ? e->d_counts : nullptr;
+    o.work = e->oh_work; o.work_tot = e->oh_tot;
     const dim3 grid(o.dense ? (unsigned)(((size_t)o.A * o.N + apb - 1) / apb) : (unsigned)((size_t)o.A * o.bpa)), block(obs_bs);
     const size_t lds = obs_lds(e, obs_bs);
     ProfScope ps(e, KIND_OBS);
-    launch_k(ps, obs_fn_of(e), grid, block, lds, e->stream, o);
+    launch_k(ps, handoff ? obs_kernel<256, false, false, ObsHandoff> : obs_fn_of(e), grid, block, lds, e->stream, o);
     return hipGetLastError();
 }
 
@@ -571,6 +587,12 @@
     if (r != hipSuccess || *misfit) return r;
     r = allow_lds(plain);
     if (r == hipSuccess) r = allow_lds(solve_launch(e, false, true));
+    if (r == hipSuccess && handoff_ok(e)) {
+        r = allow_lds(solve_launch(e, false, false, true));
+        const size_t ol = obs_lds(e, 256);
+        if (r == hipSuccess && ol > 48 * 1024)
+            r = hipFuncSetAttribute(reinterpret_cast<const void*>(obs_kernel<256, false, false, ObsHandoff>), hipFuncAttributeMaxDynamicSharedMemorySize, (int)ol);
+    }
     return r;
 }
 
@@ -642,6 +664,7 @@
     {
         auto digit = [](const char* name) { const char* v = getenv(name); return (v && v[0] >= '0' && v[0] <= '9') ? v[0] - '0' : -1; };
         e->sw.reg_lines = digit("CA_REG_LINES"); e->sw.pair = digit("CA_PAIR"); e->sw.alan_fused = digit("CA_ALAN_FUSED");
+        e->sw.obs_handoff = digit("CA_OBS_HANDOFF");
     }
     e->tiled = tiled;
     if (tiled) {
@@ -755,6 +778,10 @@
     if (r == hipSuccess) r = dalloc(e, &e->dbg, (size_t)std::max(e->grid * (2 * e->BS / 64), e->grid_q * (e->BSq / 64)) * 16);
     if (r == hipSuccess) r = dalloc(e, &e->dbg_obs, (size_t)cfg->n_arenas * ((cfg->n_agents + 15) / 16 + 16) * 4 * 16);
 #endif
+    if (r == hipSuccess && e->sw.obs_handoff != 0 && !tiled && cfg->n_agents > 16 && e->BS <= 128 && e->K >= 1 && e->K <= 10 && e->S <= SMAX) {
+        r = dalloc(e, &e->oh_work, an * (size_t)e->K);
+        if (r == hipSuccess) r = dalloc(e, &e->oh_tot, A * (size_t)((cfg->n_agents + 15) / 16));
+    }
     bool lds_misfit = false;
     if (r == hipSuccess) r = apply_variant_attributes(e, &lds_misfit);
     if (r == hipSuccess) r = allow_obs_lds(e);
@@ -795,7 +822,7 @@
                     e->episode, e->arena_stats, e->arena_steps, e->d_obst, e->dbg, e->dbg_obs,
                     e->alan_w, e->alan_t, e->alan_dirs, e->alan_u, e->alan_action, e->d_alan, e->mask_buf,
                     e->d_act_tab, e->d_act_n, e->d_ap[0], e->d_ap[1], e->d_ap[2], e->d_ap[3], e->d_ap_oct, e->d_counts,
-                    e->nv_x, e->nv_y, e->tscr};
+                    e->nv_x, e->nv_y, e->tscr, e->oh_work, e->oh_tot};
     for (void* b : bufs) if (b) hipFree(b);
     for (const auto& h : e->host_allocs) hipHostFree(h.first);
     if (e->ovf_host) hipHostFree(e->ovf_host);
@@ -1560,14 +1587,15 @@
     return CA_OK;
 }
 
-static int do_step(ca_env* e, const float* actions, uint32_t flags) {
+static int do_step(ca_env* e, const float* actions, uint32_t flags, bool allow_handoff = true) {
     { const int rs = overflow_status(e, "step"); if (rs) return rs; }
     if (e->prof_period > 1) e->profiling = (e->steps_done % (uint64_t)e->prof_period) == 0;
     StepArgs a;
     fill_args(e, a, actions, flags);
-    HIPCHK(e, launch_step(e, a));
+    const bool handoff = allow_handoff && (flags & CA_F_OBS) && !(flags & CA_F_FREEZE) && handoff_ok(e);
+    HIPCHK(e, launch_step(e, a, handoff));
     e->orient_valid = true;
-    if (flags & CA_F_OBS) HIPCHK(e, launch_obs(e));
+    if (flags & CA_F_OBS) HIPCHK(e, launch_obs(e, handoff));
     e->steps_done += 1;
     return CA_OK;
 }
@@ -1843,7 +1871,7 @@
         return CA_OK;
     }
     for (int s = 0; s < steps; ++s) {
-        const int rc = do_step(e, nullptr, flags);
+        const int rc = do_step(e, nullptr, flags, false);
         if (rc) return rc;
     }
     return CA_OK;
@@ -2059,6 +2087,12 @@
     return CA_OK;
 }
 
+int ca_obs_handoff_info(ca_env* e, int32_t* obs_handoff) {
+    if (!e) return CA_EINVAL;
+    if (obs_handoff) *obs_handoff = handoff_ok(e) ? 1 : 0;
+    return CA_OK;
+}
+
 #ifndef CA_SRC_SHA
 #define CA_SRC_SHA "unknown"
 #endif
diff --git a/collision_avoidance_amd/csrc/ca_obs.h b/collision_avoidance_amd/csrc/ca_obs.h
--- a/collision_avoidance_amd/csrc/ca_obs.h
+++ b/collision_avoidance_amd/csrc/ca_obs.h
@@ -23,6 +23,8 @@
     float oct[32];
     const float* ap_oct;
     const int* agent_counts;
+    const unsigned* work;
+    const int* work_tot;
 };
 
 #ifdef CA_STAMPS
@@ -76,12 +78,34 @@
     return (u < 0.0f) ? u + 16.0f : u;
 }
 
+struct RayWindow { int i0, w; };
+__device__ __forceinline__ RayWindow ray_window(float rx, float ry, float c, float s, float R) {
+    int i0, w;
+    const float d2 = rx * rx + ry * ry;
+    const float ax = c * rx - s * ry, ay = s * rx + c * ry;
+    const bool all = !(d2 > 1.0404f * R * R);
+    const float ua = ray_dial(ax, ay);
+    const float t = R * __builtin_amdgcn_rsqf(d2);
+    const float t2 = t * t;
+    const float hw = t * (1.0f + t2 * (0.16666667f + t2 * (0.075f + t2 * 0.32914f))) * 2.54647908947f + 0.002f;
+    int i1 = (int)floorf(ua + hw);
+    i0 = (int)ceilf(ua - hw);
+    if (all || i1 - i0 >= 15) { i0 = 0; i1 = 15; }
+    w = max(i1 - i0 + 1, 0);
+    return {i0, w};
+}
+__device__ __forceinline__ unsigned obs_work_word(int nb, int i0, int w, int base) {
+    return (unsigned)nb | ((unsigned)(i0 & 15) << 8) | ((unsigned)w << 12) | ((unsigned)base << 17);
+}
+
 template <int OBS_BS, bool NW16, bool DENSE = false, class... WIDE_TAG>
 __global__ __launch_bounds__(OBS_BS) void obs_kernel(const ObsArgs p) {
     constexpr bool WIDE = has_tag<WideObstLists, WIDE_TAG...>;
     constexpr bool AC = has_tag<ArenaCounts, WIDE_TAG...>;
     constexpr bool AP = has_tag<AgentParams, WIDE_TAG...> || AC;
     static_assert(!(WIDE && AP), "per-agent parameters go with obstacle lists of up to 16");
+    constexpr bool OH = has_tag<ObsHandoff, WIDE_TAG...>;
+    static_assert(!OH || (sizeof...(WIDE_TAG) == 1 && OBS_BS == 256 && !NW16 && !DENSE), "the hand-off form: 256 lanes, 8-bit ids, one arena per workgroup");
     constexpr int OBS_APB = OBS_BS / 16;
     extern __shared__ float4 smem4[];
     const int tid = threadIdx.x;
@@ -153,6 +177,7 @@
     }
     int nn = 0, ns = 0;
     float c = 1.0f, s = 0.0f;
+    unsigned wk = 0u;
     if (active) {
         if constexpr (DENSE) {
             const int cnts = p.counts[q];
@@ -169,7 +194,8 @@
             c = (p.orient_x + aoff)[ii]; s = -(p.orient_y + aoff)[ii];
             const unsigned li = (unsigned)r * (unsigned)N + ii;
             const char* nbase = (const char*)p.nb_idx + aoff * (size_t)K * (NW16 ? 2 : 1);
-            if (r < nn) s_nb[g * 16 + r] = ld_idx_t<NW16>(nbase, li);
+            if constexpr (OH) { if (r < nn) { wk = (p.work + aoff * (size_t)K)[li]; s_nb[g * 16 + r] = (int)(wk & 0xFFu); } }
+            else if (r < nn) s_nb[g * 16 + r] = ld_idx_t<NW16>(nbase, li);
             if constexpr (WIDE) { for (unsigned t = (unsigned)r; t < (unsigned)ns; t += 16u) s_ob[g * OBW + t] = (int)(p.obst_idx + aoff * (size_t)S)[t * (unsigned)N + ii]; }
             else if (r < ns) s_ob[g * 16 + r] = (int)(p.obst_idx + aoff * (size_t)S)[li];
         }
@@ -188,7 +214,7 @@
         const int k = r;
         int i0 = 0, w = 0;
         if (k < nn) {
-            const int nb = s_nb[g * 16 + k];
+            const int nb = OH ? (int)(wk & 0xFFu) : s_nb[g * 16 + k];
             const float rx = (GATHER ? gpx[nb] : s_px[nb]) - mx, ry = (GATHER ? gpy[nb] : s_py[nb]) - my;
             s_rel[g * 16 + k] = make_float2(rx, ry);
             float Rk = p.radius;
@@ -200,22 +226,16 @@
                 for (int e = 0; e < 8; ++e) dst[e] = src[e];
                 Rk = src[0].x;
             }
-            const float d2 = rx * rx + ry * ry, R = Rk;
-            const float ax = c * rx - s * ry, ay = s * rx + c * ry;
-            const bool all = !(d2 > 1.0404f * R * R);
-            const float ua = ray_dial(ax, ay);
-            const float t = R * __builtin_amdgcn_rsqf(d2);
-            const float t2 = t * t;
-            const float hw = t * (1.0f + t2 * (0.16666667f + t2 * (0.075f + t2 * 0.32914f))) * 2.54647908947f + 0.002f;
-            int i1 = (int)floorf(ua + hw);
-            i0 = (int)ceilf(ua - hw);
-            if (all || i1 - i0 >= 15) { i0 = 0; i1 = 15; }
-            w = max(i1 - i0 + 1, 0);
-        }
-        const int incl = wave_prefix_sum(w);
+            if constexpr (OH) { i0 = (int)((wk >> 8) & 15u); w = (int)((wk >> 12) & 31u); }
+            else { const RayWindow rw = ray_window(rx, ry, c, s, Rk); i0 = rw.i0; w = rw.w; }
+        }
         int base = 0;
-        if ((tid & 63) == 63) base = atomicAdd(&s_cnt[0], incl);
-        base = __builtin_amdgcn_readlane(base, 63) + (incl - w);
+        if constexpr (OH) base = (int)(wk >> 17);
+        else {
+            const int incl = wave_prefix_sum(w);
+            if ((tid & 63) == 63) base = atomicAdd(&s_cnt[0], incl);
+            base = __builtin_amdgcn_readlane(base, 63) + (incl - w);
+        }
         const unsigned short hd = (unsigned short)((g << 8) | (k << 4));
 #pragma unroll
         for (int t2 = 0; t2 < 4; ++t2)
@@ -327,7 +347,9 @@
         if (best_m >= 0)
             atomicMin(&s_key[ga * 16 + ray], ((unsigned long long)__float_as_uint(best) << 32) | (unsigned)best_m);
     };
-    const int ntot = s_cnt[0];
+    int ntot;
+    if constexpr (OH) ntot = p.work_tot[(size_t)p.a0 * p.bpa + bid];
+    else ntot = s_cnt[0];
     for (int pi = tid; pi < ntot; pi += OBS_BS) {
         const int pr = s_pair[pi];
         const int ga = pr >> 8, k = (pr >> 4) & 15, ray = pr & 15;
diff --git a/collision_avoidance_amd/csrc/ca_step.h b/collision_avoidance_amd/csrc/ca_step.h
--- a/collision_avoidance_amd/csrc/ca_step.h
+++ b/collision_avoidance_amd/csrc/ca_step.h
@@ -3,6 +3,7 @@
 #include "ca_lines.h"
 #include "ca_nbr.h"
 #include "ca_rules.h"
+#include "ca_obs.h"
 
 namespace ca {
 
@@ -59,6 +60,8 @@
     constexpr bool AC = has_tag<ArenaCounts, PER...>;
     constexpr bool AP = has_tag<AgentParams, PER...> || AC;
     static_assert(!AP || (ST == 0 && !ALAN && SMX <= SMAX), "per-agent parameters: the LDS line table with lists of up to 16, no ALAN form");
+    constexpr bool OH = has_tag<ObsHandoff, PER...>;
+    static_assert(!OH || (sizeof...(PER) == 1 && ST > 0 && BS <= 128 && !ALAN), "the hand-off form: register lines, one or two waves, no ALAN form");
     extern __shared__ float4 smem4[];
     constexpr bool LISTP = BS > 64 && !AP;
     __shared__ unsigned s_vmax2;
@@ -508,6 +511,10 @@
         done = 0;
         c.agent_done[q] = 0;
         pref = goal_dir(pos, gx, gy);
+        if constexpr (OH) {
+            if constexpr (LISTP) { s_px[tid] = pos.x; s_py[tid] = pos.y; }
+            else s_xy2[2 * lbase + i] = make_float2(pos.x, pos.y);
+        }
     }
     if ((p.actions || ALAN) && (p.flags & 2u)) {
         double r = active ? (double)(ALAN ? rew_alan : rew) : 0.0;
@@ -538,6 +545,44 @@
             c.step_count[a] = do_reset ? 0 : steps;
             atomicAdd(&c.arena_steps[a], 1ull);
             if (do_reset) c.episode[a] = epi + 1;
+        }
+    }
+    if constexpr (OH) {
+        const size_t wg0 = (size_t)(p.a0 + work_block(p) * apb) * (size_t)(K * N);
+        const unsigned loff = (unsigned)la * (unsigned)(K * N) + (unsigned)i;
+        int wtot = 0;
+        unsigned pw[KMAX];
+        static_for<KMAX>([&](auto kc) __attribute__((always_inline)) { pw[decltype(kc)::value] = 0u; });
+        if (active) {
+            const int ncnt = (int)(p.counts[q] & 0xFFu);
+            int jn[KMAX];
+            static_for<KMAX>([&](auto kc) __attribute__((always_inline)) {
+                constexpr int k = decltype(kc)::value;
+                jn[k] = (k < ncnt) ? ld_idx_t<CA_NBW16(BS)>((const char*)p.nb_idx + wg0 * (CA_NBW16(BS) ? 2 : 1), loff + (unsigned)(k * N)) : 0;
+            });
+            float nx[KMAX], ny[KMAX];
+            static_for<KMAX>([&](auto kc) __attribute__((always_inline)) {
+                constexpr int k = decltype(kc)::value;
+                if constexpr (LISTP) { nx[k] = s_px[lbase + jn[k]]; ny[k] = s_py[lbase + jn[k]]; }
+                else { const float2 o2 = s_xy2[2 * lbase + jn[k]]; nx[k] = o2.x; ny[k] = o2.y; }
+            });
+            static_for<KMAX>([&](auto kc) __attribute__((always_inline)) {
+                constexpr int k = decltype(kc)::value;
+                int i0 = 0, w = 0;
+                if (k < ncnt) { const RayWindow rw = ray_window(nx[k] - pos.x, ny[k] - pos.y, ox, -oy, p.radius); i0 = rw.i0; w = rw.w; }
+                pw[k] = obs_work_word(jn[k], i0, w, wtot);
+                wtot += w;
+            });
+        }
+        const int excl = wave_prefix_sum(wtot) - wtot;
+        const int bbase = excl - __builtin_amdgcn_ds_bpermute(((tid & 63) - (i & 15)) << 2, excl);
+        if (active) {
+            CA_GLOBAL unsigned* wp = (CA_GLOBAL unsigned*)c.obs_work + wg0;
+            static_for<KMAX>([&](auto kc) __attribute__((always_inline)) {
+                constexpr int k = decltype(kc)::value;
+                if (k < K) wp[loff + (unsigned)(k * N)] = pw[k] + ((unsigned)bbase << 17);
+            });
+            if ((i & 15) == 15 || i == N - 1) ((CA_GLOBAL int*)c.obs_work_tot)[(size_t)a * ((N + 15) >> 4) + (i >> 4)] = bbase + wtot;
         }
     }
     }
diff --git a/collision_avoidance_amd/vec_env.py b/collision_avoidance_amd/vec_env.py
--- a/collision_avoidance_amd/vec_env.py
+++ b/collision_avoidance_amd/vec_env.py
@@ -289,9 +289,11 @@
         per, cnt = C.c_int32(), C.c_int32()
         self._call("ca_agent_params_info", self.h, C.byref(per))
         self._call("ca_agent_counts_info", self.h, C.byref(cnt))
+        oh = C.c_int32()
+        self._call("ca_obs_handoff_info", self.h, C.byref(oh))
         return dict(block=v[0].value, grid=v[1].value, lds_bytes=v[2].value, obs_grid=v[3].value,
                     lanes_per_agent=lanes.value, rollout_one_launch=roll.value, agent_params=bool(per.value),
-                    agent_counts=bool(cnt.value))
+                    agent_counts=bool(cnt.value), obs_handoff=bool(oh.value))
 
     def tiled_info(self):
         v = [C.c_int32() for _ in range(4)]
diff --git a/include/ca_env.h b/include/ca_env.h
--- a/include/ca_env.h
+++ b/include/ca_env.h
@@ -170,6 +170,7 @@
 int ca_launch_info(ca_env* env, int32_t* block, int32_t* grid, int32_t* lds_bytes, int32_t* obs_grid);
 int ca_solver_info(ca_env* env, int32_t* lanes_per_agent, int32_t* rollout_one_launch);
 int ca_tiled_info(ca_env* env, int32_t* tiled, int32_t* tile_agents, int32_t* tiles_per_arena, int32_t* launches_per_step);
+int ca_obs_handoff_info(ca_env* env, int32_t* obs_handoff);
 const char* ca_source_sha(void);
 
 #ifdef __cplusplus
```

New measurement: 2.404 billion. 0.99x the previous value.
